# NVIDIAGameWorks/kaolin-wisp

Hardware: AMD Instinct MI355X
Metric: training rays/sec, HashGrid NeRF (nerf_hash.yaml), synthetic Lego 800x800 (higher is better)
Workload: dtype bf16

## Files before the change

### include/wisp_hip.h

```cpp
#ifndef WISP_HIP_H
#define WISP_HIP_H

#include <stdint.h>

#ifdef __cplusplus
extern "C" {
#endif

typedef void* wisp_stream_t;

enum { WISP_F32 = 0, WISP_F16 = 1, WISP_BF16 = 2 };

enum {
    WISP_OK = 0,
    WISP_ERR_INVALID = -1,
    WISP_ERR_LAUNCH = -2,
    WISP_ERR_UNSUPPORTED = -3,
    WISP_ERR_CAPACITY = -4
};

const char* wisp_last_error(void);
int wisp_abi_version(void);

int wisp_hashgrid_interpolate_fwd(const float* coords, int64_t n, int coord_dim,
                                  const void* codebook, int dtype, int feature_dim,
                                  const int64_t* first_idx, const int32_t* resolutions, int num_lods,
                                  int codebook_bitwidth, int zero_from_col,
                                  void* feats, wisp_stream_t stream);

int wisp_hashgrid_interpolate_bwd(const float* coords, int64_t n, int coord_dim,
                                  const void* grad_feats, int dtype, int feature_dim,
                                  const int64_t* first_idx, const int32_t* resolutions, int num_lods,
                                  int codebook_bitwidth, int zero_from_col,
                                  float* grad_codebook, void* workspace, int64_t workspace_bytes,
                                  const float* level_cap_scale , wisp_stream_t stream);
int64_t wisp_hashgrid_bwd_workspace_bytes(int64_t n, int coord_dim, int dtype ,
                                          int feature_dim, const int32_t* resolutions , int num_lods,
                                          int codebook_bitwidth, const float* level_cap_scale );
int wisp_hashgrid_bwd_slot_stats(int64_t n, int coord_dim, int dtype, int feature_dim, const int32_t* resolutions ,
                                 int num_lods, int codebook_bitwidth, int zero_from_col, const float* level_cap_scale,
                                 const void* workspace, int64_t workspace_bytes, uint32_t* max_fill, int32_t* cap_host,
                                 int32_t* base_cap_host, wisp_stream_t stream);

int wisp_hashgrid_grad_coords(const float* coords, int64_t n, int coord_dim, const void* grad_feats, const void* codebook,
                              int dtype, int feature_dim, const int64_t* first_idx, const int32_t* resolutions ,
                              int num_lods, int codebook_bitwidth, float* grad_coords, wisp_stream_t stream);

int wisp_hashgrid_interpolate_bwd_adamw(const float* coords, int64_t n, int coord_dim,
                                        const void* grad_feats, int dtype, int feature_dim,
                                        const int64_t* first_idx, const int32_t* resolutions, int num_lods,
                                        int codebook_bitwidth, int zero_from_col,
                                        float* grad_codebook, void* workspace, int64_t workspace_bytes,
                                        const float* level_cap_scale, float* param, float* exp_avg, float* exp_avg_sq,
                                        void* bf16_shadow, float lr, float beta1, float beta2, float eps, float weight_decay,
                                        int64_t step, float grad_scale, int64_t* covered_rows , wisp_stream_t stream);

typedef struct wisp_step_tail {
    const float* dw_partials;
    float* dec_grad;
    const float* loss_partials;
    float* loss;
    int32_t dw_rows, in_dim, loss_count;
    float inv_n;
} wisp_step_tail;
int wisp_hashgrid_interpolate_bwd_adamw_tail(const float* coords, int64_t n, int coord_dim,
                                             const void* grad_feats, int dtype, int feature_dim,
                                             const int64_t* first_idx, const int32_t* resolutions, int num_lods,
                                             int codebook_bitwidth, int zero_from_col,
                                             float* grad_codebook, void* workspace, int64_t workspace_bytes,
                                             const float* level_cap_scale, float* param, float* exp_avg, float* exp_avg_sq,
                                             void* bf16_shadow, float lr, float beta1, float beta2, float eps, float weight_decay,
                                             int64_t step, float grad_scale, int64_t* covered_rows ,
                                             const wisp_step_tail* tail, int* tail_done , wisp_stream_t stream);

int wisp_hashgrid_cells(const float* coords, int64_t n, int coord_dim, int32_t resolution, int codebook_bitwidth,
                        int32_t* cell, float* frac, int32_t* corner_idx, wisp_stream_t stream);

int wisp_hashgrid_query_fwd(const float* coords, int64_t n, const void* const* codebooks, int dtype, int feature_dim,
                            const int32_t* resolutions, int num_lods, int codebook_bitwidth, int probe_bitwidth,
                            void* feats, wisp_stream_t stream);
int wisp_hashgrid_query_bwd(const float* coords, int64_t n, const void* grad_feats, int dtype, int feature_dim,
                            const int32_t* resolutions, int num_lods, int codebook_bitwidth, int probe_bitwidth,
                            void* const* grad_codebooks, wisp_stream_t stream);

int wisp_spc_query(const uint8_t* octree, const int32_t* exsum, const float* coords, int64_t n,
                   int level, int with_parents, int64_t* pidx ,
                   wisp_stream_t stream);

int wisp_spc_query_chain(const uint8_t* octree, const int32_t* exsum, const int16_t* points, const float* coords,
                         int64_t n, int level, int first_level, const int32_t* hint_pidx, int hint_group,
                         int64_t* chain, wisp_stream_t stream);

int wisp_spc_build_bitfield(const int16_t* level_points, int64_t n_points, int level, uint32_t* bits,
                            wisp_stream_t stream);

int wisp_spc_mask_from_points(const int16_t* points, int64_t n, int level, uint8_t* leaf_mask, wisp_stream_t stream);
int wisp_spc_dense_bytes(uint8_t* dense, int level, wisp_stream_t stream);
int wisp_spc_points_from_index(const int64_t* index, int64_t n, int level, int16_t* points, wisp_stream_t stream);

int wisp_spc_raytrace_count(const uint8_t* octree, const int16_t* points, const int32_t* exsum,
                            const float* origins, const float* dirs, int64_t num_rays, int level,
                            int32_t* counts, float* cache, int cache_cap, wisp_stream_t stream);
int wisp_spc_raytrace_emit(const uint8_t* octree, const int16_t* points, const int32_t* exsum,
                           const float* origins, const float* dirs, int64_t num_rays, int level,
                           const int64_t* offsets, int with_exit, const float* cache, int cache_cap,
                           int32_t* ridx, int32_t* pidx, float* depth, wisp_stream_t stream);

int wisp_spc_first_hit(const uint8_t* octree, const int16_t* points, const int32_t* exsum,
                       const float* origins, const float* dirs, int64_t num_rays, int level,
                       const float* colors, int color_stride, int32_t level_first,
                       int32_t* pidx, float* depth, float* rgb, float* alpha, uint8_t* hit, wisp_stream_t stream);

int wisp_mark_pack_boundaries_i64(const int64_t* ids, int64_t n, uint8_t* boundary, wisp_stream_t stream);
int wisp_mark_pack_boundaries_i32(const int32_t* ids, int64_t n, uint8_t* boundary, wisp_stream_t stream);

int64_t wisp_scan_workspace_bytes(int64_t n);
int wisp_exclusive_scan_i32(const int32_t* counts, int64_t n, int64_t* offsets, void* workspace,
                            wisp_stream_t stream);
int wisp_inclusive_scan_i32(const int32_t* in, int64_t n, int32_t* out, void* workspace,
                            wisp_stream_t stream);
int wisp_boundary_tile_counts(const uint8_t* boundary, int64_t n, int32_t* counts, wisp_stream_t stream);
int wisp_boundary_pack_starts(const uint8_t* boundary, int64_t n, const int64_t* tile_offsets,
                              int64_t* starts, wisp_stream_t stream);

int wisp_spc_trilinear_coeffs(const float* coords, const int16_t* voxel_points , int64_t num_voxels,
                              int samples_per_voxel, int level, float* coeffs , wisp_stream_t stream);
int wisp_spc_trilinear_fwd(const float* coords, const void* pidx, int pidx_is_i64, const int16_t* points,
                           const int32_t* trinkets, const void* feats, int dtype, int64_t num_voxels,
                           int samples_per_voxel, int channels, int level, int half_round, float* out,
                           wisp_stream_t stream);
int wisp_spc_trilinear_bwd(const float* coords, const void* pidx, int pidx_is_i64, const int16_t* points,
                           const int32_t* trinkets, const float* grad_out, int64_t num_voxels,
                           int samples_per_voxel, int channels, int level, int64_t num_rows,
                           float* grad_feats , void* workspace, int64_t workspace_bytes,
                           wisp_stream_t stream);
int64_t wisp_spc_bwd_workspace_bytes(int64_t total_rows, int channels, int64_t dict_elems);

int wisp_spc_trilinear_multi_fwd(const float* coords, const int64_t* chain, int64_t chain_stride, const int16_t* points,
                                 const int32_t* trinkets, const void* const* feats, int dtype, int64_t num_samples,
                                 int num_lods, const int32_t* levels, int channels, int half_round, int sum, float* out,
                                 wisp_stream_t stream);
int wisp_spc_trilinear_multi_bwd(const float* coords, const int64_t* chain, int64_t chain_stride, const int16_t* points,
                                 const int32_t* trinkets, const float* grad_out, int64_t num_samples, int num_lods,
                                 const int32_t* levels, const int64_t* rows, int channels, int sum,
                                 float* const* grad_feats, void* workspace, int64_t workspace_bytes, wisp_stream_t stream);

int wisp_triplane_fwd(const float* coords, int64_t num_samples, const float* const* planes, const int32_t* sizes,
                      int num_lods, int feature_dim, int sum, float* out, wisp_stream_t stream);
int wisp_triplane_bwd(const float* coords, int64_t num_samples, const float* grad_out, const int32_t* sizes, int num_lods,
                      int feature_dim, int sum, float* const* grad_planes, wisp_stream_t stream);

int wisp_grid_interpolate_fwd(const float* coords, const void* feats, int dtype, int64_t num_coords, int feature_dim,
                              void* out, wisp_stream_t stream);
int wisp_grid_interpolate_bwd(const float* coords, const void* grad_out, int dtype, int64_t num_coords, int feature_dim,
                              void* grad_feats, wisp_stream_t stream);

// ... 244 lines not shown
                                        int64_t workspace_bytes, int* partial_rows , wisp_stream_t stream);
int wisp_nerf_mlp_reduce_partials(const float* workspace, int partial_rows, int in_dim, float* grad_params, wisp_stream_t stream);

int wisp_small_decoder_fwd(const float* x, int64_t n, int in_dim, int hidden, const float* w1, const float* b1,
                           const float* w2, const float* b2, float* out , wisp_stream_t stream);
int wisp_small_decoder_bwd(const float* x, int64_t n, int in_dim, int hidden, const float* w1, const float* b1,
                           const float* w2, const float* b2, const float* grad_out, float* grad_x, float* grad_w1,
                           float* grad_b1, float* grad_w2, float* grad_b2, wisp_stream_t stream);

int wisp_adamw_step(float* param, const float* grad, float* exp_avg, float* exp_avg_sq, int64_t n,
                    float lr, float beta1, float beta2, float eps, float weight_decay, int64_t step,
                    float grad_scale, int zero_grad , void* bf16_shadow,
                    wisp_stream_t stream);
int wisp_adamw_step_groups(float* param, const float* grad, float* exp_avg, float* exp_avg_sq, int num_groups,
                           const int64_t* group_begin, const int64_t* group_len, const float* group_lr,
                           const float* group_weight_decay, void* const* group_bf16_shadow, float beta1, float beta2,
                           float eps, int64_t step, float grad_scale, int zero_grad, wisp_stream_t stream);

int wisp_optim_step_groups(int kind, float* param, const float* grad, float* state1, float* state2, int num_groups,
                           const int64_t* group_begin, const int64_t* group_len, const float* group_lr,
                           const float* group_weight_decay, void* const* group_bf16_shadow, float hyper0, float hyper1,
                           float eps, int64_t step, float grad_scale, int zero_grad, wisp_stream_t stream);

int wisp_gather_rows(const int64_t* index, int64_t num, int64_t num_src_rows, int num_tensors, const float* const* src,
                     const int* width, float* const* dst, wisp_stream_t stream);

void* wisp_host_reader_create(void);
int wisp_host_reader_issue(void* reader, const int64_t* src, wisp_stream_t stream);
int wisp_host_reader_wait(void* reader, int64_t* value );
void wisp_host_reader_destroy(void* reader);

typedef struct wisp_nerf_step_config {
    int64_t struct_bytes;
    const uint32_t* occ_bits;
    const uint8_t* octree;
    const int32_t* exsum;
    const uint32_t* coarse_bits;
    const void* table_lookup;
    const int64_t* first_idx;
    const int64_t* first_idx_host;
    const int32_t* resolutions;
    float* table_param;
    float* table_grad;
    float* table_exp_avg;
    float* table_exp_avg_sq;
    void* table_shadow;
    const float* dec_params;
    float* dec_grad;
    float* flat_param;
    float* flat_grad;
    float* flat_exp_avg;
    float* flat_exp_avg_sq;
    void* grid_shadow;
    int64_t decoder_begin, decoder_len, grid_begin, grid_len, rest_begin, rest_len;
    int64_t table_offset;
    int64_t max_rays, max_samples;
    int32_t level, coarse_level, num_samples , loss_kind ;
    int32_t dtype_table, num_lods, feature_dim, bitwidth;
    int32_t zero_from_col, in_dim, hidden, view_freqs;
    float near, range ;
    float bg[3];
    float reserved;
} wisp_nerf_step_config;

typedef struct wisp_nerf_step_hyper {
    int64_t struct_bytes;
    int64_t step;
    float lr_decoder, lr_grid, lr_rest, weight_decay, beta1, beta2, eps, grad_scale;
    int32_t optimizer;
    int32_t tail_fold;
} wisp_nerf_step_hyper;

int64_t wisp_nerf_step_config_bytes(void);
int64_t wisp_nerf_step_workspace_bytes(const wisp_nerf_step_config* cfg);
void* wisp_nerf_step_create(const wisp_nerf_step_config* cfg, void* workspace, int64_t workspace_bytes);
int wisp_nerf_step_reconfigure(void* step, const wisp_nerf_step_config* cfg);
void wisp_nerf_step_destroy(void* step);
int wisp_nerf_step_count(void* step, int slot, const float* origins, const float* dirs, int64_t num_rays, uint64_t seed,
                         wisp_stream_t stream);
int wisp_nerf_step_run(void* step, int slot, const float* gts, const float* next_origins, const float* next_dirs,
                       int64_t next_num_rays, uint64_t next_seed, const wisp_nerf_step_hyper* hp,
                       const float* level_cap_scale, void* hashgrid_workspace, int64_t hashgrid_workspace_bytes,
                       int record_timing, int64_t* num_samples, int64_t* covered_rows, float** loss, wisp_stream_t stream);
int wisp_nerf_step_read_timing(void* step, int max_steps, float* ms, int64_t* units, int* num_steps);

int wisp_mesh_to_sdf(const double* points, int64_t n, const double* mesh, int64_t f, int triangle_ranges,
                     int64_t max_pairs_per_launch, double* sdf, void* workspace, int64_t workspace_bytes, wisp_stream_t stream);
int wisp_mesh_to_sdf_triangle(const double* points, int64_t n, const double* mesh, int64_t f, int triangle_ranges,
                              int64_t max_pairs_per_launch, double* out, void* workspace, int64_t workspace_bytes,
                              wisp_stream_t stream);
int64_t wisp_mesh_sdf_workspace_bytes(int64_t n, int64_t f);

typedef struct wisp_tex_material {
    int64_t offset;
    int32_t height, width;
    float kd[3];
    int32_t has_map;
} wisp_tex_material;
int wisp_mesh_closest_tex(const double* points, int64_t n, const double* mesh, int64_t f, const void* tidx, int tidx_is_i64,
                          const float* texv, int64_t tv, const int64_t* texf, const float* texels, int64_t num_texels,
                          const wisp_tex_material* materials, int num_materials, double* hit, float* rgb, wisp_stream_t stream);
int wisp_mesh_sample_tex(const float* uv, const int64_t* material, int64_t n, const float* texels, int64_t num_texels,
                         const wisp_tex_material* materials, int num_materials, float* rgb, wisp_stream_t stream);

int wisp_multiview_sample(const uint8_t* images, const float* cameras, const float* camera_host, int64_t num_views, int height,
                          int width, int mip, int has_alpha, const int64_t* pix, const int64_t* view, int64_t view_index,
                          int64_t num_rays, float x0, float y0, float tan_half_fov_x, float tan_half_fov_y, const float* bg,
                          float* origins, float* dirs, float* rgb, uint8_t* mask, wisp_stream_t stream);

int wisp_image_sample(const uint8_t* image, int height, int width, const int64_t* pix, int64_t n, float* coords, float* rgb,
                      wisp_stream_t stream);

int wisp_image_field_render(const float* coords, int64_t first, int64_t n, int height, int width, const float* codebook,
                            const int64_t* first_idx, const int32_t* resolutions, int num_lods, int active_lods,
                            int codebook_bitwidth, const float* weights, int hidden_padded, const uint8_t* gts, float* out_f32,
                            uint8_t* out_u8, double* err_partials, wisp_stream_t stream);
int64_t wisp_image_field_render_partials(int64_t n);

int64_t wisp_image_field_train_scratch_bytes(int64_t n, int num_lods, int hidden);
int wisp_image_field_train_step(const float* coords, const float* rgb, int64_t n, const float* codebook, const int64_t* first_idx,
                                const int32_t* resolutions, int num_lods, int active_lods, int codebook_bitwidth, const float* w1,
                                const float* b1, const float* w2, const float* b2, int hidden, float* grad_codebook,
                                float* grad_w1, float* grad_b1, float* grad_w2, float* grad_b2, float* loss, float* pred,
                                void* scratch, int64_t scratch_bytes, wisp_stream_t stream);

int64_t wisp_ssim_scratch_bytes(int H, int W, int C);
int wisp_ssim(const float* x, int64_t x_row_stride, int64_t x_pix_stride, const float* y, int64_t y_row_stride,
              int64_t y_pix_stride, int H, int W, int C, int radius, const double* weights, double cov_norm, double c1, double c2,
              double* out, double* map, void* scratch, int64_t scratch_bytes, wisp_stream_t stream);

#ifdef __cplusplus
}
#endif
#endif
```

### kaolin-wisp_amd/csrc/hashgrid.hip

```cpp
#include "wisp_common.h"
#include <stdlib.h>

#include "hashgrid_dev.h"
#include "step_tail_dev.h"

#define HG_TILE 64

#define FW_WAVES 4
template <typename T, int F, int DIM>
__global__ void __launch_bounds__(FW_WAVES * 64)
hashgrid_fwd_kernel(const float* __restrict__ coords, int64_t n, const T* __restrict__ codebook,
                    const int64_t* __restrict__ first_idx, HashLevels lv, int num_lods, uint32_t tsize,
                    int tsize_pow2, int zero_from_col, int row_shift, int off32, T* __restrict__ feats) {
    extern __shared__ __attribute__((aligned(16))) uint32_t stage_all[];
    constexpr int W = (F * (int)sizeof(T)) / 4;
    const int lane = threadIdx.x & 63;
    const int wave = threadIdx.x >> 6;
    uint32_t* stage = stage_all + (size_t)wave * num_lods * 65 * W;
    const int64_t ntiles = (n + HG_TILE - 1) / HG_TILE;
    const int row_dw = num_lods * W;

    const int nwaves = blockDim.x >> 6;
    for (int64_t tile = (int64_t)blockIdx.x * nwaves + wave; tile < ntiles; tile += (int64_t)gridDim.x * nwaves) {
        const int64_t i = tile * HG_TILE + lane;
        const bool live = i < n;
        float c[DIM];
#pragma unroll
        for (int a = 0; a < DIM; ++a) c[a] = live ? coords[i * DIM + a] : 0.0f;

        for (int l = 0; l < num_lods; ++l) {
            const int32_t res = lv.res[l];
            const bool dense = lv.dense[l] != 0;
            float acc[F];
#pragma unroll
            for (int k = 0; k < F; ++k) acc[k] = 0.0f;
            if (live && l * F < zero_from_col) {
                const T* __restrict__ table = codebook + first_idx[l] * F;
                CornerSetup<DIM> cs;
                corner_setup<DIM>(c, res, lv.hi[l], lv.hr[l], dense, tsize, tsize_pow2 != 0, cs);
                if (dense && res >= 258) {
                    const int64_t last = first_idx[num_lods] - 1 - first_idx[l];
#pragma unroll
                    for (int j = 0; j < (1 << DIM); ++j)
                        if ((int64_t)(uint32_t)cs.idx[j] > last) cs.idx[j] = (int32_t)last;
                }
                T v[1 << DIM][F];
                auto fetch = [&](int j, const T* p) {
                    if constexpr (W == 1) {
                        *reinterpret_cast<uint32_t*>(&v[j][0]) = *reinterpret_cast<const uint32_t*>(p);
                    } else if constexpr (W == 2) {
                        *reinterpret_cast<uint2*>(&v[j][0]) = *reinterpret_cast<const uint2*>(p);
                    } else if constexpr (W == 4) {
                        *reinterpret_cast<uint4*>(&v[j][0]) = *reinterpret_cast<const uint4*>(p);
                    } else {
#pragma unroll
                        for (int k = 0; k < F; ++k) v[j][k] = p[k];
                    }
                };
                if (off32 && (W == 1 || W == 2 || W == 4)) {
                    const __amdgpu_buffer_rsrc_t rsrc =
                        __builtin_amdgcn_make_buffer_rsrc(const_cast<T*>(table), (short)0, (int)0x7fffffff, 0x00020000);
                    if (W == 1 && dense && res < 258) {
                        constexpr int half = 1 << (DIM - 1);
                        typedef uint32_t u32x2_t __attribute__((ext_vector_type(2)));
#pragma unroll
                        for (int j = 0; j < half; ++j) {
                            const int voff = (int)((uint32_t)cs.idx[j] * (uint32_t)(F * sizeof(T)));
                            const u32x2_t t = __builtin_amdgcn_raw_buffer_load_b64(rsrc, voff, 0, 0);
                            *reinterpret_cast<uint32_t*>(&v[j][0]) = t[0];
                            *reinterpret_cast<uint32_t*>(&v[j + half][0]) = t[1];
                        }
                    } else if (W == 1 && !dense && tsize_pow2 != 0 && tsize >= 2u) {
                        constexpr int half = 1 << (DIM - 1);
                        typedef uint32_t u32x2_t __attribute__((ext_vector_type(2)));
#pragma unroll
                        for (int j = 0; j < half; ++j) {
                            const uint32_t i0 = (uint32_t)cs.idx[j];
                            const u32x2_t t = __builtin_amdgcn_raw_buffer_load_b64(rsrc, (int)((i0 & ~1u) * 4u), 0, 0);
                            const bool upper = (i0 & 1u) != 0;
                            *reinterpret_cast<uint32_t*>(&v[j][0]) = upper ? t[1] : t[0];
                            *reinterpret_cast<uint32_t*>(&v[j + half][0]) = upper ? t[0] : t[1];
                        }
                        if (cs.cell[0] & 1) {
#pragma unroll
// ... 125 lines not shown
                    asm volatile("v_fmac_f32_dpp %0, %0, %1 " DPPSTR : "+v"(v[j][k]) : "v"(tk));             \
            heads |= take & (SRC_FLAGS);                                                                   \
        }                                                                                                  \
    }
    HG_SEG_STEP("row_shr:1 row_mask:0xf bank_mask:0xf", 0xfffefffefffefffeull, heads << 1)
    HG_SEG_STEP("row_shr:2 row_mask:0xf bank_mask:0xf", 0xfffcfffcfffcfffcull, heads << 2)
    HG_SEG_STEP("row_shr:4 row_mask:0xf bank_mask:0xf", 0xfff0fff0fff0fff0ull, heads << 4)
    HG_SEG_STEP("row_shr:8 row_mask:0xf bank_mask:0xf", 0xff00ff00ff00ff00ull, heads << 8)
    HG_SEG_STEP("row_bcast:15 row_mask:0xa bank_mask:0xf", 0xffff0000ffff0000ull,
                (((heads >> 15) & 1ull) ? 0x00000000ffff0000ull : 0ull) | (((heads >> 47) & 1ull) ? 0xffff000000000000ull : 0ull))
    HG_SEG_STEP("row_bcast:31 row_mask:0xc bank_mask:0xf", 0xffffffff00000000ull,
                ((heads >> 31) & 1ull) ? 0xffffffff00000000ull : 0ull)
#undef HG_SEG_STEP
    const uint64_t emitters = tails & __builtin_amdgcn_ballot_w64(live);
    uint32_t is_tail;
    asm volatile("v_cndmask_b32_e64 %0, 0, 1, %1" : "=v"(is_tail) : "s"(emitters));
    return is_tail != 0;
}

template <typename T, int F, int DIM, bool MERGE>
__global__ void __launch_bounds__(1024)
hashgrid_bwd_kernel(const float* __restrict__ coords, int64_t n, const T* __restrict__ grad_feats,
                    const int64_t* __restrict__ first_idx, HashLevels lv, LevelList levels, int num_lods, uint32_t tsize,
                    int tsize_pow2, int zero_from_col, float* __restrict__ grad_codebook) {
    const int lane = threadIdx.x & 63;
    const int wave = threadIdx.x >> 6;
    const int nwaves = blockDim.x >> 6;
    const int64_t ntiles = (n + HG_TILE - 1) / HG_TILE;
    for (int64_t tile = blockIdx.x; tile < ntiles; tile += gridDim.x) {
        const int64_t i = tile * HG_TILE + lane;
        const bool live = i < n;
        float c[DIM];
#pragma unroll
        for (int a = 0; a < DIM; ++a) c[a] = live ? coords[i * DIM + a] : 0.0f;
        for (int li = wave; li < levels.n; li += nwaves) {
            const int l = __builtin_amdgcn_readfirstlane(levels.lv[li]);
            const int32_t res = __builtin_amdgcn_readfirstlane(lv.res[l]);
            const bool dense = __builtin_amdgcn_readfirstlane(lv.dense[l]) != 0;
            CornerSetup<DIM> cs;
            float v[1 << DIM][F];
            const bool issue = tail_compute<T, F, DIM, MERGE>(c, live, l, res, lv.hi[l], lv.hr[l], dense, tsize, tsize_pow2 != 0, zero_from_col,
                                                              grad_feats + (i * num_lods + l) * F, lane, cs, v);
            if (issue) {
                const int64_t base = first_idx[l], total_rows = first_idx[num_lods];
#pragma unroll
                for (int j = 0; j < (1 << DIM); ++j) {
                    const int64_t row = base + (int64_t)(uint32_t)cs.idx[j];
                    if (row >= total_rows) continue;
                    float* p = grad_codebook + row * F;
#pragma unroll
                    for (int k = 0; k < F; ++k) atomicAdd(p + k, v[j][k]);
                }
            }
        }
    }
}

#ifndef EM_THREADS
#define EM_THREADS 512
#endif
#ifndef EM_GROUPS
#define EM_GROUPS 2
#endif
#define EM_TILE (EM_THREADS * EM_GROUPS)
#ifndef EM_MIN_WAVES
#define EM_MIN_WAVES 2
#endif
#ifndef EQ_THREADS
#define EQ_THREADS 512
#endif
#define EQ_WIDE 1024
#define EQ_WIDE_MIN ((int64_t)1 << 20)
#define EQ_SMALL 1024
#define EQ_SMALL_GROUPS 1
#define RD_THREADS 1024
#define BIN_MAX_CHUNKS 1024
#ifndef HG_ACC_PLANES
#define HG_ACC_PLANES 1
#endif
#ifndef HG_FLUSH_PAIRS
#define HG_FLUSH_PAIRS 1
#endif

template <typename T, int F> struct RecordCodec {
    static constexpr bool COMPACT = (sizeof(T) == 2 && F == 2);
    static constexpr int RW = COMPACT ? 2 : 1 + F;
    static __device__ __forceinline__ uint32_t store(uint32_t* dst, uint32_t loc, const float (&v)[F]) {
        if constexpr (COMPACT) {
            uint2 w;
            w.x = ((__float_as_uint(v[0]) + 0x40u) & ~0x7fu) | (loc & 0x7fu);
            w.y = ((__float_as_uint(v[1]) + 0x40u) & ~0x7fu) | (loc >> 7);
            *reinterpret_cast<uint2*>(dst) = w;
            return max(w.x & 0x7fffff80u, w.y & 0x7fffff80u);
        } else {
            dst[0] = loc;
            uint32_t m = 0;
#pragma unroll
            for (int k = 0; k < F; ++k) { dst[1 + k] = __float_as_uint(v[k]); m = max(m, __float_as_uint(v[k]) & 0x7fffffffu); }
            return m;
        }
    }
    static __device__ __forceinline__ uint32_t load(const uint32_t (&w)[RW], float (&v)[F]) {
        if constexpr (COMPACT) {
            v[0] = __uint_as_float(w[0] & ~0x7fu);
            v[1] = __uint_as_float(w[1] & ~0x7fu);
            return (w[0] & 0x7fu) | ((w[1] & 0x7fu) << 7);
        } else {
#pragma unroll
            for (int k = 0; k < F; ++k) v[k] = __uint_as_float(w[1 + k]);
            return w[0];
        }
    }
};

template <typename T, int F, int DIM>
__global__ void __launch_bounds__(EM_THREADS, EM_MIN_WAVES)
hashgrid_bwd_emit_kernel(const float* __restrict__ coords, int64_t n, const T* __restrict__ grad_feats,
                         const int64_t* __restrict__ first_idx, HashLevels lv, LevelList levels, int num_lods,
                         uint32_t tsize, int tsize_pow2, int zero_from_col, int chunk_shift, BinLevels bins,
                         uint32_t* __restrict__ counts, uint32_t* __restrict__ records, float* __restrict__ grad_codebook) {
    constexpr int NC = 1 << DIM;
    typedef RecordCodec<T, F> Codec;
    constexpr int RW = Codec::RW;
    constexpr int GROUPS = EM_TILE / EM_THREADS;
    static_assert((F * sizeof(T)) % 4 == 0, "a (sample, level) gradient is a whole number of dwords");
    constexpr int W = (F * (int)sizeof(T)) / 4;
    extern __shared__ __attribute__((aligned(16))) uint32_t em_smem[];
    const int total_ranks = bins.rank_base[levels.n];
    uint32_t* s_rank = em_smem;
    uint32_t* s_mx = em_smem + total_ranks;
    uint32_t* s_grad = em_smem + total_ranks + 1;
    uint32_t mx = 0;
    if (threadIdx.x == 0) *s_mx = 0;
    const int row_dw = num_lods * W;
    const int rowp = row_dw | 1;
    const int lane = threadIdx.x & 63;
    const int wave = threadIdx.x >> 6;
    const uint32_t ntiles = gridDim.x;
    const int64_t tile0 = (int64_t)blockIdx.x * EM_TILE;
    const int64_t total_rows = first_idx[num_lods];
    for (int b = threadIdx.x; b < total_ranks; b += EM_THREADS) s_rank[b] = 0;
    {
        const int64_t rows = (n - tile0) < (int64_t)EM_TILE ? (n - tile0) : (int64_t)EM_TILE;
        const uint32_t* __restrict__ src = reinterpret_cast<const uint32_t*>(grad_feats) + tile0 * row_dw;
        const int total = (int)rows * row_dw;
        for (int e = threadIdx.x; e < total; e += EM_THREADS) {
            const int r = e / row_dw;
            s_grad[r * rowp + (e - r * row_dw)] = src[e];
        }
    }
    float c[GROUPS][DIM];
    bool live[GROUPS];
#pragma unroll
    for (int g = 0; g < GROUPS; ++g) {
        const int64_t i = tile0 + (int64_t)(wave * GROUPS + g) * 64 + lane;
        live[g] = i < n;
#pragma unroll
        for (int a = 0; a < DIM; ++a) c[g][a] = live[g] ? coords[i * DIM + a] : 0.0f;
    }
    __syncthreads();
    for (int li = 0; li < levels.n; ++li) {
        const int l = levels.lv[li];
        const int32_t res = lv.res[l];
        const bool dense = lv.dense[l] != 0;
        const uint32_t cap = bins.cap[li];
        uint32_t* rank_l = s_rank + bins.rank_base[li];
        uint32_t* __restrict__ rec_l = records + (size_t)bins.rec_base[li] * RW;
        const uint32_t bucket_stride = __builtin_amdgcn_readfirstlane(ntiles * cap);
        const uint32_t slot0 = __builtin_amdgcn_readfirstlane(blockIdx.x * cap);
        const int64_t rows_l = first_idx[l + 1] - first_idx[l];
        const uint32_t owned = (uint32_t)(rows_l < (int64_t)bins.entries[li] ? (rows_l < 0 ? 0 : rows_l) : (int64_t)bins.entries[li]);
        const uint32_t magic = bins.strip_magic[li], nbuckets = (uint32_t)bins.chunks[li], rot_mask = bins.rot_mask[li];
#pragma unroll
        for (int g = 0; g < GROUPS; ++g) {
            const int sl = (wave * GROUPS + g) * 64 + lane;
            CornerSetup<DIM> cs;
            float v[NC][F];
            const bool issue = tail_compute<T, F, DIM, true>(c[g], live[g], l, res, lv.hi[l], lv.hr[l], dense, tsize, tsize_pow2 != 0, zero_from_col,
                                                             reinterpret_cast<const T*>(s_grad + sl * rowp + l * W), lane, cs, v);
            if (!issue) continue;
            uint32_t pos[NC];
#pragma unroll
            for (int j = 0; j < NC; ++j) {
                const uint32_t idx = (uint32_t)cs.idx[j];
                uint32_t b, loc;
                bucket_of(idx, chunk_shift, magic, nbuckets, rot_mask, b, loc);
                pos[j] = idx < owned ? atomicAdd(&rank_l[b], 1u) : 0xffffffffu;
            }
#pragma unroll
            for (int j = 0; j < NC; ++j) {
                const uint32_t idx = (uint32_t)cs.idx[j];
                uint32_t b, loc;
                bucket_of(idx, chunk_shift, magic, nbuckets, rot_mask, b, loc);
                if (pos[j] < cap) {
                    uint32_t* dst = rec_l + (size_t)((b * bucket_stride + slot0 + pos[j]) * RW);
                    mx = max(mx, Codec::store(dst, loc, v[j]));
                } else {
                    const int64_t row = first_idx[l] + (int64_t)idx;
                    if (row < total_rows) {
                        float* p = grad_codebook + row * F;
#pragma unroll
                        for (int k = 0; k < F; ++k) atomicAdd(p + k, v[j][k]);
                    }
                }
            }
        }
    }
    if (mx) atomicMax(s_mx, mx);
    __syncthreads();
    if (threadIdx.x == 0) counts[bins.max_base + blockIdx.x] = *s_mx;
    for (int li = 0; li < levels.n; ++li) {
        const int chunks = bins.chunks[li];
        const uint32_t cap = bins.cap[li];
        const uint32_t* rank_l = s_rank + bins.rank_base[li];
        uint32_t* __restrict__ cnt_l = counts + bins.cnt_base[li];
        for (int b = threadIdx.x; b < chunks; b += EM_THREADS) {
            const uint32_t cn = rank_l[b];
            cnt_l[(size_t)b * ntiles + blockIdx.x] = cn < cap ? cn : cap;
        }
    }
}

#define EQ_MAX_ROW 16
template <typename T, int DIM, int THREADS, int GROUPS = 2>
__global__ void __launch_bounds__(THREADS, EM_MIN_WAVES)
hashgrid_bwd_emit_q_kernel(const float* __restrict__ coords, int64_t n, const T* __restrict__ grad_feats,
                           const int64_t* __restrict__ first_idx, HashLevels lv, LevelList levels, int num_lods,
                           uint32_t tsize, int tsize_pow2, int zero_from_col, int chunk_shift, BinLevels bins,
                           uint32_t* __restrict__ counts, uint32_t* __restrict__ records, float* __restrict__ grad_codebook) {
    constexpr int F = 2;
    constexpr int NC = 1 << DIM;
    typedef RecordCodec<T, F> Codec;
    static_assert(Codec::COMPACT, "two 16-bit features per level");
    constexpr int RW = Codec::RW;
    constexpr int TILE = THREADS * GROUPS;
    constexpr int QROW = 3 * NC + 1;
    extern __shared__ __attribute__((aligned(16))) uint32_t em_smem[];
    const int total_ranks = bins.rank_base[levels.n];
    uint32_t* s_rank = em_smem;
    uint32_t* s_mx = em_smem + total_ranks;
    uint32_t mx = 0;
    if (threadIdx.x == 0) *s_mx = 0;
    const int lane = threadIdx.x & 63;
    const int wave = threadIdx.x >> 6;
    uint32_t* s_queue = em_smem + ((total_ranks + 4) & ~3) + wave * (64 * QROW);
    const uint32_t ntiles = gridDim.x;
    const int64_t total_rows = first_idx[num_lods];
    for (int b = threadIdx.x; b < total_ranks; b += THREADS) s_rank[b] = 0;
    __syncthreads();
    const uint32_t q_lane = (uint32_t)((lane / NC) * QROW + (lane % NC) * 3);
    const int64_t pieces = (n + TILE - 1) / TILE;
    for (int64_t piece = blockIdx.x; piece < pieces; piece += gridDim.x) {
        const int64_t tile0 = piece * TILE;
        float c[GROUPS][DIM];
        bool live[GROUPS];
        typedef uint32_t row_t __attribute__((ext_vector_type(EQ_MAX_ROW)));
        row_t grow[GROUPS];
#pragma unroll
        for (int g = 0; g < GROUPS; ++g) {
            const int64_t i = tile0 + (int64_t)(wave * GROUPS + g) * 64 + lane;
            live[g] = i < n;
#pragma unroll
            for (int a = 0; a < DIM; ++a) c[g][a] = live[g] ? coords[i * DIM + a] : 0.0f;
            const uint32_t* __restrict__ src = reinterpret_cast<const uint32_t*>(grad_feats) + (live[g] ? i : 0) * num_lods;
            if (num_lods == EQ_MAX_ROW) {
#pragma unroll
                for (int q = 0; q < EQ_MAX_ROW / 4; ++q) {
                    const uint4 t = reinterpret_cast<const uint4*>(src)[q];
                    grow[g][4 * q] = t.x; grow[g][4 * q + 1] = t.y; grow[g][4 * q + 2] = t.z; grow[g][4 * q + 3] = t.w;
                }
            } else {
#pragma unroll
                for (int q = 0; q < EQ_MAX_ROW; ++q) grow[g][q] = q < num_lods ? src[q] : 0u;
            }
        }
        for (int li = 0; li < levels.n; ++li) {
            const int l = levels.lv[li];
            const int32_t res = lv.res[l];
            const bool dense = lv.dense[l] != 0;
            const uint32_t cap = bins.cap[li];
            uint32_t* rank_l = s_rank + bins.rank_base[li];
            uint32_t* __restrict__ rec_l = records + (size_t)bins.rec_base[li] * RW;
            const uint32_t bucket_stride = __builtin_amdgcn_readfirstlane(ntiles * cap);
            const uint32_t slot0 = __builtin_amdgcn_readfirstlane(blockIdx.x * cap);
            const int64_t base_l = first_idx[l];
            const int64_t rows_l = first_idx[l + 1] - base_l;
            const uint32_t owned = (uint32_t)(rows_l < (int64_t)bins.entries[li] ? (rows_l < 0 ? 0 : rows_l) : (int64_t)bins.entries[li]);
            const uint32_t magic = bins.strip_magic[li], nbuckets = (uint32_t)bins.chunks[li], rot_mask = bins.rot_mask[li];
#pragma unroll
            for (int g = 0; g < GROUPS; ++g) {
                CornerSetup<DIM> cs;
                float v[NC][F];
                uint32_t gw = grow[g][l & (EQ_MAX_ROW - 1)];
                const bool issue = tail_compute<T, F, DIM, true>(c[g], live[g], l, res, lv.hi[l], lv.hr[l], dense, tsize, tsize_pow2 != 0, zero_from_col,
                                                                 reinterpret_cast<const T*>(&gw), lane, cs, v);
                const uint64_t tails = __builtin_amdgcn_ballot_w64(issue);
                if (tails == 0) continue;
                if (issue) {
                    const uint32_t t = __builtin_amdgcn_mbcnt_hi((uint32_t)(tails >> 32), __builtin_amdgcn_mbcnt_lo((uint32_t)tails, 0u));
                    uint32_t* q = s_queue + t * QROW;
#pragma unroll
                    for (int j = 0; j < NC; ++j) {
                        q[3 * j] = (uint32_t)cs.idx[j];
                        q[3 * j + 1] = __float_as_uint(v[j][0]);
                        q[3 * j + 2] = __float_as_uint(v[j][1]);
                    }
                }
                __builtin_amdgcn_fence(__ATOMIC_RELEASE, "wavefront");
                __builtin_amdgcn_wave_barrier();
                const uint32_t total = (uint32_t)__popcll(tails) * NC;
                for (uint32_t p = 0; p < total; p += 64) {
                    if (p + lane < total) {
                        const uint32_t* q = s_queue + (p / NC) * QROW + q_lane;
                        const uint32_t idx = q[0];
                        float val[F];
                        val[0] = __uint_as_float(q[1]);
                        val[1] = __uint_as_float(q[2]);
                        uint32_t b, loc;
                        bucket_of(idx, chunk_shift, magic, nbuckets, rot_mask, b, loc);
                        const uint32_t pos = idx < owned ? atomicAdd(&rank_l[b], 1u) : 0xffffffffu;
                        if (pos < cap) {
                            uint32_t* dst = rec_l + (size_t)((b * bucket_stride + slot0 + pos) * RW);
                            mx = max(mx, Codec::store(dst, loc, val));
                        } else {
                            const int64_t row = base_l + (int64_t)idx;
                            if (row < total_rows) {
                                float* pg = grad_codebook + row * F;
                                atomicAdd(pg, val[0]);
                                atomicAdd(pg + 1, val[1]);
                            }
                        }
                    }
                }
                __builtin_amdgcn_fence(__ATOMIC_ACQUIRE, "wavefront");
                __builtin_amdgcn_wave_barrier();
            }
        }
    }
    if (mx) atomicMax(s_mx, mx);
    __syncthreads();
    if (threadIdx.x == 0) counts[bins.max_base + blockIdx.x] = *s_mx;
    for (int li = 0; li < levels.n; ++li) {
        const int chunks = bins.chunks[li];
        const uint32_t cap = bins.cap[li];
        const uint32_t* rank_l = s_rank + bins.rank_base[li];
        uint32_t* __restrict__ cnt_l = counts + bins.cnt_base[li];
        for (int b = threadIdx.x; b < chunks; b += THREADS) {
            const uint32_t cn = rank_l[b];
            cnt_l[(size_t)b * ntiles + blockIdx.x] = cn < cap ? cn : cap;
        }
    }
}

static inline size_t queue_emitter_lds(int total_ranks, int dim, int threads) {
    return ((size_t)((total_ranks + 4) & ~3) + (size_t)(threads / 64) * 64 * (3 * (1 << dim) + 1)) * 4;
}
template <typename T, int DIM, int THREADS, int GROUPS = 2>
static int queue_emitter_residency() {
    static const int v = [] {
        int nb = 0;
        auto eq = hashgrid_bwd_emit_q_kernel<T, DIM, THREADS, GROUPS>;
        const size_t lds = queue_emitter_lds(1024, DIM, THREADS);
        (void)hipFuncSetAttribute(reinterpret_cast<const void*>(eq), hipFuncAttributeMaxDynamicSharedMemorySize, (int)lds);
        if (hipOccupancyMaxActiveBlocksPerMultiprocessor(&nb, eq, THREADS, lds) != hipSuccess || nb <= 0) nb = THREADS >= 1024 ? 1 : 2;
        return nb;
    }();
    return v;
}

struct AccFix64 {
    unsigned long long* acc;
    float mul;
    double inv;
    __device__ __forceinline__ void zero(uint32_t i) const { acc[i] = 0ull; }
    __device__ __forceinline__ void add(uint32_t i, float v) const {
        const float a = fabsf(v) * mul;
        const float h = floorf(a);
        const unsigned long long mag = ((unsigned long long)(uint32_t)h << 32) | (uint32_t)((a - h) * 4294967296.0f);
        const unsigned long long sgn = (unsigned long long)(long long)((int32_t)__float_as_uint(v) >> 31);
        const unsigned long long q = (mag ^ sgn) - sgn;
        atomicAdd(acc + i, q);
    }
    __device__ __forceinline__ float get(uint32_t i) const { return (float)((double)(long long)acc[i] * inv); }
};
struct AccF32 {
    float* acc;
    __device__ __forceinline__ void zero(uint32_t i) const { acc[i] = 0.0f; }
    __device__ __forceinline__ void add(uint32_t i, float v) const { atomicAdd(acc + i, v); }
    __device__ __forceinline__ float get(uint32_t i) const { return acc[i]; }
};

struct AdamFlush {
    float* p; float* m; float* v; __hip_bfloat16* shadow;
    float lr, wd, b1, b2, eps, bc1, bc2_sqrt, gscale;
};
#define HG_TAIL_ROWS 8192
#define WISP_WHOLE_LEVEL ((int64_t)1 << 62)
struct TailLevels { int first_level, end_level, blocks; };
struct StepTail {
    const float* dw_partials; float* dec_grad; const float* loss_partials; float* loss;
    int dw_rows, in_dim, loss_count; float inv_n;
    int loss_wgs, dw_wgs, wgs;
};
static_assert(RD_THREADS == STEP_TAIL_THREADS, "the side jobs run in reduce workgroups");

template <typename T, int F, typename ACC, bool ADAM>
static __device__ __forceinline__ void
hashgrid_bwd_reduce_body(const ACC A, const int64_t* __restrict__ first_idx, const LevelList& levels, int chunk_shift,
                         const BinLevels& bins, uint32_t ntiles, const uint32_t* __restrict__ counts,
                         const uint32_t* __restrict__ records, float* __restrict__ grad_codebook, int li, int b, int z,
                         const AdamFlush& ad) {
    typedef RecordCodec<T, F> Codec;
    constexpr int RW = Codec::RW;
    const int splits = bins.splits[li];
    const int l = levels.lv[li];
    const uint32_t csize = 1u << chunk_shift;
    const uint32_t cap = bins.cap[li];
    const uint32_t first = (uint32_t)b << chunk_shift;
    const int64_t rows_l = first_idx[l + 1] - first_idx[l];
    const uint32_t entries = (uint32_t)(rows_l < (int64_t)bins.entries[li] ? (rows_l < 0 ? 0 : rows_l) : (int64_t)bins.entries[li]);
    const uint32_t magic = bins.strip_magic[li], nbuckets = (uint32_t)bins.chunks[li], rot_mask = bins.rot_mask[li];
    const bool strips = magic != 0;
    const uint32_t strip_rounds = (((entries + (1u << HG_STRIP_SHIFT) - 1u) >> HG_STRIP_SHIFT) + nbuckets - 1u) / nbuckets;
    const uint32_t lim = (strips ? min(strip_rounds << HG_STRIP_SHIFT, csize) : (entries > first ? min(entries - first, csize) : 0u)) * F;
    auto ax = [&](uint32_t x) -> uint32_t {
#if HG_ACC_PLANES
        return (x % (uint32_t)F) * csize + x / (uint32_t)F;
#else
        return x;
#endif
    };
    for (uint32_t e = threadIdx.x; e < lim; e += RD_THREADS) A.zero(ax(e));
    __syncthreads();
    const uint32_t* __restrict__ cnt = counts + bins.cnt_base[li] + (size_t)b * ntiles;
    const uint32_t* __restrict__ src = records + ((size_t)bins.rec_base[li] + (size_t)b * ntiles * cap) * RW;
    const int lane = threadIdx.x & 63, wave = threadIdx.x >> 6;
    constexpr int NW = RD_THREADS / 64;
    constexpr int INFLIGHT = 8;
    const uint32_t my_tiles = ntiles > (uint32_t)z ? (ntiles - z + splits - 1) / splits : 0u;
    for (uint32_t base = 0; base * NW + wave < my_tiles; base += 64) {
        const uint32_t k = (base + lane) * NW + wave;
        const uint32_t cnt_of_lane = k < my_tiles ? cnt[z + k * splits] : 0u;
        const uint32_t cc = (cnt_of_lane + 63u) >> 6;
        uint32_t inc = cc;
#pragma unroll
        for (int d = 1; d < 64; d <<= 1) {
            const uint32_t t = (uint32_t)__shfl_up((int)inc, d, 64);
            if (lane >= d) inc += t;
        }
        const uint32_t exc = inc - cc;
        const uint32_t pairs = (uint32_t)__builtin_amdgcn_readlane((int)inc, 63);
        for (uint32_t p0 = 0; p0 < pairs; p0 += INFLIGHT) {
            uint32_t w[INFLIGHT][RW];
            bool act[INFLIGHT];
#pragma unroll
            for (int u = 0; u < INFLIGHT; ++u) {
                const uint32_t pr = p0 + u < pairs ? p0 + u : p0;
                const int t = __popcll(__ballot(exc <= pr)) - 1;
                const uint32_t chunk = pr - (uint32_t)__builtin_amdgcn_readlane((int)exc, t);
                const uint32_t n_t = (uint32_t)__builtin_amdgcn_readlane((int)cnt_of_lane, t);
                const uint32_t r = chunk * 64 + lane;
                act[u] = (p0 + u < pairs) && r < n_t;
                const uint32_t tile = z + ((base + t) * NW + wave) * splits;
                const uint32_t* rec = src + ((size_t)tile * cap + (act[u] ? r : 0u)) * RW;
#pragma unroll
                for (int q = 0; q < RW; ++q) w[u][q] = rec[q];
            }
#pragma unroll
            for (int u = 0; u < INFLIGHT; ++u) {
                if (act[u]) {
                    float val[F];
                    const uint32_t e = Codec::load(w[u], val);
#pragma unroll
                    for (int kk = 0; kk < F; ++kk) {
#ifdef HG_EXP_NOATOM
                        if (e == 0xffffffffu && val[kk] == 123.0f)
#endif
                        A.add(ax(e * F + kk), val[kk]);
                    }
                }
            }
        }
    }
    __syncthreads();
    if (strips) {
        float* __restrict__ dl = grad_codebook + first_idx[l] * F;
        if constexpr (ADAM) {
            if (splits == 1) {
                const int64_t level0 = first_idx[l] * F;
                float2* __restrict__ pg = reinterpret_cast<float2*>(dl);
                float2* __restrict__ pp = reinterpret_cast<float2*>(ad.p + level0);
                float2* __restrict__ pm = reinterpret_cast<float2*>(ad.m + level0);
                float2* __restrict__ pv = reinterpret_cast<float2*>(ad.v + level0);
                uint32_t* __restrict__ ps = ad.shadow ? reinterpret_cast<uint32_t*>(ad.shadow + level0) : nullptr;
                constexpr int PQ = 4;
                const uint32_t pairs = lim / F;
                if ((((uintptr_t)grad_codebook | (uintptr_t)ad.p | (uintptr_t)ad.m | (uintptr_t)ad.v) & 7u) != 0) {
                    for (uint32_t e = threadIdx.x; e < lim; e += RD_THREADS) {
                        const uint32_t row = bucket_row((uint32_t)b, e / (uint32_t)F, chunk_shift, magic, nbuckets, rot_mask);
                        if (row >= entries) continue;
                        const int64_t x = level0 + (int64_t)row * F + e % (uint32_t)F;
                        const float c = grad_codebook[x];
                        float w = ad.p[x], m1 = ad.m[x], m2 = ad.v[x];
                        wisp_adamw_update(w, m1, m2, (c + A.get(ax(e))) * ad.gscale, ad.lr, ad.wd, ad.b1, ad.b2, ad.eps, ad.bc1, ad.bc2_sqrt);
                        ad.p[x] = w; ad.m[x] = m1; ad.v[x] = m2;
                        if (c != 0.0f) grad_codebook[x] = 0.0f;
                        if (ad.shadow) ad.shadow[x] = __float2bfloat16(w);
                    }
                    return;
                }
                for (uint32_t i0 = threadIdx.x; i0 < pairs; i0 += PQ * RD_THREADS) {
                    float2 cg[PQ], cp[PQ], cm[PQ], cv[PQ];
                    uint32_t row[PQ];
#pragma unroll
                    for (int q = 0; q < PQ; ++q) {
                        const uint32_t i = i0 + q * RD_THREADS;
                        row[q] = i < pairs ? bucket_row((uint32_t)b, i, chunk_shift, magic, nbuckets, rot_mask) : 0xffffffffu;
                        if (row[q] < entries) { cg[q] = pg[row[q]]; cp[q] = pp[row[q]]; cm[q] = pm[row[q]]; cv[q] = pv[row[q]]; }
                    }
#pragma unroll
                    for (int q = 0; q < PQ; ++q) {
                        const uint32_t i = i0 + q * RD_THREADS;
                        if (row[q] < entries) {
                            const bool dirty = cg[q].x != 0.0f || cg[q].y != 0.0f;
                            const float g0 = cg[q].x + A.get(ax(2 * i)), g1 = cg[q].y + A.get(ax(2 * i + 1));
                            wisp_adamw_update(cp[q].x, cm[q].x, cv[q].x, g0 * ad.gscale, ad.lr, ad.wd, ad.b1, ad.b2, ad.eps, ad.bc1, ad.bc2_sqrt);
                            wisp_adamw_update(cp[q].y, cm[q].y, cv[q].y, g1 * ad.gscale, ad.lr, ad.wd, ad.b1, ad.b2, ad.eps, ad.bc1, ad.bc2_sqrt);
                            pp[row[q]] = cp[q];
                            pm[row[q]] = cm[q];
                            pv[row[q]] = cv[q];
                            if (dirty) pg[row[q]] = make_float2(0.0f, 0.0f);
                            if (ps) {
                                const __hip_bfloat16 s0 = __float2bfloat16(cp[q].x), s1 = __float2bfloat16(cp[q].y);
                                ps[row[q]] = (uint32_t)__bfloat16_as_ushort(s0) | ((uint32_t)__bfloat16_as_ushort(s1) << 16);
                            }
                        }
                    }
                }
                return;
            }
        }
        auto elem = [&](uint32_t e) -> uint32_t {
            const uint32_t row = bucket_row((uint32_t)b, e / (uint32_t)F, chunk_shift, magic, nbuckets, rot_mask);
            return row < entries ? row * (uint32_t)F + e % (uint32_t)F : 0xffffffffu;
        };
        if (splits == 1) {
            constexpr int MAXE = 16;
            float cur[MAXE];
#pragma unroll
            for (int q = 0; q < MAXE; ++q) {
                const uint32_t e = threadIdx.x + q * RD_THREADS;
                const uint32_t x = e < lim ? elem(e) : 0xffffffffu;
                cur[q] = x != 0xffffffffu ? dl[x] : 0.0f;
            }
#pragma unroll
            for (int q = 0; q < MAXE; ++q) {
                const uint32_t e = threadIdx.x + q * RD_THREADS;
                const uint32_t x = e < lim ? elem(e) : 0xffffffffu;
                if (x != 0xffffffffu) {
                    const float a = A.get(ax(e));
                    if (a != 0.0f) dl[x] = cur[q] + a;
                }
            }
        } else {
            for (uint32_t e = threadIdx.x; e < lim; e += RD_THREADS) {
                const uint32_t x = elem(e);
                const float a = A.get(ax(e));
                if (x != 0xffffffffu && a != 0.0f) atomicAdd(dl + x, a);
            }
        }
        return;
    }
    const int64_t slice = (first_idx[l] + (int64_t)first) * F;
    float* __restrict__ dst = grad_codebook + slice;
    if constexpr (ADAM) {
        if (splits == 1) {
            float* __restrict__ pp = ad.p + slice;
            float* __restrict__ pm = ad.m + slice;
            float* __restrict__ pv = ad.v + slice;
            __hip_bfloat16* __restrict__ ps = ad.shadow ? ad.shadow + slice : nullptr;
            constexpr int PQ = 4;
            const uint32_t pairs = lim >> 1;
            if ((lim & 1u) == 0 && (((uintptr_t)dst | (uintptr_t)pp | (uintptr_t)pm | (uintptr_t)pv) & 7u) == 0) {
                for (uint32_t i0 = threadIdx.x; i0 < pairs; i0 += PQ * RD_THREADS) {
                    float2 cg[PQ], cp[PQ], cm[PQ], cv[PQ];
#pragma unroll
                    for (int q = 0; q < PQ; ++q) {
                        const uint32_t i = i0 + q * RD_THREADS;
                        if (i < pairs) {
                            cg[q] = reinterpret_cast<const float2*>(dst)[i]; cp[q] = reinterpret_cast<const float2*>(pp)[i];
                            cm[q] = reinterpret_cast<const float2*>(pm)[i]; cv[q] = reinterpret_cast<const float2*>(pv)[i];
                        }
                    }
#pragma unroll
                    for (int q = 0; q < PQ; ++q) {
                        const uint32_t i = i0 + q * RD_THREADS;
                        if (i < pairs) {
                            const bool dirty = cg[q].x != 0.0f || cg[q].y != 0.0f;
                            const float g0 = cg[q].x + A.get(ax(2 * i)), g1 = cg[q].y + A.get(ax(2 * i + 1));
                            wisp_adamw_update(cp[q].x, cm[q].x, cv[q].x, g0 * ad.gscale, ad.lr, ad.wd, ad.b1, ad.b2, ad.eps, ad.bc1, ad.bc2_sqrt);
                            wisp_adamw_update(cp[q].y, cm[q].y, cv[q].y, g1 * ad.gscale, ad.lr, ad.wd, ad.b1, ad.b2, ad.eps, ad.bc1, ad.bc2_sqrt);
                            reinterpret_cast<float2*>(pp)[i] = cp[q];
                            reinterpret_cast<float2*>(pm)[i] = cm[q];
                            reinterpret_cast<float2*>(pv)[i] = cv[q];
                            if (dirty) reinterpret_cast<float2*>(dst)[i] = make_float2(0.0f, 0.0f);
                            if (ps) {
                                const __hip_bfloat16 s0 = __float2bfloat16(cp[q].x), s1 = __float2bfloat16(cp[q].y);
                                reinterpret_cast<uint32_t*>(ps)[i] = (uint32_t)__bfloat16_as_ushort(s0) | ((uint32_t)__bfloat16_as_ushort(s1) << 16);
                            }
                        }
                    }
                }
            } else {
                for (uint32_t e = threadIdx.x; e < lim; e += RD_THREADS) {
                    const float c = dst[e];
                    float x = pp[e], m1 = pm[e], m2 = pv[e];
                    wisp_adamw_update(x, m1, m2, (c + A.get(ax(e))) * ad.gscale, ad.lr, ad.wd, ad.b1, ad.b2, ad.eps, ad.bc1, ad.bc2_sqrt);
                    pp[e] = x; pm[e] = m1; pv[e] = m2;
                    if (c != 0.0f) dst[e] = 0.0f;
                    if (ps) ps[e] = __float2bfloat16(x);
                }
            }
            return;
        }
    }
    if (splits == 1) {
        constexpr int MAXQ = 4;
        const uint32_t quads = lim >> 2;
        if (quads <= MAXQ * RD_THREADS && (lim & 3u) == 0 && ((uintptr_t)dst & 15u) == 0) {
            float4 cur[MAXQ];
#pragma unroll
            for (int q = 0; q < MAXQ; ++q) {
                const uint32_t i = threadIdx.x + q * RD_THREADS;
                if (i < quads) cur[q] = reinterpret_cast<const float4*>(dst)[i];
            }
#pragma unroll
            for (int q = 0; q < MAXQ; ++q) {
                const uint32_t i = threadIdx.x + q * RD_THREADS;
                if (i < quads) {
                    float4 t = cur[q];
                    t.x += A.get(ax(4 * i)); t.y += A.get(ax(4 * i + 1));
                    t.z += A.get(ax(4 * i + 2)); t.w += A.get(ax(4 * i + 3));
                    reinterpret_cast<float4*>(dst)[i] = t;
                }
            }
        } else if (HG_FLUSH_PAIRS && (lim >> 1) <= 2 * MAXQ * RD_THREADS && (lim & 1u) == 0 && ((uintptr_t)dst & 7u) == 0) {
            const uint32_t pairs = lim >> 1;
            float2 cur[2 * MAXQ];
#pragma unroll
            for (int q = 0; q < 2 * MAXQ; ++q) {
                const uint32_t i = threadIdx.x + q * RD_THREADS;
                if (i < pairs) cur[q] = reinterpret_cast<const float2*>(dst)[i];
            }
#pragma unroll
            for (int q = 0; q < 2 * MAXQ; ++q) {
                const uint32_t i = threadIdx.x + q * RD_THREADS;
                if (i < pairs) {
                    float2 t = cur[q];
                    t.x += A.get(ax(2 * i)); t.y += A.get(ax(2 * i + 1));
                    reinterpret_cast<float2*>(dst)[i] = t;
                }
            }
        } else {
            for (uint32_t e = threadIdx.x; e < lim; e += RD_THREADS) {
                const float a = A.get(ax(e));
                if (a != 0.0f) dst[e] += a;
            }
        }
    } else {
        for (uint32_t e = threadIdx.x; e < lim; e += RD_THREADS) {
            const float a = A.get(ax(e));
            if (a != 0.0f) atomicAdd(dst + e, a);
        }
    }
}

template <typename T, int F, bool ADAM>
__global__ void __launch_bounds__(RD_THREADS)
hashgrid_bwd_reduce_kernel(const int64_t* __restrict__ first_idx, LevelList levels, int chunk_shift, BinLevels bins,
                           uint32_t ntiles, const uint32_t* __restrict__ counts, const uint32_t* __restrict__ records,
                           float* __restrict__ grad_codebook, int extra_bits, AdamFlush ad, TailLevels tail, StepTail side) {
    extern __shared__ __attribute__((aligned(16))) unsigned char rd_smem[];
    __shared__ uint32_t s_wave_max[RD_THREADS / 64];
    if constexpr (ADAM) {
        if (blockIdx.x < (unsigned)side.wgs) {
            float* lds = reinterpret_cast<float*>(rd_smem);
            const int w = (int)blockIdx.x - side.loss_wgs;
            if (w < 0) wisp_tail::loss_sum(side.loss_partials, side.loss_count, side.inv_n, side.loss, (int)threadIdx.x, lds);
            else wisp_tail::dw_reduce(side.dw_partials, side.dw_rows, side.in_dim, side.dec_grad, w, (int)threadIdx.x, lds);
            return;
        }
        const unsigned tail_index = blockIdx.x - (unsigned)side.wgs;
        if (tail_index < (unsigned)tail.blocks) {
            const int64_t k = (int64_t)tail_index;
            const int64_t begin = first_idx[tail.first_level] * F, end = first_idx[tail.end_level] * F;
            for (int64_t lo = begin + k * (int64_t)(HG_TAIL_ROWS * F); lo < end; lo += (int64_t)tail.blocks * (HG_TAIL_ROWS * F)) {
                const int64_t hi = lo + HG_TAIL_ROWS * F < end ? lo + HG_TAIL_ROWS * F : end;
                for (int64_t e = lo + threadIdx.x; e < hi; e += RD_THREADS) {
                    const float c = grad_codebook[e];
                    float x = ad.p[e], m1 = ad.m[e], m2 = ad.v[e];
                    wisp_adamw_update(x, m1, m2, c * ad.gscale, ad.lr, ad.wd, ad.b1, ad.b2, ad.eps, ad.bc1, ad.bc2_sqrt);
                    ad.p[e] = x; ad.m[e] = m1; ad.v[e] = m2;
                    if (c != 0.0f) grad_codebook[e] = 0.0f;
                    if (ad.shadow) ad.shadow[e] = __float2bfloat16(x);
                }
            }
            return;
        }
    }
    const int bid = (int)(gridDim.x - 1u - blockIdx.x);
    int li = 0;
    while (li + 1 < levels.n && bid >= bins.blk_base[li + 1]) ++li;
    const int splits = bins.splits[li];
    const int local = bid - bins.blk_base[li];
    const int b = local / splits, z = local - b * splits;
    uint32_t m = 0;
    for (uint32_t t = threadIdx.x; t < ntiles; t += RD_THREADS) m = max(m, counts[bins.max_base + t]);
#pragma unroll
    for (int d = 32; d >= 1; d >>= 1) m = max(m, (uint32_t)__shfl_xor((int)m, d, 64));
    if ((threadIdx.x & 63) == 0) s_wave_max[threadIdx.x >> 6] = m;
    __syncthreads();
    m = s_wave_max[0];
#pragma unroll
    for (int w = 1; w < RD_THREADS / 64; ++w) m = max(m, s_wave_max[w]);
    const int e = (int)(m >> 23);
    if (e < 255) {
        int sh = 165 - e - extra_bits;
        if (sh > 159) sh = 159;
        AccFix64 A{reinterpret_cast<unsigned long long*>(rd_smem), __uint_as_float((uint32_t)(sh - 32 + 127) << 23),
                   __longlong_as_double((long long)(1023 - sh) << 52)};
        hashgrid_bwd_reduce_body<T, F, AccFix64, ADAM>(A, first_idx, levels, chunk_shift, bins, ntiles, counts, records, grad_codebook, li, b, z, ad);
    } else {
        AccF32 A{reinterpret_cast<float*>(rd_smem)};
        hashgrid_bwd_reduce_body<T, F, AccF32, ADAM>(A, first_idx, levels, chunk_shift, bins, ntiles, counts, records, grad_codebook, li, b, z, ad);
    }
}

static inline int hg_grid(int64_t n) {
    int64_t tiles = ceil_div64(n, HG_TILE);
    int64_t g = tiles < 2048 ? tiles : 2048;
    return (int)(g < 1 ? 1 : g);
}

template <typename T, int F, int DIM>
static int launch_fwd(const float* coords, int64_t n, const void* codebook, const int64_t* first_idx,
                      const HashLevels& lv, int num_lods, uint32_t tsize, int zero_from_col, void* feats,
                      hipStream_t s) {
    constexpr int W = (F * (int)sizeof(T)) / 4;
    const size_t wave_lds = (size_t)num_lods * 65 * W * 4;
    int waves = FW_WAVES;
    while (waves > 1 && waves * wave_lds > 64 * 1024) --waves;
    const size_t lds = waves * wave_lds;
    const int pow2 = (tsize & (tsize - 1)) == 0;
    const int row_dw = num_lods * W;
    int row_shift = -1;
    if ((row_dw & (row_dw - 1)) == 0) { row_shift = 0; while ((1 << row_shift) < row_dw) ++row_shift; }
    auto kern = hashgrid_fwd_kernel<T, F, DIM>;
    if (lds > 48 * 1024) { if (const hipError_t e = WISP_ALLOW_LDS(kern, lds)) return wisp_fail(WISP_ERR_LAUNCH, __func__, hipGetErrorString(e)); }
    const int64_t tiles = ceil_div64(n, HG_TILE);
    int64_t g = ceil_div64(tiles, waves);
    if (g > 8192) g = 8192;
    const int off32 = (uint64_t)num_lods * tsize * F * sizeof(T) < 0x7fffffffull ? 1 : 0;
    hipLaunchKernelGGL(kern, dim3((unsigned)(g < 1 ? 1 : g)), dim3(waves * 64), lds, s, coords, n, (const T*)codebook,
                       first_idx, lv, num_lods, tsize, pow2, zero_from_col, row_shift, off32, (T*)feats);
    return 0;
}

static bool env_flag(const char* name, bool dflt) {
    const char* e = getenv(name);
    if (!e || !e[0]) return dflt;
    return e[0] != '0';
}
static bool bwd_merge_enabled() { static const bool v = env_flag("WISP_HG_BWD_MERGE", true); return v; }
static bool bwd_bin_enabled() { static const bool v = env_flag("WISP_HG_BWD_BIN", true); return v; }

static bool strip_buckets_enabled() { static const bool v = env_flag("WISP_HG_STRIP_BUCKETS", true); return v; }
static bool queue_emitter_enabled() { static const bool v = env_flag("WISP_HG_BWD_QUEUE", true); return v; }
static int64_t queue_emitter_grid_cap(int resident_per_cu) {
    static const int forced = [] { const char* e = getenv("WISP_HG_EMIT_WGS_PER_CU"); return e && e[0] ? atoi(e) : -1; }();
    const int per_cu = forced >= 0 ? forced : resident_per_cu;
    static const int cus = [] {
        int dev = 0, v = 0;
        if (hipGetDevice(&dev) != hipSuccess ||
            hipDeviceGetAttribute(&v, hipDeviceAttributeMultiprocessorCount, dev) != hipSuccess || v <= 0) v = 256;
        return v;
    }();
    return per_cu > 0 ? (int64_t)per_cu * cus : 0;
}

static int64_t coarse_level_wgs(int64_t n) { return n >= ((int64_t)1 << 21) ? 64 : 16; }

struct BinPlan { int chunk_shift, max_chunks, max_splits, total_blocks, total_ranks, emit_threads ; int64_t ntiles; BinLevels bins; int64_t count_bytes, record_bytes; bool ok;
                 uint32_t base_cap[HG_MAX_LODS]; };
static BinPlan bin_plan(int64_t n, const HashLevels& lv, const LevelList& levels, int feature_dim, int64_t tsize, int dim,
                        int rec_dwords, int64_t max_emitters = 0, const float* cap_scale = nullptr, int64_t piece = EM_TILE) {
    BinPlan p{};
    const int corners = 1 << dim;
    int64_t centries = 16384 / feature_dim;
    {
        static const struct { int64_t entries, below; } alt = [] {
            const char* e = getenv("WISP_HG_CHUNK_ENTRIES_BELOW");
            long long a = 0, b = 0;
            if (e && sscanf(e, "%lld:%lld", &a, &b) == 2 && a >= 256 && b > 0) return decltype(alt){(int64_t)a, (int64_t)b};
            return decltype(alt){0, 0};
        }();
        if (alt.entries > 0 && n < alt.below && alt.entries < centries) centries = alt.entries;
    }
    while (((int64_t)1 << (p.chunk_shift + 1)) <= centries) ++p.chunk_shift;
    p.ntiles = ceil_div64(n, piece);
    p.emit_threads = 0;
    int64_t tile_samples = piece;
    if (max_emitters > 0 && p.ntiles > max_emitters) {
        const int64_t pieces_per_wg = ceil_div64(p.ntiles, max_emitters);
        tile_samples = pieces_per_wg * piece;
        p.ntiles = ceil_div64(p.ntiles, pieces_per_wg);
    }
    int64_t cnt = 0, rec = 0;
    p.ok = true;
    for (int li = 0; li < levels.n; ++li) {
        const int l = levels.lv[li];
        int64_t entries = tsize;
        if (lv.dense[l]) { entries = 1; for (int a = 0; a < dim; ++a) entries *= (int64_t)lv.res[l]; }
        if (entries > tsize) entries = tsize;
        const int64_t chunks = (entries + ((int64_t)1 << p.chunk_shift) - 1) >> p.chunk_shift;
        int64_t cap = (tile_samples * corners + chunks - 1) / chunks;
        cap = lv.dense[l] ? cap * 2 : cap + cap / 4;
        if (cap < 128) cap = 128;
        if (lv.dense[l] && cap > 2048 * (tile_samples / EM_TILE)) cap = 2048 * (tile_samples / EM_TILE);
        if (cap > tile_samples * corners) cap = tile_samples * corners;
        p.base_cap[li] = (uint32_t)cap;
        if (cap_scale) {
            float f = cap_scale[l];
            if (!(f > 0.0f)) f = 1.0f;
            if (f < 1.0f) { cap = (int64_t)((double)cap * f) + 1; if (cap < 32) cap = 32; }
        }
        if (max_emitters > 0) {
            cap = (cap + 31) / 32;
            cap = (cap | 1) * 32;
        }
        if (chunks > BIN_MAX_CHUNKS || entries > 0xffffffffLL || chunks * p.ntiles * cap * rec_dwords > 0xffffffffLL) p.ok = false;
        p.bins.chunks[li] = (int32_t)chunks;
        p.bins.strip_magic[li] = 0; p.bins.rot_mask[li] = 0;
        if (lv.dense[l] && chunks >= 2 && strip_buckets_enabled()) {
            p.bins.strip_magic[li] = (uint32_t)((((uint64_t)1 << 32) + (uint64_t)chunks - 1) / (uint64_t)chunks);
            uint32_t pw = 1; while (pw * 2 <= (uint32_t)chunks) pw *= 2;
            p.bins.rot_mask[li] = pw - 1;
        }
        p.bins.cap[li] = (uint32_t)cap;
        p.bins.cnt_base[li] = cnt;
        p.bins.rec_base[li] = rec;
        p.bins.entries[li] = (uint32_t)entries;
        int splits = (int)(coarse_level_wgs(n) / chunks);
        if (splits < 2 && chunks <= 32) splits = 2;
        if (splits > p.ntiles) splits = (int)p.ntiles;
        p.bins.splits[li] = splits < 1 ? 1 : splits;
        if (chunks > p.max_chunks) p.max_chunks = (int)chunks;
        if (p.bins.splits[li] > p.max_splits) p.max_splits = p.bins.splits[li];
        p.bins.blk_base[li] = p.total_blocks;
        p.total_blocks += (int)chunks * p.bins.splits[li];
        p.bins.rank_base[li] = p.total_ranks;
        p.total_ranks += (int)chunks;
        cnt += chunks * p.ntiles;
        rec += chunks * p.ntiles * cap;
    }
    p.bins.blk_base[levels.n] = p.total_blocks;
    p.bins.rank_base[levels.n] = p.total_ranks;
    p.bins.max_base = cnt;
    cnt += p.ntiles;
    p.count_bytes = (cnt * 4 + 255) / 256 * 256;
    p.record_bytes = rec * rec_dwords * 4;
    return p;
}

// ... 114 lines not shown
    while (((int64_t)1 << (21 + extra_bits)) < n) ++extra_bits;
    StepTail side{};
    if (fused && side_jobs && side_done && rd_lds >= sizeof(float) * STEP_TAIL_DW_LDS_FLOATS) {
        side = *side_jobs;
        side.loss_wgs = side.loss_partials && side.loss ? 1 : 0;
        side.dw_wgs = side.dw_partials && side.dec_grad && side.dw_rows > 0 ? wisp_tail::DW_COL_BLOCKS : 0;
        side.wgs = side.loss_wgs + side.dw_wgs;
        *side_done = 1;
    }
    hipLaunchKernelGGL(rd, dim3(plan.total_blocks + tail.blocks + side.wgs), dim3(RD_THREADS), rd_lds, s, first_idx, active, plan.chunk_shift,
                       plan.bins, (uint32_t)plan.ntiles, counts, records, grad_codebook, extra_bits, fused ? *adam : AdamFlush{}, tail, side);
    return 0;
}

#define HG_DISPATCH_F(T, DIM, FN, ...)                                   \
    switch (feature_dim) {                                               \
        case 2: FN<T, 2, DIM>(__VA_ARGS__); break;                       \
        case 4: FN<T, 4, DIM>(__VA_ARGS__); break;                       \
        case 8: FN<T, 8, DIM>(__VA_ARGS__); break;                       \
        case 16: FN<T, 16, DIM>(__VA_ARGS__); break;                     \
        default: return wisp_fail(WISP_ERR_UNSUPPORTED, __func__, "feature_dim must be 2, 4, 8 or 16"); \
    }

#define HG_DISPATCH(FN, ...)                                             \
    if (coord_dim == 3) {                                                \
        if (dtype == WISP_F32) { HG_DISPATCH_F(float, 3, FN, __VA_ARGS__) }              \
        else if (dtype == WISP_F16) { HG_DISPATCH_F(__half, 3, FN, __VA_ARGS__) }        \
        else { HG_DISPATCH_F(__hip_bfloat16, 3, FN, __VA_ARGS__) }                       \
    } else {                                                             \
        if (dtype == WISP_F32) { HG_DISPATCH_F(float, 2, FN, __VA_ARGS__) }              \
        else if (dtype == WISP_F16) { HG_DISPATCH_F(__half, 2, FN, __VA_ARGS__) }        \
        else { HG_DISPATCH_F(__hip_bfloat16, 2, FN, __VA_ARGS__) }                       \
    }

extern "C" int wisp_hashgrid_interpolate_fwd(const float* coords, int64_t n, int coord_dim, const void* codebook,
                                             int dtype, int feature_dim, const int64_t* first_idx,
                                             const int32_t* resolutions, int num_lods, int codebook_bitwidth,
                                             int zero_from_col, void* feats, wisp_stream_t stream) {
    WISP_REQUIRE(n >= 0, "negative n");
    if (n == 0) return WISP_OK;
    WISP_REQUIRE(coords && codebook && first_idx && resolutions && feats, "null pointer");
    WISP_REQUIRE(coord_dim == 2 || coord_dim == 3, "coord_dim must be 2 or 3");
    WISP_REQUIRE(num_lods >= 1 && num_lods <= HG_MAX_LODS, "num_lods out of range");
    WISP_REQUIRE(codebook_bitwidth >= 1 && codebook_bitwidth <= 30, "codebook_bitwidth out of range");
    WISP_REQUIRE(dtype == WISP_F32 || dtype == WISP_F16 || dtype == WISP_BF16, "bad dtype");
    HashLevels lv;
    const int64_t tsize = (int64_t)1 << codebook_bitwidth;
    WISP_REQUIRE(fill_levels(resolutions, num_lods, coord_dim, tsize, lv) == 0, "bad resolution");
    hipStream_t s = (hipStream_t)stream;
    HG_DISPATCH(launch_fwd, coords, n, codebook, first_idx, lv, num_lods, (uint32_t)tsize, zero_from_col, feats, s)
    WISP_CHECK_LAUNCH();
    return WISP_OK;
}

extern "C" int wisp_hashgrid_interpolate_bwd(const float* coords, int64_t n, int coord_dim, const void* grad_feats,
                                             int dtype, int feature_dim, const int64_t* first_idx,
                                             const int32_t* resolutions, int num_lods, int codebook_bitwidth,
                                             int zero_from_col, float* grad_codebook, void* workspace,
                                             int64_t workspace_bytes, const float* level_cap_scale, wisp_stream_t stream) {
    WISP_REQUIRE(n >= 0, "negative n");
    if (n == 0) return WISP_OK;
    WISP_REQUIRE(coords && grad_feats && first_idx && resolutions && grad_codebook, "null pointer");
    WISP_REQUIRE(coord_dim == 2 || coord_dim == 3, "coord_dim must be 2 or 3");
    WISP_REQUIRE(num_lods >= 1 && num_lods <= HG_MAX_LODS, "num_lods out of range");
    WISP_REQUIRE(codebook_bitwidth >= 1 && codebook_bitwidth <= 30, "codebook_bitwidth out of range");
    WISP_REQUIRE(dtype == WISP_F32 || dtype == WISP_F16 || dtype == WISP_BF16, "bad dtype");
    HashLevels lv;
    const int64_t tsize = (int64_t)1 << codebook_bitwidth;
    WISP_REQUIRE(fill_levels(resolutions, num_lods, coord_dim, tsize, lv) == 0, "bad resolution");
    hipStream_t s = (hipStream_t)stream;
    HG_DISPATCH(launch_bwd, coords, n, grad_feats, first_idx, lv, num_lods, (uint32_t)tsize, zero_from_col,
                grad_codebook, workspace, workspace_bytes, level_cap_scale, s)
    WISP_CHECK_LAUNCH();
    return WISP_OK;
}

static int bwd_adamw_impl(const float* coords, int64_t n, int coord_dim, const void* grad_feats,
                          int dtype, int feature_dim, const int64_t* first_idx,
                          const int32_t* resolutions, int num_lods, int codebook_bitwidth,
                          int zero_from_col, float* grad_codebook, void* workspace,
                          int64_t workspace_bytes, const float* level_cap_scale, float* param,
                          float* exp_avg, float* exp_avg_sq, void* bf16_shadow, float lr, float beta1,
                          float beta2, float eps, float weight_decay, int64_t step, float grad_scale,
                          int64_t* covered_rows, const StepTail* side_jobs, int* side_done,
                          wisp_stream_t stream) {
    WISP_REQUIRE(n >= 0, "negative n");
    WISP_REQUIRE(num_lods >= 1 && num_lods <= HG_MAX_LODS, "num_lods out of range");
    WISP_REQUIRE(covered_rows && param && exp_avg && exp_avg_sq && step >= 1, "optimizer arguments missing");
    for (int l = 0; l < num_lods; ++l) covered_rows[l] = 0;
    if (n == 0) return WISP_OK;
    WISP_REQUIRE(coords && grad_feats && first_idx && resolutions && grad_codebook, "null pointer");
    WISP_REQUIRE(coord_dim == 2 || coord_dim == 3, "coord_dim must be 2 or 3");
    WISP_REQUIRE(codebook_bitwidth >= 1 && codebook_bitwidth <= 30, "codebook_bitwidth out of range");
    WISP_REQUIRE(dtype == WISP_F32 || dtype == WISP_F16 || dtype == WISP_BF16, "bad dtype");
    HashLevels lv;
    const int64_t tsize = (int64_t)1 << codebook_bitwidth;
    WISP_REQUIRE(fill_levels(resolutions, num_lods, coord_dim, tsize, lv) == 0, "bad resolution");
    const AdamFlush ad{param, exp_avg, exp_avg_sq, (__hip_bfloat16*)bf16_shadow, lr, weight_decay, beta1, beta2, eps,
                       1.0f - powf(beta1, (float)step), sqrtf(1.0f - powf(beta2, (float)step)), grad_scale};
    hipStream_t s = (hipStream_t)stream;
    HG_DISPATCH(launch_bwd, coords, n, grad_feats, first_idx, lv, num_lods, (uint32_t)tsize, zero_from_col,
                grad_codebook, workspace, workspace_bytes, level_cap_scale, s, &ad, covered_rows, side_jobs, side_done)
    WISP_CHECK_LAUNCH();
    return WISP_OK;
}

extern "C" int wisp_hashgrid_interpolate_bwd_adamw(const float* coords, int64_t n, int coord_dim, const void* grad_feats,
                                                   int dtype, int feature_dim, const int64_t* first_idx,
                                                   const int32_t* resolutions, int num_lods, int codebook_bitwidth,
                                                   int zero_from_col, float* grad_codebook, void* workspace,
                                                   int64_t workspace_bytes, const float* level_cap_scale, float* param,
                                                   float* exp_avg, float* exp_avg_sq, void* bf16_shadow, float lr, float beta1,
                                                   float beta2, float eps, float weight_decay, int64_t step, float grad_scale,
                                                   int64_t* covered_rows, wisp_stream_t stream) {
    return bwd_adamw_impl(coords, n, coord_dim, grad_feats, dtype, feature_dim, first_idx, resolutions, num_lods, codebook_bitwidth,
                          zero_from_col, grad_codebook, workspace, workspace_bytes, level_cap_scale, param, exp_avg, exp_avg_sq, bf16_shadow,
                          lr, beta1, beta2, eps, weight_decay, step, grad_scale, covered_rows, nullptr, nullptr, stream);
}

extern "C" int wisp_hashgrid_interpolate_bwd_adamw_tail(const float* coords, int64_t n, int coord_dim, const void* grad_feats,
                                                        int dtype, int feature_dim, const int64_t* first_idx,
                                                        const int32_t* resolutions, int num_lods, int codebook_bitwidth,
                                                        int zero_from_col, float* grad_codebook, void* workspace,
                                                        int64_t workspace_bytes, const float* level_cap_scale, float* param,
                                                        float* exp_avg, float* exp_avg_sq, void* bf16_shadow, float lr, float beta1,
                                                        float beta2, float eps, float weight_decay, int64_t step, float grad_scale,
                                                        int64_t* covered_rows, const wisp_step_tail* tail, int* tail_done,
                                                        wisp_stream_t stream) {
    WISP_REQUIRE(tail && tail_done, "side-job descriptor missing");
    WISP_REQUIRE(tail->dw_rows >= 0 && tail->loss_count >= 0 && tail->in_dim >= 1 && tail->in_dim <= wisp_mlp::IN, "side-job descriptor out of range");
    *tail_done = 0;
    StepTail side{};
    side.dw_partials = tail->dw_partials; side.dec_grad = tail->dec_grad; side.dw_rows = tail->dw_rows; side.in_dim = tail->in_dim;
    side.loss_partials = tail->loss_partials; side.loss = tail->loss; side.loss_count = tail->loss_count; side.inv_n = tail->inv_n;
    return bwd_adamw_impl(coords, n, coord_dim, grad_feats, dtype, feature_dim, first_idx, resolutions, num_lods, codebook_bitwidth,
                          zero_from_col, grad_codebook, workspace, workspace_bytes, level_cap_scale, param, exp_avg, exp_avg_sq, bf16_shadow,
                          lr, beta1, beta2, eps, weight_decay, step, grad_scale, covered_rows, &side, tail_done, stream);
}

template <typename T>
__global__ void __launch_bounds__(256)
hashgrid_grad_coords_kernel(const float* __restrict__ coords, int64_t n, const T* __restrict__ grad_feats,
                            const T* __restrict__ codebook, const int64_t* __restrict__ first_idx, HashLevels lv, int num_lods,
                            int F, uint32_t tsize, int pow2, float* __restrict__ grad_coords) {
    const int64_t i = (int64_t)blockIdx.x * blockDim.x + threadIdx.x;
    if (i >= n) return;
    const float c[3] = {coords[i * 3], coords[i * 3 + 1], coords[i * 3 + 2]};
    float gx = 0.0f, gy = 0.0f, gz = 0.0f;
    for (int l = 0; l < num_lods; ++l) {
        CornerSetup<3> cs;
        corner_setup<3>(c, lv.res[l], lv.hi[l], lv.hr[l], lv.dense[l] != 0, tsize, pow2 != 0, cs);
        const int64_t base = first_idx[l];
        const int64_t rows = first_idx[l + 1] - base;
        const T* __restrict__ tab = codebook + base * F;
        int64_t r[8];
#pragma unroll
        for (int k = 0; k < 8; ++k) { int64_t q = cs.idx[k]; r[k] = (q < rows ? q : rows - 1) * F; }
        const float x_ = cs.frac[0], y_ = cs.frac[1], z_ = cs.frac[2];
        const float _x = 1.0f - x_, _y = 1.0f - y_, _z = 1.0f - z_;
        for (int j = 0; j < F; ++j) {
            const float go = (float)grad_feats[i * (int64_t)num_lods * F + j];
            float v[8];
#pragma unroll
            for (int k = 0; k < 8; ++k) v[k] = (float)tab[r[k] + j];
            gx += go * ((_y * _z) * (v[4] - v[0]) + (_y * z_) * (v[5] - v[1]) + (y_ * _z) * (v[6] - v[2]) + (y_ * z_) * (v[7] - v[3]));
            gy += go * ((_x * _z) * (v[2] - v[0]) + (_x * z_) * (v[3] - v[1]) + (x_ * _z) * (v[6] - v[4]) + (x_ * z_) * (v[7] - v[6]));
            gz += go * ((_x * _y) * (v[1] - v[0]) + (_x * y_) * (v[3] - v[2]) + (x_ * _y) * (v[5] - v[4]) + (x_ * y_) * (v[7] - v[6]));
        }
    }
    grad_coords[i * 3] = gx; grad_coords[i * 3 + 1] = gy; grad_coords[i * 3 + 2] = gz;
}

extern "C" int wisp_hashgrid_grad_coords(const float* coords, int64_t n, int coord_dim, const void* grad_feats, const void* codebook,
                                         int dtype, int feature_dim, const int64_t* first_idx, const int32_t* resolutions,
                                         int num_lods, int codebook_bitwidth, float* grad_coords, wisp_stream_t stream) {
    WISP_REQUIRE(n >= 0, "negative n");
    if (n == 0) return WISP_OK;
    WISP_REQUIRE(coords && grad_feats && codebook && first_idx && resolutions && grad_coords, "null pointer");
    WISP_REQUIRE(coord_dim == 2 || coord_dim == 3, "coord_dim must be 2 or 3");
    WISP_REQUIRE(num_lods >= 1 && num_lods <= HG_MAX_LODS, "num_lods out of range");
    WISP_REQUIRE(feature_dim >= 1, "feature_dim out of range");
    WISP_REQUIRE(codebook_bitwidth >= 1 && codebook_bitwidth <= 30, "codebook_bitwidth out of range");
    WISP_REQUIRE(dtype == WISP_F32 || dtype == WISP_F16 || dtype == WISP_BF16, "bad dtype");
    hipStream_t s = (hipStream_t)stream;
    if (coord_dim == 2) {
        if (const hipError_t e = hipMemsetAsync(grad_coords, 0, sizeof(float) * 3 * (size_t)n, s)) return wisp_fail(WISP_ERR_LAUNCH, __func__, hipGetErrorString(e));
        return WISP_OK;
    }
    HashLevels lv;
    const int64_t tsize = (int64_t)1 << codebook_bitwidth;
    WISP_REQUIRE(fill_levels(resolutions, num_lods, coord_dim, tsize, lv) == 0, "bad resolution");
    const dim3 grid((unsigned)ceil_div64(n, 256));
    const int pow2 = 1;
    if (dtype == WISP_F32)
        hipLaunchKernelGGL(hashgrid_grad_coords_kernel<float>, grid, dim3(256), 0, s, coords, n, (const float*)grad_feats,
                           (const float*)codebook, first_idx, lv, num_lods, feature_dim, (uint32_t)tsize, pow2, grad_coords);
    else if (dtype == WISP_F16)
        hipLaunchKernelGGL(hashgrid_grad_coords_kernel<__half>, grid, dim3(256), 0, s, coords, n, (const __half*)grad_feats,
                           (const __half*)codebook, first_idx, lv, num_lods, feature_dim, (uint32_t)tsize, pow2, grad_coords);
    else
        hipLaunchKernelGGL(hashgrid_grad_coords_kernel<__hip_bfloat16>, grid, dim3(256), 0, s, coords, n, (const __hip_bfloat16*)grad_feats,
                           (const __hip_bfloat16*)codebook, first_idx, lv, num_lods, feature_dim, (uint32_t)tsize, pow2, grad_coords);
    WISP_CHECK_LAUNCH();
    return WISP_OK;
}

struct QueryLevels {
    int32_t res[HG_MAX_LODS]; int32_t dense[HG_MAX_LODS]; float hi[HG_MAX_LODS]; float hr[HG_MAX_LODS];
    void* table[HG_MAX_LODS];
};

template <typename T, bool BWD>
__global__ void __launch_bounds__(256)
hashgrid_query_kernel(const float* __restrict__ coords, int64_t n, QueryLevels lv, int num_lods, uint32_t mod, int pow2,
                      int probe, int F, int64_t table_rows, T* __restrict__ io) {
    const int64_t e = (int64_t)blockIdx.x * blockDim.x + threadIdx.x;
    if (e >= n * num_lods) return;
    const int64_t i = e / num_lods;
    const int l = (int)(e - i * num_lods);
    const float c[3] = {coords[i * 3], coords[i * 3 + 1], coords[i * 3 + 2]};
// ... 89 lines not shown
                                       void* const* grad_codebooks, wisp_stream_t stream) {
    if (int rc = query_check(coords, n, grad_codebooks, dtype, feature_dim, resolutions, num_lods, codebook_bitwidth, probe_bitwidth, grad_feats)) return rc;
    if (n == 0) return WISP_OK;
    for (int l = 0; l < num_lods; ++l) WISP_REQUIRE(grad_codebooks[l], "null gradient table");
    WISP_REQUIRE(launch_query<true>(coords, n, grad_codebooks, dtype, feature_dim, resolutions, num_lods, codebook_bitwidth,
                                    probe_bitwidth, const_cast<void*>(grad_feats), (hipStream_t)stream) == 0, "bad resolution");
    WISP_CHECK_LAUNCH();
    return WISP_OK;
}

template <int DIM>
__global__ void __launch_bounds__(256)
hashgrid_cells_kernel(const float* __restrict__ coords, int64_t n, int32_t res, float hi, float hr, int dense, uint32_t tsize,
                      int pow2, int32_t* __restrict__ cell, float* __restrict__ frac, int32_t* __restrict__ corner_idx) {
    const int64_t i = (int64_t)blockIdx.x * blockDim.x + threadIdx.x;
    if (i >= n) return;
    float c[DIM];
#pragma unroll
    for (int a = 0; a < DIM; ++a) c[a] = coords[i * DIM + a];
    CornerSetup<DIM> cs;
    corner_setup<DIM>(c, res, hi, hr, dense != 0, tsize, pow2 != 0, cs);
#pragma unroll
    for (int a = 0; a < DIM; ++a) { cell[i * DIM + a] = cs.cell[a]; frac[i * DIM + a] = cs.frac[a]; }
    if (corner_idx) {
#pragma unroll
        for (int j = 0; j < (1 << DIM); ++j) corner_idx[i * (1 << DIM) + j] = cs.idx[j];
    }
}

extern "C" int wisp_hashgrid_cells(const float* coords, int64_t n, int coord_dim, int32_t resolution, int codebook_bitwidth,
                                   int32_t* cell, float* frac, int32_t* corner_idx, wisp_stream_t stream) {
    WISP_REQUIRE(n >= 0, "negative n");
    if (n == 0) return WISP_OK;
    WISP_REQUIRE(coords && cell && frac, "null pointer");
    WISP_REQUIRE(coord_dim == 2 || coord_dim == 3, "coord_dim must be 2 or 3");
    WISP_REQUIRE(codebook_bitwidth >= 1 && codebook_bitwidth <= 30, "codebook_bitwidth out of range");
    HashLevels lv;
    const int64_t tsize = (int64_t)1 << codebook_bitwidth;
    WISP_REQUIRE(fill_levels(&resolution, 1, coord_dim, tsize, lv) == 0, "bad resolution");
    const int pow2 = 1;
    const dim3 grid((unsigned)ceil_div64(n, 256)), block(256);
    hipStream_t s = (hipStream_t)stream;
    if (coord_dim == 3)
        hipLaunchKernelGGL(hashgrid_cells_kernel<3>, grid, block, 0, s, coords, n, lv.res[0], lv.hi[0], lv.hr[0], lv.dense[0],
                           (uint32_t)tsize, pow2, cell, frac, corner_idx);
    else
        hipLaunchKernelGGL(hashgrid_cells_kernel<2>, grid, block, 0, s, coords, n, lv.res[0], lv.hi[0], lv.hr[0], lv.dense[0],
                           (uint32_t)tsize, pow2, cell, frac, corner_idx);
    WISP_CHECK_LAUNCH();
    return WISP_OK;
}

extern "C" int64_t wisp_hashgrid_bwd_workspace_bytes(int64_t n, int coord_dim, int dtype, int feature_dim,
                                                     const int32_t* resolutions, int num_lods, int codebook_bitwidth,
                                                     const float* level_cap_scale) {
    if (n <= 0 || num_lods <= 0 || num_lods > HG_MAX_LODS || feature_dim <= 0 || !resolutions) return 0;
    if (coord_dim != 2 && coord_dim != 3) return 0;
    HashLevels lv;
    const int64_t tsize = (int64_t)1 << codebook_bitwidth;
    if (fill_levels(resolutions, num_lods, coord_dim, tsize, lv) != 0) return 0;
    LevelList all{0, {0}};
    for (int l = 0; l < num_lods; ++l) all.lv[all.n++] = l;
    if (dtype == WISP_F32 || dtype == WISP_F16 || dtype == WISP_BF16) {
        const BinPlan e = plan_for(n, lv, all, coord_dim, feature_dim, dtype, tsize, num_lods, level_cap_scale);
        return e.ok ? e.count_bytes + e.record_bytes : 0;
    }
    const BinPlan p = bin_plan(n, lv, all, feature_dim, tsize, coord_dim, 1 + feature_dim, 0, level_cap_scale);
    int64_t bytes = p.ok ? p.count_bytes + p.record_bytes : 0;
    if (feature_dim == 2 && num_lods <= EQ_MAX_ROW && queue_emitter_enabled()) {
        const BinPlan q = plan_for(n, lv, all, coord_dim, feature_dim, WISP_BF16, tsize, num_lods, level_cap_scale);
        if (q.ok && q.count_bytes + q.record_bytes > bytes) bytes = q.count_bytes + q.record_bytes;
    }
    return bytes;
}

__global__ void __launch_bounds__(1024)
hashgrid_bwd_slot_stats_kernel(LevelList levels, BinLevels bins, uint32_t ntiles, int num_lods, const uint32_t* __restrict__ counts,
                               uint32_t* __restrict__ max_fill) {
    __shared__ uint32_t s_max[16], s_sum[16];
    const int li = blockIdx.x;
    const uint32_t* __restrict__ c = counts + bins.cnt_base[li];
    const int64_t cells = (int64_t)bins.chunks[li] * ntiles;
    uint32_t m = 0, sum = 0;
    for (int64_t e = threadIdx.x; e < cells; e += blockDim.x) { const uint32_t v = c[e]; m = max(m, v); sum += v; }
#pragma unroll
    for (int d = 32; d >= 1; d >>= 1) { m = max(m, (uint32_t)__shfl_xor((int)m, d, 64)); sum += (uint32_t)__shfl_xor((int)sum, d, 64); }
    if ((threadIdx.x & 63) == 0) { s_max[threadIdx.x >> 6] = m; s_sum[threadIdx.x >> 6] = sum; }
    __syncthreads();
    if (threadIdx.x == 0) {
        for (int w = 1; w < 16; ++w) { m = max(m, s_max[w]); sum += s_sum[w]; }
        max_fill[levels.lv[li]] = m;
        max_fill[num_lods + levels.lv[li]] = sum;
    }
}

extern "C" int wisp_hashgrid_bwd_slot_stats(int64_t n, int coord_dim, int dtype, int feature_dim, const int32_t* resolutions,
                                            int num_lods, int codebook_bitwidth, int zero_from_col, const float* level_cap_scale,
                                            const void* workspace, int64_t workspace_bytes, uint32_t* max_fill,
                                            int32_t* cap_host, int32_t* base_cap_host, wisp_stream_t stream) {
    WISP_REQUIRE(n > 0 && resolutions && max_fill && cap_host && base_cap_host, "bad arguments");
    WISP_REQUIRE(coord_dim == 2 || coord_dim == 3, "coord_dim must be 2 or 3");
    WISP_REQUIRE(num_lods >= 1 && num_lods <= HG_MAX_LODS, "num_lods out of range");
    HashLevels lv;
    const int64_t tsize = (int64_t)1 << codebook_bitwidth;
    WISP_REQUIRE(fill_levels(resolutions, num_lods, coord_dim, tsize, lv) == 0, "bad resolution");
    LevelList active{0, {0}};
    for (int l = 0; l < num_lods; ++l)
        if (l * feature_dim < zero_from_col) active.lv[active.n++] = l;
    for (int l = 0; l < num_lods; ++l) { cap_host[l] = 0; base_cap_host[l] = 0; }
    const BinPlan plan = plan_for(n, lv, active, coord_dim, feature_dim, dtype, tsize, num_lods, level_cap_scale);
    bool merge = bwd_merge_enabled() && bwd_bin_enabled() && (feature_dim * (1 << coord_dim) <= 32);
    for (int l = 0; l < num_lods; ++l)
        if (lv.res[l] > 65536) merge = false;
    const int elem = dtype == WISP_F32 ? 4 : 2;
    const size_t em_lds = ((size_t)plan.total_ranks + 1 + (size_t)EM_TILE * ((num_lods * ((feature_dim * elem) / 4)) | 1)) * 4;
    if (!merge || em_lds > 150 * 1024 || !workspace || !plan.ok || plan.count_bytes + plan.record_bytes > workspace_bytes || n < 4096 ||
        active.n == 0)
        return 1;
    for (int li = 0; li < active.n; ++li) { cap_host[active.lv[li]] = (int32_t)plan.bins.cap[li]; base_cap_host[active.lv[li]] = (int32_t)plan.base_cap[li]; }
    hipStream_t s = (hipStream_t)stream;
    (void)hipMemsetAsync(max_fill, 0, sizeof(uint32_t) * 2 * num_lods, s);
    hipLaunchKernelGGL(hashgrid_bwd_slot_stats_kernel, dim3(active.n), dim3(1024), 0, s, active, plan.bins, (uint32_t)plan.ntiles,
                       num_lods, (const uint32_t*)workspace, max_fill);
    WISP_CHECK_LAUNCH();
    return WISP_OK;
}
```

### kaolin-wisp_amd/csrc/train_step.hip

```cpp
#include "wisp_common.h"

#include <new>
#include <vector>

namespace {

constexpr int NS_TIMED_KERNELS = 4;
constexpr int NS_STEP_EVENTS = 6;
constexpr int NS_EV_BEGIN[NS_TIMED_KERNELS] = {0, 1, 3, 4};
constexpr int NS_EV_END[NS_TIMED_KERNELS] = {1, 2, 4, 5};
constexpr int NS_MAX_TIMED_STEPS = 512;
constexpr int NS_LOSS_RING = 8;

struct MarchSlot {
    const float* origins = nullptr;
    const float* dirs = nullptr;
    int64_t num_rays = 0;
    uint64_t seed = 0;
    uint32_t* hitmask = nullptr;
    int32_t* counts = nullptr;
    int64_t* offsets = nullptr;
    void* scan_ws = nullptr;
    void* reader = nullptr;
    bool counted = false;
};

struct Layout {
    int64_t hitmask[2], counts[2], offsets[2], scan_ws[2];
    int64_t ridx, samples, depth, deltas, boundary, feats, dir_code, image, color, density, g_color, g_density, g_feats, comp_ws, loss, mlp_ws;
    int64_t comp_ws_floats, mlp_ws_bytes, total;
};

static int64_t align256(int64_t v) { return (v + 255) / 256 * 256; }

static int elt_bytes(int dtype) { return dtype == WISP_F32 ? 4 : 2; }

static Layout layout_of(const wisp_nerf_step_config& c) {
    Layout L{};
    int64_t at = 0;
    auto take = [&](int64_t bytes) { const int64_t o = at; at = align256(at + bytes); return o; };
    const int64_t R = c.max_rays, S = c.max_samples;
    const int64_t words = (c.num_samples + 31) / 32;
    for (int k = 0; k < 2; ++k) {
        L.hitmask[k] = take(R * words * 4);
        L.counts[k] = take(R * 4);
        L.offsets[k] = take((R + 1) * 8);
        L.scan_ws[k] = take(wisp_scan_workspace_bytes(R));
    }
    const int64_t row = (int64_t)c.num_lods * c.feature_dim * elt_bytes(c.dtype_table);
    L.ridx = take(S * 8);
    L.samples = take(S * 12);
    L.depth = take(S * 4);
    L.deltas = take(S * 4);
    L.boundary = take(S);
    L.feats = take(S * row);
    L.dir_code = take(R * 32 * 2);
    const int64_t image_bytes = wisp_nerf_mlp_operand_image_bytes(c.hidden);
    L.image = take(image_bytes > 0 ? image_bytes : 0);
    L.color = take(S * 12);
    L.density = take(S * 4);
    L.g_color = take(S * 12);
    L.g_density = take(S * 4);
    L.g_feats = take(S * row);
    L.comp_ws_floats = R > 4096 ? 2 * R : 8192;
    L.comp_ws = take(L.comp_ws_floats * 4);
    L.loss = take(NS_LOSS_RING * 4);
    L.mlp_ws_bytes = wisp_nerf_mlp_bwd_workspace_bytes(S, c.hidden) + 256;
    L.mlp_ws = take(L.mlp_ws_bytes);
    L.total = at;
    return L;
}

struct Step {
    wisp_nerf_step_config cfg;
    std::vector<int64_t> first_idx_host;
    std::vector<int32_t> res;
    char* ws = nullptr;
    Layout lay{};
    MarchSlot slot[2];
    int loss_at = 0;
    std::vector<hipEvent_t> ev;
    std::vector<int64_t> ev_units;
    int timed_steps = 0;
};

template <typename T> static T* at(const Step* s, int64_t off) { return reinterpret_cast<T*>(s->ws + off); }

static bool config_ok(const wisp_nerf_step_config* c, const char** why) {
#define NEED(cond, text) do { if (!(cond)) { *why = text; return false; } } while (0)
    NEED(c != nullptr, "null config");
    NEED(c->struct_bytes == (int64_t)sizeof(wisp_nerf_step_config), "wisp_nerf_step_config has another size than this library's (header / binding drift)");
    NEED(c->octree && c->exsum && c->level >= 1 && c->level <= 10 && c->num_samples >= 1, "occupancy structure");
    NEED(c->range > 0.0f, "dist_max must exceed dist_min");
    NEED(c->table_lookup && c->first_idx && c->first_idx_host && c->resolutions, "hash table");
    NEED(c->num_lods >= 1 && c->num_lods <= 16 && c->feature_dim == 2, "the fused step covers two-feature tables of at most 16 levels");
    NEED(c->dtype_table == WISP_BF16 || c->dtype_table == WISP_F16, "the fused step reads a 16-bit copy of the table (bf16 / fp16)");
    NEED(c->in_dim == c->num_lods * c->feature_dim && c->in_dim <= 32 && c->hidden == 64 && c->view_freqs == 4, "decoder shape (hidden 64, 4 view frequencies, 'cat' features)");
    NEED(c->dec_params && c->dec_grad && c->table_grad, "parameter / gradient pointers");
    NEED(c->loss_kind >= 0 && c->loss_kind <= 2, "loss kind");
    NEED(c->max_rays >= 1 && c->max_samples >= 1, "capacities");
    NEED(c->flat_param && c->flat_grad && c->flat_exp_avg && c->flat_exp_avg_sq, "flat optimizer buffers");
#undef NEED
    return true;
}

static int do_count(Step* s, int k, const float* o, const float* d, int64_t R, uint64_t seed, hipStream_t st) {
    const wisp_nerf_step_config& c = s->cfg;
    MarchSlot& m = s->slot[k];
    m.counted = false;
    if (!o || !d || R < 1) return wisp_fail(WISP_ERR_INVALID, "wisp_nerf_step_count", "null rays");
    if (R > c.max_rays) return wisp_fail(WISP_ERR_CAPACITY, "wisp_nerf_step_count", "more rays than the step was created for");
    int rc = wisp_raymarch_ray_count(c.occ_bits, c.octree, c.exsum, o, d, R, c.near, c.range, c.num_samples, c.level, nullptr, seed,
                                     c.coarse_bits, c.coarse_level, m.hitmask, m.counts, st);
    if (rc != WISP_OK) return rc;
    rc = wisp_exclusive_scan_i32(m.counts, R, m.offsets, m.scan_ws, st);
    if (rc != WISP_OK) return rc;
    rc = wisp_host_reader_issue(m.reader, m.offsets + R, st);
    if (rc != WISP_OK) return rc;
    m.origins = o; m.dirs = d; m.num_rays = R; m.seed = seed; m.counted = true;
    return WISP_OK;
}

}

extern "C" int64_t wisp_nerf_step_config_bytes(void) { return (int64_t)sizeof(wisp_nerf_step_config); }

extern "C" int64_t wisp_nerf_step_workspace_bytes(const wisp_nerf_step_config* cfg) {
    const char* why = "";
    if (!config_ok(cfg, &why)) return wisp_fail(WISP_ERR_INVALID, __func__, why);
    return layout_of(*cfg).total + 256;
}

extern "C" void* wisp_nerf_step_create(const wisp_nerf_step_config* cfg, void* workspace, int64_t workspace_bytes) {
    const char* why = "";
    if (!config_ok(cfg, &why)) { (void)wisp_fail(WISP_ERR_INVALID, __func__, why); return nullptr; }
    Step* s = new (std::nothrow) Step();
    if (!s) return nullptr;
    s->cfg = *cfg;
    s->first_idx_host.assign(cfg->first_idx_host, cfg->first_idx_host + cfg->num_lods + 1);
    s->res.assign(cfg->resolutions, cfg->resolutions + cfg->num_lods);
    s->cfg.first_idx_host = s->first_idx_host.data();
    s->cfg.resolutions = s->res.data();
    s->lay = layout_of(s->cfg);
    char* base = reinterpret_cast<char*>((reinterpret_cast<uintptr_t>(workspace) + 255) / 256 * 256);
    if (!workspace || base + s->lay.total > reinterpret_cast<char*>(workspace) + workspace_bytes) {
        (void)wisp_fail(WISP_ERR_INVALID, __func__, "workspace smaller than wisp_nerf_step_workspace_bytes()");
        delete s;
        return nullptr;
    }
    s->ws = base;
    for (int k = 0; k < 2; ++k) {
        MarchSlot& m = s->slot[k];
        m.hitmask = at<uint32_t>(s, s->lay.hitmask[k]);
        m.counts = at<int32_t>(s, s->lay.counts[k]);
        m.offsets = at<int64_t>(s, s->lay.offsets[k]);
        m.scan_ws = at<void>(s, s->lay.scan_ws[k]);
        m.reader = wisp_host_reader_create();
        if (!m.reader) {
            (void)wisp_fail(WISP_ERR_LAUNCH, __func__, "wisp_host_reader_create failed");
            if (k == 1) wisp_host_reader_destroy(s->slot[0].reader);
            delete s;
            return nullptr;
        }
    }
    s->ev.reserve((size_t)NS_MAX_TIMED_STEPS * NS_STEP_EVENTS);
    for (int i = 0; i < NS_MAX_TIMED_STEPS * NS_STEP_EVENTS; ++i) {
        hipEvent_t e;
        if (hipEventCreate(&e) != hipSuccess) break;
        s->ev.push_back(e);
    }
    s->ev_units.assign(NS_MAX_TIMED_STEPS, 0);
    return s;
}

extern "C" int wisp_nerf_step_reconfigure(void* step, const wisp_nerf_step_config* cfg) {
    WISP_REQUIRE(step, "null handle");
    const char* why = "";
    if (!config_ok(cfg, &why)) return wisp_fail(WISP_ERR_INVALID, __func__, why);
    Step* s = static_cast<Step*>(step);
    const Layout now = layout_of(*cfg);
    if (now.total != s->lay.total || cfg->max_rays != s->cfg.max_rays || cfg->max_samples != s->cfg.max_samples ||
        cfg->num_samples != s->cfg.num_samples || cfg->num_lods != s->cfg.num_lods || cfg->dtype_table != s->cfg.dtype_table ||
        cfg->hidden != s->cfg.hidden)
        return wisp_fail(WISP_ERR_INVALID, __func__, "another workspace layout: destroy the handle and create a new one");
    for (int k = 0; k < 2; ++k)
        if (s->slot[k].counted) { int64_t v = 0; (void)wisp_host_reader_wait(s->slot[k].reader, &v); s->slot[k].counted = false; }
    s->cfg = *cfg;
    s->first_idx_host.assign(cfg->first_idx_host, cfg->first_idx_host + cfg->num_lods + 1);
    s->res.assign(cfg->resolutions, cfg->resolutions + cfg->num_lods);
    s->cfg.first_idx_host = s->first_idx_host.data();
    s->cfg.resolutions = s->res.data();
    return WISP_OK;
}

extern "C" void wisp_nerf_step_destroy(void* step) {
    if (!step) return;
    Step* s = static_cast<Step*>(step);
    for (int k = 0; k < 2; ++k) {
        if (s->slot[k].counted) { int64_t v = 0; (void)wisp_host_reader_wait(s->slot[k].reader, &v); }
        wisp_host_reader_destroy(s->slot[k].reader);
    }
    for (hipEvent_t e : s->ev) (void)hipEventDestroy(e);
    delete s;
}

extern "C" int wisp_nerf_step_count(void* step, int slot, const float* origins, const float* dirs, int64_t num_rays, uint64_t seed,
                                    wisp_stream_t stream) {
    WISP_REQUIRE(step && (slot == 0 || slot == 1), "bad handle / slot");
    Step* s = static_cast<Step*>(step);
    if (s->slot[slot].counted) { int64_t v = 0; (void)wisp_host_reader_wait(s->slot[slot].reader, &v); }
    return do_count(s, slot, origins, dirs, num_rays, seed, (hipStream_t)stream);
}

extern "C" int wisp_nerf_step_run(void* step, int slot, const float* gts, const float* next_origins, const float* next_dirs,
                                  int64_t next_num_rays, uint64_t next_seed, const wisp_nerf_step_hyper* hp,
                                  const float* level_cap_scale, void* hashgrid_workspace, int64_t hashgrid_workspace_bytes,
                                  int record_timing, int64_t* num_samples, int64_t* covered_rows, float** loss, wisp_stream_t stream) {
    WISP_REQUIRE(step && (slot == 0 || slot == 1) && gts && hp && num_samples && loss, "null argument");
    Step* s = static_cast<Step*>(step);
    const wisp_nerf_step_config& c = s->cfg;
    MarchSlot& m = s->slot[slot];
    WISP_REQUIRE(m.counted, "this slot holds no counted batch (wisp_nerf_step_count first)");
    WISP_REQUIRE(hp->struct_bytes == (int64_t)sizeof(wisp_nerf_step_hyper), "wisp_nerf_step_hyper has another size than this library's");
    hipStream_t st = (hipStream_t)stream;
    int64_t S = 0;
    int rc = wisp_host_reader_wait(m.reader, &S);
    m.counted = false;
    if (rc != WISP_OK) return rc;
    *num_samples = S;
    const int64_t R = m.num_rays;
    if (S > c.max_samples) return wisp_fail(WISP_ERR_CAPACITY, __func__, "more packed samples than the step was created for");
    if (S < 1) return wisp_fail(WISP_ERR_CAPACITY, __func__, "no sample survived the occupancy test");

    int64_t* ridx = at<int64_t>(s, s->lay.ridx);
    float* samples = at<float>(s, s->lay.samples);
    float* depth = at<float>(s, s->lay.depth);
    float* deltas = at<float>(s, s->lay.deltas);
    uint8_t* boundary = at<uint8_t>(s, s->lay.boundary);
    void* feats = at<void>(s, s->lay.feats);
    void* code = at<void>(s, s->lay.dir_code);
    float* color = at<float>(s, s->lay.color);
    float* density = at<float>(s, s->lay.density);
    float* g_color = at<float>(s, s->lay.g_color);
    float* g_density = at<float>(s, s->lay.g_density);
    void* g_feats = at<void>(s, s->lay.g_feats);
    float* loss_slot = at<float>(s, s->lay.loss) + s->loss_at;
    s->loss_at = (s->loss_at + 1) % NS_LOSS_RING;
    *loss = loss_slot;

    hipEvent_t* ev = nullptr;
    if (record_timing && s->timed_steps < NS_MAX_TIMED_STEPS &&
        s->ev.size() >= (size_t)(s->timed_steps + 1) * NS_STEP_EVENTS) {
        ev = s->ev.data() + (size_t)s->timed_steps * NS_STEP_EVENTS;
        s->ev_units[s->timed_steps] = S;
        ++s->timed_steps;
    }
#define NS_MARK(i) do { if (ev) (void)hipEventRecord(ev[i], st); } while (0)
#define NS_CALL(expr) do { rc = (expr); if (rc != WISP_OK) return rc; } while (0)

    void* image = wisp_nerf_mlp_operand_image_bytes(c.hidden) > 0 ? at<void>(s, s->lay.image) : nullptr;
    NS_CALL(wisp_raymarch_ray_emit_coded(m.origins, m.dirs, R, c.near, c.range, c.num_samples, nullptr, m.seed, m.hitmask, m.offsets,
                                         ridx, samples, depth, deltas, boundary, nullptr, c.view_freqs, code,
                                         image ? c.dec_params : nullptr, c.in_dim, c.hidden, image, st));
    if (next_origins) NS_CALL(do_count(s, slot ^ 1, next_origins, next_dirs, next_num_rays, next_seed, st));

    NS_MARK(0);
    NS_CALL(wisp_hashgrid_interpolate_fwd(samples, S, 3, c.table_lookup, c.dtype_table, c.feature_dim, c.first_idx, c.resolutions,
                                          c.num_lods, c.bitwidth, c.zero_from_col, feats, st));
    NS_MARK(1);
    if (image)
        NS_CALL(wisp_nerf_mlp_fwd_rays_img(feats, c.dtype_table, code, ridx, S, c.in_dim, c.hidden, c.view_freqs, c.dec_params, image, color,
                                           density, st));
    else
        NS_CALL(wisp_nerf_mlp_fwd_rays(feats, c.dtype_table, code, ridx, S, c.in_dim, c.hidden, c.view_freqs, c.dec_params, color, density, st));
    NS_MARK(2);
    const bool fold = hp->optimizer == 2 && c.table_param && c.table_exp_avg && c.table_exp_avg_sq;
    const bool tail_fold = fold && hp->tail_fold != 0;
    wisp_step_tail tail{};
    tail.in_dim = c.in_dim;
    float* comp_ws = at<float>(s, s->lay.comp_ws);
    float* mlp_ws = at<float>(s, s->lay.mlp_ws);
    if (tail_fold) {
        NS_CALL(wisp_composite_loss_partials(color, density, deltas, m.offsets, R, S, c.bg, gts, c.loss_kind, g_color, g_density, nullptr,
                                             comp_ws, s->lay.comp_ws_floats, &tail.loss_count, &tail.inv_n, st));
        tail.loss_partials = comp_ws;
        tail.loss = loss_slot;
    } else {
        NS_CALL(wisp_composite_loss(color, density, deltas, m.offsets, R, S, c.bg, gts, c.loss_kind, g_color, g_density, nullptr, loss_slot,
                                    comp_ws, s->lay.comp_ws_floats, st));
    }
    NS_MARK(3);
    if (tail_fold) {
        if (image)
            NS_CALL(wisp_nerf_mlp_bwd_rays_img_partials(feats, c.dtype_table, code, ridx, S, c.in_dim, c.hidden, c.view_freqs, c.dec_params, image,
                                                        g_color, g_density, g_feats, mlp_ws, s->lay.mlp_ws_bytes, &tail.dw_rows, st));
        else
            NS_CALL(wisp_nerf_mlp_bwd_rays_partials(feats, c.dtype_table, code, ridx, S, c.in_dim, c.hidden, c.view_freqs, c.dec_params, g_color,
                                                    g_density, g_feats, mlp_ws, s->lay.mlp_ws_bytes, &tail.dw_rows, st));
        tail.dw_partials = mlp_ws;
        tail.dec_grad = c.dec_grad;
    } else if (image) {
        NS_CALL(wisp_nerf_mlp_bwd_rays_img(feats, c.dtype_table, code, ridx, S, c.in_dim, c.hidden, c.view_freqs, c.dec_params, image, g_color,
                                           g_density, g_feats, c.dec_grad, mlp_ws, s->lay.mlp_ws_bytes, st));
    } else {
        NS_CALL(wisp_nerf_mlp_bwd_rays(feats, c.dtype_table, code, ridx, S, c.in_dim, c.hidden, c.view_freqs, c.dec_params, g_color, g_density,
                                       g_feats, c.dec_grad, mlp_ws, s->lay.mlp_ws_bytes, st));
    }
    int64_t covered[16] = {0};
    NS_MARK(4);
    if (tail_fold) {
        int tail_done = 0;
        NS_CALL(wisp_hashgrid_interpolate_bwd_adamw_tail(samples, S, 3, g_feats, c.dtype_table, c.feature_dim, c.first_idx, c.resolutions,
                                                         c.num_lods, c.bitwidth, c.zero_from_col, c.table_grad, hashgrid_workspace,
                                                         hashgrid_workspace_bytes, level_cap_scale, c.table_param, c.table_exp_avg,
                                                         c.table_exp_avg_sq, c.table_shadow, hp->lr_grid, hp->beta1, hp->beta2, hp->eps,
                                                         hp->weight_decay, hp->step, hp->grad_scale, covered, &tail, &tail_done, st));
        if (!tail_done) {
            NS_CALL(wisp_nerf_mlp_reduce_partials(tail.dw_partials, tail.dw_rows, tail.in_dim, tail.dec_grad, st));
            NS_CALL(wisp_loss_sum(tail.loss_partials, tail.loss_count, tail.inv_n, tail.loss, st));
        }
    } else if (fold)
        NS_CALL(wisp_hashgrid_interpolate_bwd_adamw(samples, S, 3, g_feats, c.dtype_table, c.feature_dim, c.first_idx, c.resolutions,
                                                    c.num_lods, c.bitwidth, c.zero_from_col, c.table_grad, hashgrid_workspace,
                                                    hashgrid_workspace_bytes, level_cap_scale, c.table_param, c.table_exp_avg,
                                                    c.table_exp_avg_sq, c.table_shadow, hp->lr_grid, hp->beta1, hp->beta2, hp->eps,
                                                    hp->weight_decay, hp->step, hp->grad_scale, covered, st));
    else
        NS_CALL(wisp_hashgrid_interpolate_bwd(samples, S, 3, g_feats, c.dtype_table, c.feature_dim, c.first_idx, c.resolutions, c.num_lods,
                                              c.bitwidth, c.zero_from_col, c.table_grad, hashgrid_workspace, hashgrid_workspace_bytes,
                                              level_cap_scale, st));
    NS_MARK(5);
    if (covered_rows)
        for (int l = 0; l < c.num_lods; ++l) covered_rows[l] = covered[l];

    if (hp->optimizer >= 1) {
        int64_t begin[24], len[24];
        float lr[24], wd[24];
        void* shadow[24];
        int n = 0;
        auto add = [&](int64_t b, int64_t l, float rate, void* sh) {
            if (l > 0 && n < 24) { begin[n] = b; len[n] = l; lr[n] = rate; wd[n] = hp->weight_decay; shadow[n] = sh; ++n; }
        };
        add(c.decoder_begin, c.decoder_len, hp->lr_decoder, nullptr);
        const int64_t ga = c.grid_begin, gb = c.grid_begin + c.grid_len;
        char* gsh = static_cast<char*>(c.grid_shadow);
        if (!fold) {
            add(ga, c.grid_len, hp->lr_grid, gsh);
        } else {
            int64_t at_ = ga;
            for (int l = 0; l < c.num_lods; ++l) {
                int64_t rows = covered[l];
                const int64_t have = s->first_idx_host[l + 1] - s->first_idx_host[l];
                if (rows > have) rows = have;
                if (rows <= 0) continue;
                const int64_t lo = c.table_offset + s->first_idx_host[l] * c.feature_dim;
                const int64_t hi = c.table_offset + (s->first_idx_host[l] + rows) * c.feature_dim;
                if (lo > at_) add(at_, lo - at_, hp->lr_grid, gsh ? gsh + (at_ - ga) * 2 : nullptr);
                if (hi > at_) at_ = hi;
            }
            if (gb > at_) add(at_, gb - at_, hp->lr_grid, gsh ? gsh + (at_ - ga) * 2 : nullptr);
        }
        add(c.rest_begin, c.rest_len, hp->lr_rest, nullptr);
        if (n > 0)
            NS_CALL(wisp_adamw_step_groups(c.flat_param, c.flat_grad, c.flat_exp_avg, c.flat_exp_avg_sq, n, begin, len, lr, wd, shadow,
                                           hp->beta1, hp->beta2, hp->eps, hp->step, hp->grad_scale, 1, st));
    }
#undef NS_MARK
#undef NS_CALL
    return WISP_OK;
}

extern "C" int wisp_nerf_step_read_timing(void* step, int max_steps, float* ms , int64_t* units ,
                                          int* num_steps ) {
    WISP_REQUIRE(step && ms && units && num_steps && max_steps >= 0, "null argument");
    Step* s = static_cast<Step*>(step);
    const int n = s->timed_steps < max_steps ? s->timed_steps : max_steps;
    for (int i = 0; i < n; ++i) {
        hipEvent_t* ev = s->ev.data() + (size_t)i * NS_STEP_EVENTS;
        for (int k = 0; k < NS_TIMED_KERNELS; ++k) {
            float t = 0.0f;
            const hipError_t e = hipEventElapsedTime(&t, ev[NS_EV_BEGIN[k]], ev[NS_EV_END[k]]);
            if (e != hipSuccess) return wisp_fail(WISP_ERR_LAUNCH, __func__, hipGetErrorString(e));
            ms[(size_t)i * NS_TIMED_KERNELS + k] = t;
        }
        units[i] = s->ev_units[i];
    }
    *num_steps = n;
    s->timed_steps = 0;
    return WISP_OK;
}
```

### kaolin-wisp_amd/wisp/_C.py

```python
import ctypes
import os

import numpy as np
import torch

_HERE = os.path.dirname(os.path.abspath(__file__))
LIB_PATH = os.environ.get("WISP_HIP_LIB") or os.path.normpath(os.path.join(_HERE, "..", "csrc", "libwisp_hip.so"))

if not os.path.exists(LIB_PATH):
    raise ImportError(
        f"wisp HIP extension not built: {LIB_PATH} is missing. Build it with "
        f"`make -C {os.path.dirname(LIB_PATH)}` (or `python -c 'import __graft_entry__ as g; g.build()'`). "
        "There is no CPU fallback for the hot path.")

lib = ctypes.CDLL(LIB_PATH)

F32, F16, BF16 = 0, 1, 2
_DTYPE_CODE = {torch.float32: F32, torch.float16: F16, torch.bfloat16: BF16}

c_vp, c_i64, c_i32, c_f32, c_u64 = ctypes.c_void_p, ctypes.c_int64, ctypes.c_int, ctypes.c_float, ctypes.c_uint64
c_f64 = ctypes.c_double

SIGNATURES = {
    "wisp_hashgrid_interpolate_fwd": [c_vp, c_i64, c_i32, c_vp, c_i32, c_i32, c_vp, c_vp, c_i32, c_i32, c_i32, c_vp, c_vp],
    "wisp_hashgrid_interpolate_bwd": [c_vp, c_i64, c_i32, c_vp, c_i32, c_i32, c_vp, c_vp, c_i32, c_i32, c_i32, c_vp, c_vp, c_i64, c_vp, c_vp],
    "wisp_hashgrid_interpolate_bwd_adamw": [c_vp, c_i64, c_i32, c_vp, c_i32, c_i32, c_vp, c_vp, c_i32, c_i32, c_i32, c_vp, c_vp, c_i64, c_vp,
                                            c_vp, c_vp, c_vp, c_vp, c_f32, c_f32, c_f32, c_f32, c_f32, c_i64, c_f32, c_vp, c_vp],
    "wisp_hashgrid_interpolate_bwd_adamw_tail": [c_vp, c_i64, c_i32, c_vp, c_i32, c_i32, c_vp, c_vp, c_i32, c_i32, c_i32, c_vp, c_vp, c_i64, c_vp,
                                                 c_vp, c_vp, c_vp, c_vp, c_f32, c_f32, c_f32, c_f32, c_f32, c_i64, c_f32, c_vp, c_vp, c_vp, c_vp],
    "wisp_hashgrid_grad_coords": [c_vp, c_i64, c_i32, c_vp, c_vp, c_i32, c_i32, c_vp, c_vp, c_i32, c_i32, c_vp, c_vp],
    "wisp_hashgrid_bwd_workspace_bytes": [c_i64, c_i32, c_i32, c_i32, c_vp, c_i32, c_i32, c_vp],
    "wisp_hashgrid_bwd_slot_stats": [c_i64, c_i32, c_i32, c_i32, c_vp, c_i32, c_i32, c_i32, c_vp, c_vp, c_i64, c_vp, c_vp, c_vp, c_vp],
    "wisp_hashgrid_cells": [c_vp, c_i64, c_i32, c_i32, c_i32, c_vp, c_vp, c_vp, c_vp],
    "wisp_hashgrid_query_fwd": [c_vp, c_i64, c_vp, c_i32, c_i32, c_vp, c_i32, c_i32, c_i32, c_vp, c_vp],
    "wisp_hashgrid_query_bwd": [c_vp, c_i64, c_vp, c_i32, c_i32, c_vp, c_i32, c_i32, c_i32, c_vp, c_vp],
    "wisp_spc_query": [c_vp, c_vp, c_vp, c_i64, c_i32, c_i32, c_vp, c_vp],
    "wisp_spc_query_chain": [c_vp, c_vp, c_vp, c_vp, c_i64, c_i32, c_i32, c_vp, c_i32, c_vp, c_vp],
    "wisp_spc_build_bitfield": [c_vp, c_i64, c_i32, c_vp, c_vp],
    "wisp_spc_raytrace_count": [c_vp, c_vp, c_vp, c_vp, c_vp, c_i64, c_i32, c_vp, c_vp, c_i32, c_vp],
    "wisp_spc_raytrace_emit": [c_vp, c_vp, c_vp, c_vp, c_vp, c_i64, c_i32, c_vp, c_i32, c_vp, c_i32, c_vp, c_vp, c_vp, c_vp],
    "wisp_spc_first_hit": [c_vp, c_vp, c_vp, c_vp, c_vp, c_i64, c_i32, c_vp, c_i32, c_i32, c_vp, c_vp, c_vp, c_vp, c_vp, c_vp],
    "wisp_spc_trilinear_coeffs": [c_vp, c_vp, c_i64, c_i32, c_i32, c_vp, c_vp],
    "wisp_spc_trilinear_fwd": [c_vp, c_vp, c_i32, c_vp, c_vp, c_vp, c_i32, c_i64, c_i32, c_i32, c_i32, c_i32, c_vp, c_vp],
    "wisp_spc_trilinear_bwd": [c_vp, c_vp, c_i32, c_vp, c_vp, c_vp, c_i64, c_i32, c_i32, c_i32, c_i64, c_vp, c_vp, c_i64, c_vp],
    "wisp_spc_bwd_workspace_bytes": [c_i64, c_i32, c_i64],
    "wisp_spc_trilinear_multi_fwd": [c_vp, c_vp, c_i64, c_vp, c_vp, c_vp, c_i32, c_i64, c_i32, c_vp, c_i32, c_i32, c_i32, c_vp, c_vp],
    "wisp_spc_trilinear_multi_bwd": [c_vp, c_vp, c_i64, c_vp, c_vp, c_vp, c_i64, c_i32, c_vp, c_vp, c_i32, c_i32, c_vp, c_vp, c_i64, c_vp],
    "wisp_triplane_fwd": [c_vp, c_i64, c_vp, c_vp, c_i32, c_i32, c_i32, c_vp, c_vp],
    "wisp_triplane_bwd": [c_vp, c_i64, c_vp, c_vp, c_i32, c_i32, c_i32, c_vp, c_vp],
    "wisp_codebook_trilinear_fwd": [c_vp, c_vp, c_i32, c_vp, c_vp, c_vp, c_vp, c_i64, c_i32, c_i32, c_i32, c_i32, c_i32, c_vp, c_vp],
    "wisp_codebook_decode_rows": [c_vp, c_vp, c_i64, c_i32, c_i32, c_i32, c_vp, c_vp],
    "wisp_codebook_trilinear_bwd": [c_vp, c_vp, c_i32, c_vp, c_vp, c_vp, c_vp, c_vp, c_i64, c_i32, c_i32, c_i32, c_i32, c_i64, c_vp, c_vp, c_vp, c_i64, c_vp],
    "wisp_codebook_trilinear_multi_bwd": [c_vp, c_vp, c_i64, c_vp, c_vp, c_vp, c_vp, c_vp, c_i64, c_i32, c_vp, c_vp, c_i32, c_i32, c_i32, c_vp, c_vp,
                                          c_vp, c_i64, c_vp],
    "wisp_mark_pack_boundaries_i64": [c_vp, c_i64, c_vp, c_vp],
    "wisp_mark_pack_boundaries_i32": [c_vp, c_i64, c_vp, c_vp],
    "wisp_scan_workspace_bytes": [c_i64],
    "wisp_exclusive_scan_i32": [c_vp, c_i64, c_vp, c_vp, c_vp],
    "wisp_inclusive_scan_i32": [c_vp, c_i64, c_vp, c_vp, c_vp],
    "wisp_boundary_tile_counts": [c_vp, c_i64, c_vp, c_vp],
    "wisp_boundary_pack_starts": [c_vp, c_i64, c_vp, c_vp, c_vp],
    "wisp_raymarch_ray_count": [c_vp, c_vp, c_vp, c_vp, c_vp, c_i64, c_f32, c_f32, c_i32, c_i32, c_vp, c_u64, c_vp, c_i32, c_vp, c_vp, c_vp],
    "wisp_raymarch_ray_emit": [c_vp, c_vp, c_i64, c_f32, c_f32, c_i32, c_vp, c_u64, c_vp, c_vp, c_vp, c_vp, c_vp, c_vp, c_vp, c_vp, c_vp],
    "wisp_raymarch_ray_emit_coded": [c_vp, c_vp, c_i64, c_f32, c_f32, c_i32, c_vp, c_u64, c_vp, c_vp, c_vp, c_vp, c_vp, c_vp, c_vp, c_vp, c_i32,
                                     c_vp, c_vp, c_i32, c_i32, c_vp, c_vp],
    "wisp_raymarch_voxel_emit": [c_vp, c_vp, c_vp, c_vp, c_i64, c_i32, c_vp, c_u64, c_vp, c_vp, c_vp, c_vp, c_vp, c_vp],
    "wisp_raymarch_uniform_count": [c_vp, c_i64, c_f32, c_vp, c_vp],
    "wisp_spc_mask_from_points": [c_vp, c_i64, c_i32, c_vp, c_vp],
    "wisp_spc_dense_bytes": [c_vp, c_i32, c_vp],
    "wisp_spc_points_from_index": [c_vp, c_i64, c_i32, c_vp, c_vp],
    "wisp_sdf_trace_step_fused": [c_i64, c_i32, c_vp, c_vp, c_vp, c_vp, c_f32, c_f32, c_f32, c_vp, c_vp, c_vp, c_vp, c_vp, c_vp, c_vp,
                                  c_vp, c_vp, c_vp, c_vp, c_vp, c_vp, c_vp, c_i32, c_vp, c_i32, c_i32, c_i32, c_vp, c_vp, c_vp,
                                  c_vp, c_i32, c_f32, c_vp, c_vp],
    "wisp_sdf_query": [c_vp, c_i64, c_vp, c_vp, c_vp, c_vp, c_vp, c_i32, c_vp, c_i32, c_i32, c_i32, c_vp, c_vp, c_vp, c_vp, c_i32, c_i32,
                       c_vp, c_vp, c_vp, c_vp],
    "wisp_sdf_fd_gradient": [c_vp, c_i64, c_vp, c_vp, c_vp, c_vp, c_vp, c_i32, c_vp, c_i32, c_i32, c_i32, c_vp, c_vp, c_vp, c_vp, c_i32,
                             c_i32, c_f32, c_vp, c_vp],
    "wisp_hash_sdf_query": [c_vp, c_i64, c_vp, c_i32, c_vp, c_vp, c_i32, c_i32, c_i32, c_i32, c_i32, c_vp, c_vp, c_vp, c_vp, c_i32,
                            c_vp, c_vp, c_vp, c_vp],
    "wisp_hash_sdf_fd_gradient": [c_vp, c_i64, c_vp, c_i32, c_vp, c_vp, c_i32, c_i32, c_i32, c_i32, c_i32, c_vp, c_vp, c_vp, c_vp, c_i32,
                                  c_f32, c_vp, c_vp],
    "wisp_hash_sdf_trace_step_fused": [c_i64, c_i32, c_vp, c_vp, c_vp, c_vp, c_f32, c_f32, c_f32, c_vp, c_vp, c_vp, c_vp, c_vp, c_vp, c_vp,
                                       c_vp, c_vp, c_vp, c_i32, c_vp, c_vp, c_i32, c_i32, c_i32, c_i32, c_i32, c_vp, c_vp, c_vp, c_vp, c_i32,
                                       c_f32, c_vp, c_vp],
    "wisp_triplane_sdf_query": [c_vp, c_i64, c_vp, c_vp, c_i32, c_i32, c_i32, c_vp, c_vp, c_vp, c_vp, c_i32, c_vp, c_vp, c_vp, c_vp],
    "wisp_triplane_sdf_fd_gradient": [c_vp, c_i64, c_vp, c_vp, c_i32, c_i32, c_i32, c_vp, c_vp, c_vp, c_vp, c_i32, c_f32, c_vp, c_vp],
    "wisp_triplane_sdf_trace_step_fused": [c_i64, c_i32, c_vp, c_vp, c_vp, c_vp, c_f32, c_f32, c_f32, c_vp, c_vp, c_vp, c_vp, c_vp, c_vp,
                                           c_vp, c_vp, c_vp, c_vp, c_vp, c_i32, c_i32, c_i32, c_vp, c_vp, c_vp, c_vp, c_i32, c_f32, c_vp,
                                           c_vp],
    "wisp_hash_sdf_train_scratch_bytes": [c_i64, c_i32, c_i32, c_i32, c_i32],
    "wisp_hash_sdf_train_step": [c_vp, c_vp, c_i64, c_vp, c_i32, c_vp, c_vp, c_i32, c_i32, c_i32, c_i32, c_i32, c_vp, c_vp, c_vp, c_vp, c_i32,
                                 c_vp, c_vp, c_vp, c_vp, c_vp, c_vp, c_vp, c_i64, c_vp],
    "wisp_triplane_sdf_train_scratch_bytes": [c_i64, c_vp, c_i32, c_i32, c_i32, c_i32],
    "wisp_triplane_sdf_train_step": [c_vp, c_vp, c_i64, c_vp, c_vp, c_i32, c_i32, c_i32, c_vp, c_vp, c_vp, c_vp, c_i32, c_vp, c_vp, c_vp,
                                     c_vp, c_vp, c_vp, c_vp, c_i64, c_vp],
    "wisp_sdf_train_scratch_bytes": [c_i64, c_i32, c_i32, c_i32],
    "wisp_sdf_train_step": [c_vp, c_vp, c_i64, c_vp, c_vp, c_vp, c_vp, c_vp, c_vp, c_vp, c_i32, c_i32, c_i32, c_vp, c_vp, c_vp, c_vp, c_i32,
                            c_vp, c_vp, c_vp, c_vp, c_vp, c_vp, c_vp, c_i64, c_vp, c_i64, c_vp],
    "wisp_sdf_tex_train_scratch_bytes": [c_i64, c_i32, c_i32, c_i32, c_i32],
    "wisp_sdf_tex_train_step": [c_vp, c_vp, c_vp, c_i64, c_vp, c_vp, c_vp, c_vp, c_vp, c_vp, c_vp, c_i32, c_i32, c_i32, c_i32, c_vp, c_vp,
                                c_vp, c_vp, c_i32, c_vp, c_vp, c_vp, c_vp, c_vp, c_vp, c_vp, c_i64, c_vp, c_i64, c_vp],
    "wisp_grid_interpolate_fwd": [c_vp, c_vp, c_i32, c_i64, c_i32, c_vp, c_vp],
    "wisp_grid_interpolate_bwd": [c_vp, c_vp, c_i32, c_i64, c_i32, c_vp, c_vp],
    "wisp_small_decoder_fwd": [c_vp, c_i64, c_i32, c_i32, c_vp, c_vp, c_vp, c_vp, c_vp, c_vp],
    "wisp_small_decoder_bwd": [c_vp, c_i64, c_i32, c_i32, c_vp, c_vp, c_vp, c_vp, c_vp, c_vp, c_vp, c_vp, c_vp, c_vp, c_vp],
    "wisp_uniform_sample": [c_i32, c_vp, c_vp, c_vp, c_i64, c_vp, c_vp, c_vp, c_vp],
    "wisp_raymarch_uniform_emit": [c_vp, c_vp, c_vp, c_vp, c_i64, c_f32, c_vp, c_vp, c_vp, c_vp, c_vp, c_vp, c_vp],
    "wisp_packed_sum_reduce": [c_vp, c_i64, c_i32, c_vp, c_i64, c_vp, c_vp],
    "wisp_packed_cumsum": [c_vp, c_i64, c_i32, c_vp, c_i64, c_i32, c_i32, c_vp, c_vp],
    "wisp_find_depth_bound": [c_vp, c_vp, c_vp, c_i64, c_i64, c_vp, c_vp],
    "wisp_sphere_trace_step": [c_i64, c_vp, c_vp, c_vp, c_vp, c_f32, c_f32, c_f32, c_vp, c_vp, c_vp, c_vp, c_vp, c_vp, c_vp, c_vp, c_vp, c_vp],
    "wisp_optim_step_groups": [c_i32, c_vp, c_vp, c_vp, c_vp, c_i32, c_vp, c_vp, c_vp, c_vp, c_vp, c_f32, c_f32, c_f32, c_i64, c_f32, c_i32, c_vp],
    "wisp_adamw_step_groups": [c_vp, c_vp, c_vp, c_vp, c_i32, c_vp, c_vp, c_vp, c_vp, c_vp, c_f32, c_f32, c_f32, c_i64, c_f32, c_i32, c_vp],
    "wisp_gather_rows": [c_vp, c_i64, c_i64, c_i32, c_vp, c_vp, c_vp, c_vp],
    "wisp_composite_loss": [c_vp, c_vp, c_vp, c_vp, c_i64, c_i64, c_vp, c_vp, c_i32, c_vp, c_vp, c_vp, c_vp, c_vp, c_i64, c_vp],
    "wisp_composite_loss_partials": [c_vp, c_vp, c_vp, c_vp, c_i64, c_i64, c_vp, c_vp, c_i32, c_vp, c_vp, c_vp, c_vp, c_i64, c_vp, c_vp, c_vp],
    "wisp_loss_sum": [c_vp, c_i32, c_f32, c_vp, c_vp],
    "wisp_rgb_loss": [c_vp, c_vp, c_i64, c_i32, c_vp, c_vp, c_vp, c_vp],
    "wisp_generate_rays": [c_vp, c_vp, c_i64, c_i32, c_f32, c_f32, c_f32, c_f32, c_f32, c_f32, c_vp, c_vp, c_vp, c_vp, c_vp],
    "wisp_composite_fwd": [c_vp, c_vp, c_vp, c_vp, c_vp, c_vp, c_i64, c_i64, c_i64, c_vp, c_vp, c_vp, c_vp, c_vp, c_vp, c_vp],
    "wisp_composite_bwd": [c_vp, c_vp, c_vp, c_vp, c_vp, c_vp, c_vp, c_vp, c_vp, c_i64, c_i64, c_vp, c_vp, c_vp, c_vp],
    "wisp_nerf_mlp_param_count": [c_i32, c_i32, c_i32],
    "wisp_nerf_mlp_fwd": [c_vp, c_i32, c_vp, c_i64, c_i32, c_i32, c_i32, c_vp, c_i32, c_vp, c_vp, c_vp],
    "wisp_nerf_mlp_bwd": [c_vp, c_i32, c_vp, c_i64, c_i32, c_i32, c_i32, c_vp, c_i32, c_vp, c_vp, c_vp, c_vp, c_vp, c_i64, c_vp],
    "wisp_nerf_prune_query": [c_vp, c_vp, c_i64, c_i32, c_vp, c_i32, c_i32, c_i32, c_vp, c_vp, c_i32, c_i32, c_i32, c_vp, c_i32, c_i32,
                              c_i32, c_vp, c_f32, c_f32, c_vp, c_vp, c_vp],
    "wisp_nerf_prune_query_debug": [c_vp, c_vp, c_i64, c_i32, c_vp, c_i32, c_i32, c_i32, c_vp, c_vp, c_i32, c_i32, c_i32, c_vp, c_i32,
                                    c_i32, c_i32, c_vp, c_f32, c_f32, c_vp, c_vp, c_vp, c_vp, c_vp],
    "wisp_nerf_query": [c_vp, c_vp, c_vp, c_i64, c_i64, c_vp, c_i32, c_i32, c_i32, c_vp, c_vp, c_i32, c_i32, c_i32, c_vp, c_i32, c_i32,
                        c_i32, c_vp, c_vp, c_vp],
    "wisp_nerf_mlp_dir_code": [c_vp, c_i64, c_i32, c_vp, c_vp],
    "wisp_nerf_mlp_operand_image_bytes": [c_i32],
    "wisp_nerf_mlp_build_operand_image": [c_vp, c_i32, c_i32, c_vp, c_vp],
    "wisp_nerf_mlp_fwd_rays_img": [c_vp, c_i32, c_vp, c_vp, c_i64, c_i32, c_i32, c_i32, c_vp, c_vp, c_vp, c_vp, c_vp],
    "wisp_nerf_mlp_bwd_rays_img": [c_vp, c_i32, c_vp, c_vp, c_i64, c_i32, c_i32, c_i32, c_vp, c_vp, c_vp, c_vp, c_vp, c_vp, c_vp, c_i64, c_vp],
    "wisp_nerf_mlp_fwd_rays": [c_vp, c_i32, c_vp, c_vp, c_i64, c_i32, c_i32, c_i32, c_vp, c_vp, c_vp, c_vp],
    "wisp_nerf_mlp_bwd_rays": [c_vp, c_i32, c_vp, c_vp, c_i64, c_i32, c_i32, c_i32, c_vp, c_vp, c_vp, c_vp, c_vp, c_vp, c_i64, c_vp],
    "wisp_nerf_mlp_bwd_rays_partials": [c_vp, c_i32, c_vp, c_vp, c_i64, c_i32, c_i32, c_i32, c_vp, c_vp, c_vp, c_vp, c_vp, c_i64, c_vp, c_vp],
    "wisp_nerf_mlp_bwd_rays_img_partials": [c_vp, c_i32, c_vp, c_vp, c_i64, c_i32, c_i32, c_i32, c_vp, c_vp, c_vp, c_vp, c_vp, c_vp, c_i64, c_vp, c_vp],
    "wisp_nerf_mlp_reduce_partials": [c_vp, c_i32, c_i32, c_vp, c_vp],
    "wisp_nerf_mlp_bwd_workspace_bytes": [c_i64, c_i32],
    "wisp_nerf_mlp_workspace_floats": [],
    "wisp_adamw_step": [c_vp, c_vp, c_vp, c_vp, c_i64, c_f32, c_f32, c_f32, c_f32, c_f32, c_i64, c_f32, c_i32, c_vp, c_vp],
    "wisp_host_reader_create": [],
    "wisp_host_reader_issue": [c_vp, c_vp, c_vp],
    "wisp_host_reader_wait": [c_vp, c_vp],
    "wisp_host_reader_destroy": [c_vp],
    "wisp_nerf_step_config_bytes": [],
    "wisp_nerf_step_workspace_bytes": [c_vp],
    "wisp_nerf_step_create": [c_vp, c_vp, c_i64],
    "wisp_nerf_step_reconfigure": [c_vp, c_vp],
    "wisp_nerf_step_destroy": [c_vp],
    "wisp_nerf_step_count": [c_vp, c_i32, c_vp, c_vp, c_i64, c_u64, c_vp],
    "wisp_nerf_step_run": [c_vp, c_i32, c_vp, c_vp, c_vp, c_i64, c_u64, c_vp, c_vp, c_vp, c_i64, c_i32, c_vp, c_vp, c_vp, c_vp],
    "wisp_nerf_step_read_timing": [c_vp, c_i32, c_vp, c_vp, c_vp],
    "wisp_mesh_to_sdf": [c_vp, c_i64, c_vp, c_i64, c_i32, c_i64, c_vp, c_vp, c_i64, c_vp],
    "wisp_mesh_to_sdf_triangle": [c_vp, c_i64, c_vp, c_i64, c_i32, c_i64, c_vp, c_vp, c_i64, c_vp],
    "wisp_mesh_sdf_workspace_bytes": [c_i64, c_i64],
    "wisp_mesh_closest_tex": [c_vp, c_i64, c_vp, c_i64, c_vp, c_i32, c_vp, c_i64, c_vp, c_vp, c_i64, c_vp, c_i32, c_vp, c_vp, c_vp],
    "wisp_mesh_sample_tex": [c_vp, c_vp, c_i64, c_vp, c_i64, c_vp, c_i32, c_vp, c_vp],
    "wisp_multiview_sample": [c_vp, c_vp, c_vp, c_i64, c_i32, c_i32, c_i32, c_i32, c_vp, c_vp, c_i64, c_i64, c_f32, c_f32, c_f32, c_f32,
                              c_vp, c_vp, c_vp, c_vp, c_vp, c_vp],
    "wisp_image_sample": [c_vp, c_i32, c_i32, c_vp, c_i64, c_vp, c_vp, c_vp],
    "wisp_image_field_render": [c_vp, c_i64, c_i64, c_i32, c_i32, c_vp, c_vp, c_vp, c_i32, c_i32, c_i32, c_vp, c_i32, c_vp, c_vp, c_vp,
                                c_vp, c_vp],
    "wisp_image_field_render_partials": [c_i64],
    "wisp_image_field_train_scratch_bytes": [c_i64, c_i32, c_i32],
    "wisp_image_field_train_step": [c_vp, c_vp, c_i64, c_vp, c_vp, c_vp, c_i32, c_i32, c_i32, c_vp, c_vp, c_vp, c_vp, c_i32, c_vp, c_vp, c_vp,
                                    c_vp, c_vp, c_vp, c_vp, c_vp, c_i64, c_vp],
    "wisp_ssim_scratch_bytes": [c_i32, c_i32, c_i32],
    "wisp_ssim": [c_vp, c_i64, c_i64, c_vp, c_i64, c_i64, c_i32, c_i32, c_i32, c_i32, c_vp, c_f64, c_f64, c_f64, c_vp, c_vp, c_vp, c_i64, c_vp],
    "wisp_last_error": [],
    "wisp_abi_version": [],
}
_RESTYPES = {"wisp_ssim_scratch_bytes": c_i64, "wisp_image_field_render_partials": c_i64, "wisp_image_field_train_scratch_bytes": c_i64, "wisp_mesh_sdf_workspace_bytes": c_i64, "wisp_nerf_mlp_bwd_workspace_bytes": c_i64, "wisp_spc_bwd_workspace_bytes": c_i64, "wisp_sdf_train_scratch_bytes": c_i64, "wisp_sdf_tex_train_scratch_bytes": c_i64, "wisp_hash_sdf_train_scratch_bytes": c_i64, "wisp_triplane_sdf_train_scratch_bytes": c_i64, "wisp_hashgrid_bwd_workspace_bytes": c_i64, "wisp_scan_workspace_bytes": c_i64, "wisp_nerf_mlp_param_count": c_i64, "wisp_nerf_mlp_workspace_floats": c_i64,
             "wisp_last_error": ctypes.c_char_p, "wisp_host_reader_create": c_vp, "wisp_host_reader_destroy": None,
             "wisp_nerf_step_config_bytes": c_i64, "wisp_nerf_step_workspace_bytes": c_i64, "wisp_nerf_step_create": c_vp,
             "wisp_nerf_step_destroy": None}

for _name, _args in SIGNATURES.items():
    _fn = getattr(lib, _name)
    _fn.argtypes = _args
    _fn.restype = _RESTYPES.get(_name, c_i32)

ABI_VERSION = 4
if lib.wisp_abi_version() != ABI_VERSION:
    raise ImportError(f"{LIB_PATH} implements ABI version {lib.wisp_abi_version()}, this binding is written for version "
                      f"{ABI_VERSION}: rebuild the library (make -C {os.path.dirname(LIB_PATH)})")


WISP_ERR_CAPACITY = -4


class NerfStepConfig(ctypes.Structure):
    _fields_ = ([("struct_bytes", c_i64)]
                + [(n, c_vp) for n in ("occ_bits", "octree", "exsum", "coarse_bits", "table_lookup", "first_idx", "first_idx_host",
                                       "resolutions", "table_param", "table_grad", "table_exp_avg", "table_exp_avg_sq", "table_shadow",
                                       "dec_params", "dec_grad", "flat_param", "flat_grad", "flat_exp_avg", "flat_exp_avg_sq",
                                       "grid_shadow")]
                + [(n, c_i64) for n in ("decoder_begin", "decoder_len", "grid_begin", "grid_len", "rest_begin", "rest_len", "table_offset",
                                        "max_rays", "max_samples")]
                + [(n, c_i32) for n in ("level", "coarse_level", "num_samples", "loss_kind", "dtype_table", "num_lods", "feature_dim",
                                        "bitwidth", "zero_from_col", "in_dim", "hidden", "view_freqs")]
                + [("near", c_f32), ("range", c_f32), ("bg", c_f32 * 3), ("reserved", c_f32)])


class NerfStepHyper(ctypes.Structure):
    _fields_ = ([("struct_bytes", c_i64), ("step", c_i64)]
                + [(n, c_f32) for n in ("lr_decoder", "lr_grid", "lr_rest", "weight_decay", "beta1", "beta2", "eps", "grad_scale")]
                + [("optimizer", c_i32), ("tail_fold", c_i32)])


class StepTail(ctypes.Structure):
    _fields_ = ([(n, c_vp) for n in ("dw_partials", "dec_grad", "loss_partials", "loss")]
                + [(n, c_i32) for n in ("dw_rows", "in_dim", "loss_count")] + [("inv_n", c_f32)])


if ctypes.sizeof(NerfStepConfig) != lib.wisp_nerf_step_config_bytes():
    raise ImportError(f"wisp_nerf_step_config: this binding lays it out in {ctypes.sizeof(NerfStepConfig)} bytes, {LIB_PATH} in "
                      f"{lib.wisp_nerf_step_config_bytes()}: rebuild the library")


TIMING = None
TIMING_ALL = None
_cdll = lib


class _LibProxy:

    def __getattr__(self, name):
        fn = getattr(_cdll, name)
        sig = SIGNATURES.get(name)
        if not sig or sig[-1] is not c_vp or name.endswith("_bytes") or name.endswith("_count") and "raymarch" not in name and "raytrace" not in name:
            setattr(self, name, fn)
            return fn

# ... 105 lines not shown


def _host_res(resolutions):
    key = resolutions if type(resolutions) is tuple else tuple(int(r) for r in resolutions)
    hit = _res_cache.get(key)
    if hit is None:
        arr, ptr = _host_i32(key)
        hit = _res_cache[key] = (key, arr, ptr)
    return hit


def _host_f32(values):
    arr = np.ascontiguousarray(np.asarray(values, dtype=np.float32).reshape(-1))
    return arr, arr.ctypes.data_as(c_vp)


_first_idx_ok = {}


def _check_first_idx(first_idx, num_lods, rows):
    if first_idx.numel() < num_lods + 1:
        raise RuntimeError(f"codebook_first_idx must hold num_lods + 1 = {num_lods + 1} offsets, got {first_idx.numel()}")
    key = (first_idx.data_ptr(), first_idx._version, num_lods, rows)
    if key not in _first_idx_ok:
        if len(_first_idx_ok) > 64:
            _first_idx_ok.clear()
        host = [int(v) for v in first_idx[:num_lods + 1].tolist()]
        if host[num_lods] > rows:
            raise RuntimeError(f"codebook_first_idx[{num_lods}] = {host[num_lods]} exceeds the {rows} rows of the table")
        _first_idx_ok[key] = host
    return _first_idx_ok[key]


def hashgrid_interpolate(coords, codebook, first_idx, resolutions, codebook_bitwidth, zero_from_col=None):
    coords = _need(coords, torch.float32, "coords")
    codebook = _need(codebook, None, "codebook")
    first_idx = _need(first_idx, torch.int64, "codebook_first_idx")
    n, dim = coords.shape
    L, F = len(resolutions), codebook.shape[1]
    _check_first_idx(first_idx, L, codebook.shape[0])
    if zero_from_col is None:
        zero_from_col = L * F
    _, res_arr, res_ptr = _host_res(resolutions)
    feats = torch.empty(n, L * F, dtype=codebook.dtype, device=coords.device)
    with _timed("hashgrid_fwd", n):
        _check(lib.wisp_hashgrid_interpolate_fwd(_p(coords), n, dim, _p(codebook), _DTYPE_CODE[codebook.dtype], F,
                                                 _p(first_idx), res_ptr, L, codebook_bitwidth, zero_from_col, _p(feats),
                                                 _stream()), "hashgrid_interpolate_fwd")
    return feats


def hashgrid_interpolate_backward(coords, grad_feats, codebook_shape, first_idx, resolutions, codebook_bitwidth,
                                  zero_from_col=None, out=None, adamw=None):
    coords = _need(coords, torch.float32, "coords")
    grad_feats = _need(grad_feats, None, "grad_feats")
    first_idx = _need(first_idx, torch.int64, "codebook_first_idx")
    n, dim = coords.shape
    L, F = len(resolutions), codebook_shape[1]
    first_host = _check_first_idx(first_idx, L, codebook_shape[0])
    if zero_from_col is None:
        zero_from_col = L * F
    res_key, res_arr, res_ptr = _host_res(resolutions)
    grad = out if out is not None else torch.zeros(tuple(codebook_shape), dtype=torch.float32, device=coords.device)
    assert grad.dtype == torch.float32 and grad.is_contiguous()
    dt = _DTYPE_CODE[grad_feats.dtype]
    fit = _slot_fit(coords.device, dim, dt, F, res_key, codebook_bitwidth, zero_from_col, n >= HASHGRID_EMIT_WIDE_MIN) if n >= 4096 else None
    scale_arr, scale_ptr = fit.scales(n) if fit is not None else (None, None)
    ws_bytes = int(lib.wisp_hashgrid_bwd_workspace_bytes(n, dim, dt, F, res_ptr, L, codebook_bitwidth, scale_ptr))
    ws = _bwd_workspace(coords.device, ws_bytes) if 0 < ws_bytes <= HASHGRID_BWD_WORKSPACE_LIMIT else None
    covered = None
    with _timed("hashgrid_bwd", n):
        if adamw is None:
            _check(lib.wisp_hashgrid_interpolate_bwd(_p(coords), n, dim, _p(grad_feats), dt, F,
                                                     _p(first_idx), res_ptr, L, codebook_bitwidth, zero_from_col, _p(grad),
                                                     _p(ws), ws.numel() if ws is not None else 0, scale_ptr, _stream()),
                   "hashgrid_interpolate_bwd")
        else:
            assert out is not None, "the fused update leaves the uncovered rows' gradient in `out`"
            prm, m1, m2, sh = adamw["param"], adamw["exp_avg"], adamw["exp_avg_sq"], adamw.get("shadow")
            for t in (prm, m1, m2):
                assert t.is_cuda and t.dtype == torch.float32 and t.is_contiguous() and t.numel() == grad.numel()
            assert sh is None or (sh.dtype == torch.bfloat16 and sh.is_contiguous() and sh.numel() == grad.numel())
            cov = (ctypes.c_int64 * L)()
            _check(lib.wisp_hashgrid_interpolate_bwd_adamw(_p(coords), n, dim, _p(grad_feats), dt, F,
                                                           _p(first_idx), res_ptr, L, codebook_bitwidth, zero_from_col, _p(grad),
                                                           _p(ws), ws.numel() if ws is not None else 0, scale_ptr,
                                                           _p(prm), _p(m1), _p(m2), _p(sh), float(adamw["lr"]), float(adamw["beta1"]),
                                                           float(adamw["beta2"]), float(adamw["eps"]), float(adamw["weight_decay"]),
                                                           int(adamw["step"]), float(adamw.get("grad_scale", 1.0)),
                                                           ctypes.cast(cov, ctypes.c_void_p), _stream()),
                   "hashgrid_interpolate_bwd_adamw")
            covered = [min(int(c), first_host[l + 1] - first_host[l]) for l, c in enumerate(cov)]
    if fit is not None and ws is not None:
        fit.after_launch(n, res_ptr, scale_arr, scale_ptr, ws, ws_bytes)
    return grad if adamw is None else (grad, covered)


def hashgrid_grad_coords(coords, grad_feats, codebook, first_idx, resolutions, codebook_bitwidth):
    coords = _need(coords, torch.float32, "coords")
    codebook = _need(codebook, None, "codebook")
    if grad_feats.dtype != codebook.dtype:
        grad_feats = grad_feats.to(codebook.dtype)
    grad_feats = _need(grad_feats, None, "grad_feats")
    first_idx = _need(first_idx, torch.int64, "codebook_first_idx")
    n, dim = coords.shape
    L, F = len(resolutions), codebook.shape[1]
    _check_first_idx(first_idx, L, codebook.shape[0])
    if grad_feats.shape != (n, L * F):
        raise ValueError(f"grad_feats must be [{n}, {L * F}], got {tuple(grad_feats.shape)}")
    res_arr, res_ptr = _host_i32(resolutions)
    out = torch.empty(n, 3, dtype=torch.float32, device=coords.device)
    _check(lib.wisp_hashgrid_grad_coords(_p(coords), n, dim, _p(grad_feats), _p(codebook), _DTYPE_CODE[codebook.dtype], F,
                                         _p(first_idx), res_ptr, L, int(codebook_bitwidth), _p(out), _stream()), "hashgrid_grad_coords")
    return out


HASHGRID_BWD_WORKSPACE_LIMIT = 24 << 30
_bwd_ws = {}
_slot_fits = {}
SLOT_FIT_ENABLED = os.environ.get("WISP_HG_SLOT_FIT", "1") != "0"


class _SlotFit:
    CHECK_EVERY, HEADROOM, GROW, FLOOR, ADOPT_AFTER = 32, float(os.environ.get("WISP_HG_SLOT_HEADROOM", "1.2")), 1.6, 0.02, 8

    def __init__(self, device, dim, dt, F, res, bitwidth, zero_from_col):
        self.key = (dim, dt, F, res, bitwidth, zero_from_col)
        self.L = len(res)
        self.scale = [1.0] * self.L
        self.calls = 0
        self.pending = None
        self.last = None
        self.dev_fill = torch.zeros(2 * self.L, dtype=torch.int32, device=device)
        self.host_fill = torch.zeros(2 * self.L, dtype=torch.int32).pin_memory()
        self._scale_c = None

    def scales(self, n):
        self._collect()
        if self._scale_c is None or self._scale_c[2] != self.scale:
            arr = (ctypes.c_float * self.L)(*self.scale)
            self._scale_c = (arr, ctypes.cast(arr, ctypes.c_void_p), list(self.scale))
        return self._scale_c[0], self._scale_c[1]

    def _collect(self):
        p = self.pending
        if p is None:
            return
        if self.calls - p["at"] < self.ADOPT_AFTER:
            return
        p["event"].synchronize()
        self.pending = None
        both = self.host_fill.tolist()
        fill, written = both[:self.L], both[self.L:]
        for l in range(self.L):
            cap, base = p["cap"][l], p["base"][l]
            if base <= 0:
                continue
            if fill[l] >= cap:
                self.scale[l] = min(1.0, max(self.scale[l], cap / base) * self.GROW)
            else:
                self.scale[l] = min(1.0, max(self.FLOOR, self.HEADROOM * fill[l] / base))
        self.last = dict(fill=fill, records=written, cap=list(p["cap"]), base=list(p["base"]), scale=list(self.scale),
                         workspace_bytes=p["ws_bytes"])

    def after_launch(self, n, res_ptr, scale_arr, scale_ptr, ws, ws_bytes):
        self.calls += 1
        if self.pending is not None or (self.calls - 1) % self.CHECK_EVERY:
            return
        dim, dt, F, res, bitwidth, zero_from_col = self.key
        cap = (ctypes.c_int32 * self.L)()
        base = (ctypes.c_int32 * self.L)()
        rc = lib.wisp_hashgrid_bwd_slot_stats(n, dim, dt, F, res_ptr, self.L, bitwidth, zero_from_col, scale_ptr, _p(ws), ws.numel(),
                                              _p(self.dev_fill), ctypes.cast(cap, ctypes.c_void_p), ctypes.cast(base, ctypes.c_void_p),
                                              _stream())
        if rc < 0:
            _check(rc, "hashgrid_bwd_slot_stats")
        if rc != 0:
            return
        self.host_fill.copy_(self.dev_fill, non_blocking=True)
        ev = torch.cuda.Event()
        ev.record()
        self.pending = dict(event=ev, cap=list(cap), base=list(base), ws_bytes=int(ws_bytes), at=self.calls)


HASHGRID_EMIT_WIDE_MIN = 1 << 20


def _slot_fit(device, dim, dt, F, res, bitwidth, zero_from_col, wide=False):
    if not SLOT_FIT_ENABLED:
        return None
    key = (device, _stream().value, dim, dt, F, res, bitwidth, zero_from_col, bool(wide))
    fit = _slot_fits.get(key)
    if fit is None:
        fit = _slot_fits[key] = _SlotFit(device, dim, dt, F, res, bitwidth, zero_from_col)
    return fit


def hashgrid_cells(coords, resolution, codebook_bitwidth, with_corners=True):
    coords = _need(coords, torch.float32, "coords")
# ... 1709 lines not shown
```

### kaolin-wisp_amd/wisp/trainers/_native_step.py

```python
import ctypes
import os

import numpy as np
import torch

ENABLED = os.environ.get("WISP_NATIVE_STEP", "1") != "0"
TAIL_FOLD = os.environ.get("WISP_STEP_TAIL_FOLD", "1") != "0"


def _hip():
    import wisp._C as C
    return C


class _Elapsed:
    __slots__ = ("ms",)

    def __init__(self, ms):
        self.ms = ms

    def elapsed_time(self, _other):
        return self.ms


class NativeHashStep:
    TIMED = ("hashgrid_fwd", "nerf_mlp_fwd", "nerf_mlp_bwd", "hashgrid_bwd")

    def __init__(self, trainer):
        self.t = trainer
        self.handle = None
        self.key = None
        self.shape = None
        self.keep = None
        self.pending = None
        self.next_slot = 0
        self.hg_ws = None
        self.hg_scale = None
        self.fallbacks = 0
        self.steps = 0

    def applies(self, rays, jitter):
        t = self.t
        d = t._direct
        C = _hip()
        if not ENABLED or d is None or not d.hash_fast or not t.enable_amp or d.biasless or jitter is not None:
            return False
        if t.optimizer != 'adamw' or t.world > 1 or t.force_allreduce or getattr(t, "grad_accum_steps", 1) > 1:
            return False
        if t.comm_timing is not None or C.TIMING_ALL is not None:
            return False
        cls = type(t)
        from wisp.trainers.multiview_trainer import MultiviewTrainStep, FUSED_COMPOSITE_LOSS
        if not FUSED_COMPOSITE_LOSS or 'optimizer_step' in t.__dict__ or cls.optimizer_step is not MultiviewTrainStep.optimizer_step \
                or cls.reduce_and_update is not MultiviewTrainStep.reduce_and_update:
            return False
        pipe = t.pipeline
        tracer, grid = pipe.tracer, pipe.nef.grid
        i, h, f = d.shape
        if tracer.raymarch_type != 'ray' or h != 64 or f != 4 or i != len(d.res) * 2 or i > 32 or d.table.shape[1] != 2:
            return False
        if t.rgb_loss_type not in ('huber', 'l2', 'l1') or not rays.origins.is_cuda or rays.origins.dtype != torch.float32:
            return False
        if torch.is_tensor(rays.dist_min) or torch.is_tensor(rays.dist_max):
            return False
        if not C.nerf_mlp_rays_preferred(torch.bfloat16, i, h, f, True):
            return False
        blas = grid.blas
        return blas.max_level <= 10 and rays.origins.shape[0] <= t.max_rays and rays.origins.is_contiguous() and rays.dirs.is_contiguous()

    def _capacity(self):
        t = self.t
        return int(t.max_rays), int(max(2 * t.target_sample_size, 1 << 17))

    def _ensure(self, rays):
        C = _hip()
        t, d = self.t, self.t._direct
        from wisp.ops.grid import current_shadow
        pipe = t.pipeline
        tracer, grid = pipe.tracer, pipe.nef.grid
        blas = grid.blas
        dev = rays.origins.device
        blas._to_device(dev)
        f = t.flat
        shadow = current_shadow(d.table, torch.bfloat16)
        if shadow is None:
            return False
        packed, packed_grad = d._params()
        max_rays, max_samples = self._capacity()
        near, far = float(rays.dist_min), float(rays.dist_max)
        key = (id(blas), blas.octree.data_ptr(), near, far, tracer.num_steps, d.table.data_ptr(), shadow.data_ptr(), f.data.data_ptr(),
               f.grad.data_ptr(), packed.data_ptr(), packed_grad.data_ptr(), max_rays, max_samples, t.rgb_loss_type,
               tuple(float(v) for v in tracer._bg_host()), torch.cuda.current_stream().cuda_stream)
        if self.handle is not None and key == self.key:
            return True
        level = blas.max_level
        occ = blas._bitfield(level)
        if occ is None:
            return False
        coarse, lc = blas._coarse_bitfield(rays, tracer.num_steps, level)
        L = len(d.res)
        first_host = (ctypes.c_int64 * (L + 1))(*[int(v) for v in d._first_idx_host[:L + 1]])
        res = (ctypes.c_int32 * L)(*d.res)
        off = next(o for p, o in f._grid_params if p is d.table)
        n = d.table.numel()
        ga, gb = f.ranges["grid"]
        da, db = f.ranges["decoder"]
        ra, rb = f.ranges["rest"]
        cfg = C.NerfStepConfig()
        cfg.struct_bytes = ctypes.sizeof(C.NerfStepConfig)
        P = lambda x: None if x is None else x.data_ptr()
        cfg.occ_bits, cfg.octree, cfg.exsum, cfg.coarse_bits = P(occ), P(blas.octree), P(blas.prefix), P(coarse)
        cfg.table_lookup, cfg.first_idx = P(shadow), P(d.first_idx)
        cfg.first_idx_host, cfg.resolutions = ctypes.cast(first_host, ctypes.c_void_p), ctypes.cast(res, ctypes.c_void_p)
        cfg.table_param, cfg.table_grad = P(d.table), P(d.table.grad)
        cfg.table_exp_avg, cfg.table_exp_avg_sq = f.exp_avg.data_ptr() + 4 * off, f.exp_avg_sq.data_ptr() + 4 * off
        cfg.table_shadow = None if f.shadow is None else f.shadow.data_ptr() + 2 * (off - ga)
        cfg.dec_params, cfg.dec_grad = P(packed), P(packed_grad)
        cfg.flat_param, cfg.flat_grad, cfg.flat_exp_avg, cfg.flat_exp_avg_sq = P(f.data), P(f.grad), P(f.exp_avg), P(f.exp_avg_sq)
        cfg.grid_shadow = P(f.shadow)
        cfg.decoder_begin, cfg.decoder_len, cfg.grid_begin, cfg.grid_len, cfg.rest_begin, cfg.rest_len = da, db - da, ga, gb - ga, ra, rb - ra
        cfg.table_offset, cfg.max_rays, cfg.max_samples = off, max_rays, max_samples
        cfg.level, cfg.coarse_level, cfg.num_samples = level, int(lc), int(tracer.num_steps)
        cfg.loss_kind = {"huber": 0, "l2": 1, "l1": 2}[t.rgb_loss_type]
        cfg.dtype_table, cfg.num_lods, cfg.feature_dim, cfg.bitwidth = C.BF16, L, 2, int(d.bitwidth)
        i, h, fq = d.shape
        cfg.zero_from_col, cfg.in_dim, cfg.hidden, cfg.view_freqs = int(d.zero_from_col), i, h, fq
        cfg.near = float(np.float32(near))
        cfg.range = float(np.float32(far - near))
        bg = tracer._bg_host()
        cfg.bg[0], cfg.bg[1], cfg.bg[2] = float(bg[0]), float(bg[1]), float(bg[2])
        shape = (max_rays, max_samples, int(tracer.num_steps), L, dev, torch.cuda.current_stream().cuda_stream)
        if self.handle is not None and shape == self.shape and C.lib.wisp_nerf_step_reconfigure(self.handle, ctypes.byref(cfg)) == 0:
            ws = self.keep[0]
        else:
            self.close()
            need = int(C.lib.wisp_nerf_step_workspace_bytes(ctypes.byref(cfg)))
            if need <= 0:
                raise RuntimeError(f"wisp_nerf_step_workspace_bytes: {C.last_error()}")
            ws = torch.empty(need, dtype=torch.uint8, device=dev)
            self.handle = C.lib.wisp_nerf_step_create(ctypes.byref(cfg), ws.data_ptr(), need)
            if not self.handle:
                self.handle = None
                raise RuntimeError(f"wisp_nerf_step_create: {C.last_error()}")
            self.loss_view = {}
        self.key, self.shape = key, shape
        self.keep = (ws, first_host, res, occ, coarse, shadow, packed, packed_grad, blas, cfg)
        self.blas = blas
        if self.pending is not None:
            self.pending["slot"] = None
        return True

    def close(self):
        if self.handle is not None:
            _hip().lib.wisp_nerf_step_destroy(self.handle)
            self.handle, self.key, self.keep, self.shape = None, None, None, None

    def __del__(self):
        try:
            self.close()
        except Exception:
            pass

    def _hyper(self):
        C = _hip()
        t = self.t
        step = t.opt_steps + 1
        s = t._lr_scale(step)
        hp = C.NerfStepHyper()
        hp.struct_bytes = ctypes.sizeof(C.NerfStepHyper)
        hp.step = step
        hp.lr_decoder = t.lr * s
        hp.lr_grid = t.lr * t.grid_lr_weight * s
        hp.lr_rest = t.lr * s
        hp.weight_decay, hp.beta1, hp.beta2, hp.eps = t.weight_decay, t.betas[0], t.betas[1], t.eps
        hp.grad_scale = 1.0 / t.world
        hp.optimizer = 2 if t.fuse_grid_optimizer else 1
        hp.tail_fold = 1 if TAIL_FOLD else 0
        return hp

    def _hashgrid_scratch(self, dev, n_guess):
        C = _hip()
        d = self.t._direct
        res_key, res_arr, res_ptr = C._host_res(d.res)
        fit = C._slot_fit(dev, 3, C.BF16, 2, res_key, d.bitwidth, d.zero_from_col, n_guess >= C.HASHGRID_EMIT_WIDE_MIN) if n_guess >= 4096 else None
        scale_arr, scale_ptr = fit.scales(n_guess) if fit is not None else (None, None)
        if self.hg_ws is None or self.hg_scale is not scale_arr:
            _, max_samples = self._capacity()
            need = max(int(C.lib.wisp_hashgrid_bwd_workspace_bytes(n, 3, C.BF16, 2, res_ptr, len(d.res), d.bitwidth, scale_ptr))
                       for n in (max_samples, min(max_samples, C.HASHGRID_EMIT_WIDE_MIN - 1), max(4096, int(1.3 * n_guess))))
            if self.hg_ws is None or self.hg_ws.numel() < need or self.hg_ws.numel() > 3 * need + (64 << 20):
                self.hg_ws = None
                self.hg_ws = torch.empty(need + 256, dtype=torch.uint8, device=dev)
            self.hg_scale = scale_arr
        return fit, res_ptr, scale_arr, scale_ptr

    def step(self, rays, img_gts, prefetch):
        C = _hip()
        t, d = self.t, self.t._direct
        if not self._ensure(rays):
            return None
        lib, h = C.lib, self.handle
        dev = rays.origins.device
        stream = C._stream()
        blas = self.blas
        p, self.pending = self.pending, None
        if p is None or p["rays"] is not rays:
            st, d._pending = d._pending, None
            seed = st["seed"] if (st is not None and st.get("rays") is rays) else blas._draw_seed()
            slot = self.next_slot
        elif p["slot"] is None or p["blas"] is not blas:
            seed, slot = p["seed"], self.next_slot
        else:
            seed, slot = p["seed"], p["slot"]
            p = "counted"
        if p != "counted":
            C._check(lib.wisp_nerf_step_count(h, slot, rays.origins.data_ptr(), rays.dirs.data_ptr(), rays.origins.shape[0], seed, stream),
                     "nerf_step_count")
        self.next_slot = slot ^ 1
        gts = img_gts if (img_gts.dtype == torch.float32 and img_gts.is_contiguous()) else img_gts.float().contiguous()
        nxt = None
        if prefetch is not None and self.applies(prefetch, None) and float(prefetch.dist_min) == float(rays.dist_min) \
                and float(prefetch.dist_max) == float(rays.dist_max):
            nxt = dict(rays=prefetch, slot=slot ^ 1, seed=blas._draw_seed(), blas=blas)
        guess = t.pipeline.tracer.get_prev_num_samples() or t.target_sample_size
        fit, res_ptr, scale_arr, scale_ptr = self._hashgrid_scratch(dev, int(guess))
        hp = self._hyper()
        S = ctypes.c_int64(0)
        cov = (ctypes.c_int64 * 16)()
        loss_ptr = ctypes.c_void_p()
        record = 1 if C.TIMING is not None else 0
        t.wait_for_parameters()
        rc = lib.wisp_nerf_step_run(h, slot, gts.data_ptr(),
                                    None if nxt is None else nxt["rays"].origins.data_ptr(), None if nxt is None else nxt["rays"].dirs.data_ptr(),
                                    0 if nxt is None else nxt["rays"].origins.shape[0], 0 if nxt is None else nxt["seed"],
                                    ctypes.byref(hp), scale_ptr, self.hg_ws.data_ptr(), self.hg_ws.numel(), record,
                                    ctypes.byref(S), ctypes.cast(cov, ctypes.c_void_p), ctypes.byref(loss_ptr), stream)
        if rc == C.WISP_ERR_CAPACITY:
            self.fallbacks += 1
            d._pending = d._count(rays, None, seed=seed)
            d._next_seed = None if nxt is None else nxt["seed"]
            return None
        C._check(rc, "nerf_step_run")
        self.pending = nxt
        self.steps += 1
        n = int(S.value)
        t.pipeline.tracer.prev_num_samples = n
        t.opt_steps += 1
        if hp.optimizer == 2:
            L = len(d.res)
            first = d._first_idx_host
            cover = [min(int(cov[l]), first[l + 1] - first[l]) for l in range(L)]
            ga, gb = t.flat.ranges["grid"]
            t.fused_elements_last = 2 * sum(max(0, c) for c in cover)
            self.covered_last = cover
        else:
            t.fused_elements_last = 0
        t.flat.mark_shadow_current()
        if fit is not None:
            ws_bytes = self.hg_ws.numel()
            if fit.pending is None and fit.calls % fit.CHECK_EVERY == 0:
                ws_bytes = int(C.lib.wisp_hashgrid_bwd_workspace_bytes(n, 3, C.BF16, 2, res_ptr, len(d.res), d.bitwidth, scale_ptr))
            fit.after_launch(n, res_ptr, scale_arr, scale_ptr, self.hg_ws, ws_bytes)
        addr = loss_ptr.value
        view = self.loss_view.get(addr)
        if view is None:
            ws = self.keep[0]
            o = addr - ws.data_ptr()
            view = self.loss_view[addr] = ws[o:o + 4].view(torch.float32)
        return view, n

    def drain_timing(self, sink):
        if self.handle is None or sink is None:
            return
        C = _hip()
        cap = 2048
        ms = (ctypes.c_float * (4 * cap))()
        units = (ctypes.c_int64 * cap)()
        n = ctypes.c_int32(0)
        C._check(C.lib.wisp_nerf_step_read_timing(self.handle, cap, ctypes.cast(ms, ctypes.c_void_p), ctypes.cast(units, ctypes.c_void_p),
                                                  ctypes.byref(n)), "nerf_step_read_timing")
        for i in range(int(n.value)):
            for k, name in enumerate(self.TIMED):
                sink.setdefault(name, []).append((_Elapsed(float(ms[4 * i + k])), None, int(units[i])))
```

### kaolin-wisp_amd/wisp/trainers/multiview_trainer.py

```python
import logging as log
import math
import os
import weakref
from dataclasses import dataclass
from typing import Optional

import numpy as np
import torch
import torch.distributed as dist

from wisp.core import Rays
from wisp.ops.grid import current_shadow, mark_shadow_current, register_table_aux
from wisp.trainers.base_trainer import BaseTrainer, ConfigBaseTrainer


def _hip():
    import wisp._C as _C
    return _C


def _range_push(msg):
    torch.cuda.nvtx.range_push(msg)


# ... 629 lines not shown
                                   "fp32 master of other ranks' slices is stale; call sync_master() on every rank, then "
                                   "flat.refresh_shadow(), before the next step")

    def sync_master(self):
        if not self._master_stale:
            return
        self.wait_for_parameters()
        plan = self._plan
        f = self.flat
        self._gather_grid(f.data[plan["ga"]:plan["gb"]], plan, "fp32")
        f.mark_shadow_current()
        self._master_stale = False

    def wait_for_parameters(self):
        ev = self._params_ready
        if ev is not None:
            if self.comm_timing:
                here = torch.cuda.Event(enable_timing=True)
                here.record()
                self.comm_timing[-1]["waited_at"] = here
            torch.cuda.current_stream().wait_event(ev)
            self._params_ready = None

    def comm_summary(self):
        rows = [r for r in (self.comm_timing or []) if r["waited_at"] is not None]
        if not rows:
            return None
        n = len(rows)
        phases = {}
        for r in rows:
            prev = r["start"]
            for label, ev in r["marks"]:
                phases[label] = phases.get(label, 0.0) + prev.elapsed_time(ev)
                prev = ev
        total = sum(r["start"].elapsed_time(r["done"]) for r in rows) / n
        exposed = sum(max(0.0, r["waited_at"].elapsed_time(r["done"])) for r in rows) / n
        out = dict(steps=n, side_stream_ms=total, exposed_wait_ms=exposed, hidden_ms=max(0.0, total - exposed),
                   path="reduce-scatter + sharded optimizer + all-gather" if self.sharded_optimizer else "all-reduce + replicated optimizer")
        for label, v in phases.items():
            out[label + "_ms"] = v / n
        out["collective_ms"] = sum(v for k, v in phases.items() if k != "optimizer") / n
        return out

    def pre_step(self):
        if self.prune_every > -1 and self.total_iterations > 1 and self.total_iterations % self.prune_every == 0:
            self.prune()

    def prune(self):
        self.wait_for_parameters()
        nef = self.pipeline.nef
        if (getattr(nef, 'prune_density_decay', None) is None or getattr(nef, 'prune_min_density', None) is None
                or getattr(nef.grid, 'dense_points', None) is None or not hasattr(nef, 'prune')):
            return
        self.sync_master()
        cells = nef.grid.dense_points.shape[0]
        dev = self._prune_gen.device
        unit = torch.rand(cells, 3, generator=self._prune_gen, device=dev)
        views = torch.randn(cells, 3, generator=self._prune_gen, device=dev)
        if not (hasattr(nef, 'prune_fused') and nef.prune_fused()):
            views = torch.nn.functional.normalize(views, dim=1)
        nef.prune(unit_samples=unit, view_dirs=views)

    def calc_adaptive_rays(self, num_rays_in_batch):
        spr = self.pipeline.tracer.get_prev_num_samples() / max(num_rays_in_batch, 1)
        n = self.target_sample_size / max(spr, 1)
        self.num_rays = int(math.floor(min(n, self.max_rays)))
        return self.num_rays

    def loss_fn(self, rgb, gts):
        if self.rgb_loss_type == 'l2':
            return torch.nn.functional.mse_loss(rgb, gts, reduction='none').mean()
        if self.rgb_loss_type == 'l1':
            return torch.abs(rgb - gts).mean()
        if self.rgb_loss_type == 'huber':
            return torch.nn.functional.smooth_l1_loss(rgb, gts, reduction='none').mean()
        raise NotImplementedError

    def native_timing_into(self, sink):
        if self._native is not None:
            self._native.drain_timing(sink)

    def accumulate(self, rays: Rays, img_gts, jitter=None):
        assert self.grad_accum_steps > 1, "set grad_accum_steps to the number of micro-batches per optimizer step first"
        self._refuse_stale_master_forward()
        if self._direct is not None and self.pipeline.nef.training:
            with torch.no_grad():
                loss, _ = self._direct.run(rays, img_gts, jitter, None, fused_update=None)
        else:
            self.wait_for_parameters()
            kw = {} if jitter is None else {"jitter": jitter}
            with torch.autocast('cuda', dtype=torch.bfloat16, enabled=self.enable_amp):
                rb = self.pipeline(rays=rays, lod_idx=None, channels=["rgb"], **kw)
                loss = self.loss_fn(rb.rgb.float(), img_gts)
            loss.backward()
        return loss.detach(), self.pipeline.tracer.get_prev_num_samples()

    def step(self, rays: Rays, img_gts, jitter=None, prefetch: Optional[Rays] = None):
        _range_push("MultiviewTrainer.step")
        try:
            self.pre_step()
            self._refuse_stale_master_forward()
            self.total_iterations += 1
            self._fused_cover = None
            self._last_step_modular = not (self._direct is not None and self.pipeline.nef.training)
            done = None
            if not self._last_step_modular and self._native is not None and self._native.applies(rays, jitter):
                done = self._native.step(rays, img_gts, prefetch)
            if done is not None:
                loss = done[0]
                self.calc_adaptive_rays(rays.origins.shape[0])
                return loss, done[1]
            if not self._last_step_modular:
                with torch.no_grad():
                    loss, _ = self._direct.run(rays, img_gts, jitter, prefetch, fused_update=self._fused_update_args())
            else:
                self.wait_for_parameters()
                kw = {} if jitter is None else {"jitter": jitter}
                with torch.autocast('cuda', dtype=torch.bfloat16, enabled=self.enable_amp):
                    rb = self.pipeline(rays=rays, lod_idx=None, channels=["rgb"], **kw)
                    loss = self.loss_fn(rb.rgb.float(), img_gts)
                _range_push("MultiviewTrainer.backward")
                try:
                    loss.backward()
                finally:
                    _range_pop()
            self.reduce_and_update()
            self.calc_adaptive_rays(rays.origins.shape[0])
        finally:
            _range_pop()
        return loss.detach(), self.pipeline.tracer.get_prev_num_samples()


EVAL_FUSED_QUERY = True


@dataclass
class ConfigMultiviewTrainer(ConfigBaseTrainer):
    start_prune: int = 1000
    prune_every: int = 100
    random_lod: bool = False
    rgb_lambda: float = 1.0
    opacity_loss: float = 0.0
    rgb_loss_type: str = 'l2'
    rgb_loss_denom: str = 'rays'
    target_sample_size: int = 2 ** 18
    save_valid_imgs: bool = False


class MultiviewTrainer(BaseTrainer):

    def __init__(self, cfg, pipeline, train_dataset, validation_dataset=None, tracker=None, device='cuda', scene_state=None):
        super().__init__(cfg=cfg, pipeline=pipeline, train_dataset=train_dataset, tracker=tracker, device=device,
                         scene_state=scene_state)
        self.validation_dataset = validation_dataset

    def pre_step(self):
        super().pre_step()
        every = self.cfg.prune_every
        if every > -1 and self.total_iterations > 1 and self.total_iterations % every == 0:
            self.pipeline.nef.prune()

    def calc_adaptive_rays(self, rays, warmup=False):
        pipe = self.pipeline
        if warmup:
            marched = pipe.nef.grid.raymarch(rays, level=pipe.nef.grid.active_lods[-1], num_samples=pipe.tracer.num_steps,
                                             raymarch_type=pipe.tracer.raymarch_type)
            pipe.tracer.prev_num_samples = marched.samples.shape[0]
        per_ray = pipe.tracer.get_prev_num_samples() / rays.shape[0]
        num_rays = int(math.floor(min(self.cfg.target_sample_size / max(per_ray, 1), 2 ** 18)))
        transform = getattr(self.train_dataset, 'transform', None)
        if not hasattr(transform, 'set_num_samples') or type(transform).__name__ != 'SampleRays':
            raise Exception("SampleRays should be used as the transform for the dataset")
        transform.set_num_samples(num_rays)

    def step(self, data):
        _range_push("MultiviewTrainer.step")
        try:
            return self._step(data)
        finally:
            _range_pop()

    def _step(self, data):
        rays = data['rays'].to(self.device).squeeze(0)
        img_gts = data['rgb'].to(self.device).squeeze(0)
        tracer = self.pipeline.tracer
        if tracer.get_prev_num_samples() is None:
            self.calc_adaptive_rays(rays, warmup=True)
            return
        self.optimizer.zero_grad()
        lod_idx = None
        if self.cfg.random_lod:
            import random
            lods = self.pipeline.nef.grid.num_lods
            total = float(sum(2 ** i for i in range(lods)))
# ... 125 lines not shown
```

Before: 15.19 million.

## Skip reading hash-grid gradient buffer in fused Adam flush when known clean

Adds a grad-clean flag so the fused AdamW flush in the hashgrid backward reduce can skip loading the dense gradient buffer when no emit block spilled direct atomic writes into it and the previous step left it zeroed. Spill state is tracked with a dirty bit packed into the count and max words, and is OR-reduced across tiles and waves. Python tracks cleanliness across native steps and marks it dirty on fallback or rebuild. This saves one float2 load stream per entry in the flush, at the cost of extra bookkeeping, atomics, and the risk of wrong gradients if the cleanliness invariant is broken.

New measurement: 15.39 million, median of 6. 1.01x the previous value.

```diff
diff --git a/include/wisp_hip.h b/include/wisp_hip.h
--- a/include/wisp_hip.h
+++ b/include/wisp_hip.h
@@ -72,6 +72,18 @@
                                              void* bf16_shadow, float lr, float beta1, float beta2, float eps, float weight_decay,
                                              int64_t step, float grad_scale, int64_t* covered_rows ,
                                              const wisp_step_tail* tail, int* tail_done , wisp_stream_t stream);
+
+#define WISP_HG_BWD_GRAD_CLEAN 1u
+int wisp_hashgrid_interpolate_bwd_adamw_flags(const float* coords, int64_t n, int coord_dim,
+                                              const void* grad_feats, int dtype, int feature_dim,
+                                              const int64_t* first_idx, const int32_t* resolutions, int num_lods,
+                                              int codebook_bitwidth, int zero_from_col,
+                                              float* grad_codebook, void* workspace, int64_t workspace_bytes,
+                                              const float* level_cap_scale, float* param, float* exp_avg, float* exp_avg_sq,
+                                              void* bf16_shadow, float lr, float beta1, float beta2, float eps, float weight_decay,
+                                              int64_t step, float grad_scale, int64_t* covered_rows ,
+                                              const wisp_step_tail* tail , int* tail_done ,
+                                              uint32_t flags, wisp_stream_t stream);
 
 int wisp_hashgrid_cells(const float* coords, int64_t n, int coord_dim, int32_t resolution, int codebook_bitwidth,
                         int32_t* cell, float* frac, int32_t* corner_idx, wisp_stream_t stream);
@@ -482,6 +494,7 @@
                        int64_t next_num_rays, uint64_t next_seed, const wisp_nerf_step_hyper* hp,
                        const float* level_cap_scale, void* hashgrid_workspace, int64_t hashgrid_workspace_bytes,
                        int record_timing, int64_t* num_samples, int64_t* covered_rows, float** loss, wisp_stream_t stream);
+int wisp_nerf_step_grad_clean(void* step);
 int wisp_nerf_step_read_timing(void* step, int max_steps, float* ms, int64_t* units, int* num_steps);
 
 int wisp_mesh_to_sdf(const double* points, int64_t n, const double* mesh, int64_t f, int triangle_ranges,
diff --git a/kaolin-wisp_amd/csrc/hashgrid.hip b/kaolin-wisp_amd/csrc/hashgrid.hip
--- a/kaolin-wisp_amd/csrc/hashgrid.hip
+++ b/kaolin-wisp_amd/csrc/hashgrid.hip
@@ -1,5 +1,6 @@
 #include "wisp_common.h"
 #include <stdlib.h>
+#include <type_traits>
 
 #include "hashgrid_dev.h"
 #include "step_tail_dev.h"
@@ -291,6 +292,9 @@
 #define HG_FLUSH_PAIRS 1
 #endif
 
+#define HG_DIRTY_BIT 0x80000000u
+#define HG_WORD_MASK 0x7fffffffu
+
 template <typename T, int F> struct RecordCodec {
     static constexpr bool COMPACT = (sizeof(T) == 2 && F == 2);
     static constexpr int RW = COMPACT ? 2 : 1 + F;
@@ -339,8 +343,9 @@
     uint32_t* s_rank = em_smem;
     uint32_t* s_mx = em_smem + total_ranks;
     uint32_t* s_grad = em_smem + total_ranks + 1;
+    __shared__ uint32_t s_spill;
     uint32_t mx = 0;
-    if (threadIdx.x == 0) *s_mx = 0;
+    if (threadIdx.x == 0) { *s_mx = 0; s_spill = 0; }
     const int row_dw = num_lods * W;
     const int rowp = row_dw | 1;
     const int lane = threadIdx.x & 63;
@@ -405,6 +410,7 @@
                     uint32_t* dst = rec_l + (size_t)((b * bucket_stride + slot0 + pos[j]) * RW);
                     mx = max(mx, Codec::store(dst, loc, v[j]));
                 } else {
+                    if (idx >= owned) atomicOr(&s_spill, HG_DIRTY_BIT);
                     const int64_t row = first_idx[l] + (int64_t)idx;
                     if (row < total_rows) {
                         float* p = grad_codebook + row * F;
@@ -417,7 +423,7 @@
     }
     if (mx) atomicMax(s_mx, mx);
     __syncthreads();
-    if (threadIdx.x == 0) counts[bins.max_base + blockIdx.x] = *s_mx;
+    if (threadIdx.x == 0) counts[bins.max_base + blockIdx.x] = *s_mx | s_spill;
     for (int li = 0; li < levels.n; ++li) {
         const int chunks = bins.chunks[li];
         const uint32_t cap = bins.cap[li];
@@ -425,7 +431,7 @@
         uint32_t* __restrict__ cnt_l = counts + bins.cnt_base[li];
         for (int b = threadIdx.x; b < chunks; b += EM_THREADS) {
             const uint32_t cn = rank_l[b];
-            cnt_l[(size_t)b * ntiles + blockIdx.x] = cn < cap ? cn : cap;
+            cnt_l[(size_t)b * ntiles + blockIdx.x] = cn <= cap ? cn : (cap | HG_DIRTY_BIT);
         }
     }
 }
@@ -448,8 +454,9 @@
     const int total_ranks = bins.rank_base[levels.n];
     uint32_t* s_rank = em_smem;
     uint32_t* s_mx = em_smem + total_ranks;
+    __shared__ uint32_t s_spill;
     uint32_t mx = 0;
-    if (threadIdx.x == 0) *s_mx = 0;
+    if (threadIdx.x == 0) { *s_mx = 0; s_spill = 0; }
     const int lane = threadIdx.x & 63;
     const int wave = threadIdx.x >> 6;
     uint32_t* s_queue = em_smem + ((total_ranks + 4) & ~3) + wave * (64 * QROW);
@@ -532,6 +539,7 @@
                             uint32_t* dst = rec_l + (size_t)((b * bucket_stride + slot0 + pos) * RW);
                             mx = max(mx, Codec::store(dst, loc, val));
                         } else {
+                            if (idx >= owned) atomicOr(&s_spill, HG_DIRTY_BIT);
                             const int64_t row = base_l + (int64_t)idx;
                             if (row < total_rows) {
                                 float* pg = grad_codebook + row * F;
@@ -548,7 +556,7 @@
     }
     if (mx) atomicMax(s_mx, mx);
     __syncthreads();
-    if (threadIdx.x == 0) counts[bins.max_base + blockIdx.x] = *s_mx;
+    if (threadIdx.x == 0) counts[bins.max_base + blockIdx.x] = *s_mx | s_spill;
     for (int li = 0; li < levels.n; ++li) {
         const int chunks = bins.chunks[li];
         const uint32_t cap = bins.cap[li];
@@ -556,7 +564,7 @@
         uint32_t* __restrict__ cnt_l = counts + bins.cnt_base[li];
         for (int b = threadIdx.x; b < chunks; b += THREADS) {
             const uint32_t cn = rank_l[b];
-            cnt_l[(size_t)b * ntiles + blockIdx.x] = cn < cap ? cn : cap;
+            cnt_l[(size_t)b * ntiles + blockIdx.x] = cn <= cap ? cn : (cap | HG_DIRTY_BIT);
         }
     }
 }
@@ -602,6 +610,7 @@
 struct AdamFlush {
     float* p; float* m; float* v; __hip_bfloat16* shadow;
     float lr, wd, b1, b2, eps, bc1, bc2_sqrt, gscale;
+    int grad_clean;
 };
 #define HG_TAIL_ROWS 8192
 #define WISP_WHOLE_LEVEL ((int64_t)1 << 62)
@@ -618,7 +627,7 @@
 hashgrid_bwd_reduce_body(const ACC A, const int64_t* __restrict__ first_idx, const LevelList& levels, int chunk_shift,
                          const BinLevels& bins, uint32_t ntiles, const uint32_t* __restrict__ counts,
                          const uint32_t* __restrict__ records, float* __restrict__ grad_codebook, int li, int b, int z,
-                         const AdamFlush& ad) {
+                         const AdamFlush& ad, bool may_skip_grad, uint32_t* s_wave_flag) {
     typedef RecordCodec<T, F> Codec;
     constexpr int RW = Codec::RW;
     const int splits = bins.splits[li];
@@ -647,9 +656,12 @@
     constexpr int NW = RD_THREADS / 64;
     constexpr int INFLIGHT = 8;
     const uint32_t my_tiles = ntiles > (uint32_t)z ? (ntiles - z + splits - 1) / splits : 0u;
+    uint32_t seen = 0;
     for (uint32_t base = 0; base * NW + wave < my_tiles; base += 64) {
         const uint32_t k = (base + lane) * NW + wave;
-        const uint32_t cnt_of_lane = k < my_tiles ? cnt[z + k * splits] : 0u;
+        const uint32_t cnt_word = k < my_tiles ? cnt[z + k * splits] : 0u;
+        seen |= cnt_word;
+        const uint32_t cnt_of_lane = cnt_word & HG_WORD_MASK;
         const uint32_t cc = (cnt_of_lane + 63u) >> 6;
         uint32_t inc = cc;
 #pragma unroll
@@ -691,7 +703,22 @@
             }
         }
     }
+    bool need_grad = true;
+    if constexpr (ADAM) {
+        if (may_skip_grad && splits == 1) {
+            const bool overflowed = __ballot((seen & HG_DIRTY_BIT) != 0) != 0ull;
+            if (lane == 0) s_wave_flag[wave] = overflowed ? 1u : 0u;
+        }
+    }
     __syncthreads();
+    if constexpr (ADAM) {
+        if (may_skip_grad && splits == 1) {
+            uint32_t any = 0;
+#pragma unroll
+            for (int w = 0; w < NW; ++w) any |= s_wave_flag[w];
+            need_grad = any != 0;
+        }
+    }
     if (strips) {
         float* __restrict__ dl = grad_codebook + first_idx[l] * F;
         if constexpr (ADAM) {
@@ -718,6 +745,8 @@
                     }
                     return;
                 }
+                auto flush = [&](auto with_grad) {
+                constexpr bool WITH_GRAD = decltype(with_grad)::value;
                 for (uint32_t i0 = threadIdx.x; i0 < pairs; i0 += PQ * RD_THREADS) {
                     float2 cg[PQ], cp[PQ], cm[PQ], cv[PQ];
                     uint32_t row[PQ];
@@ -725,7 +754,10 @@
                     for (int q = 0; q < PQ; ++q) {
                         const uint32_t i = i0 + q * RD_THREADS;
                         row[q] = i < pairs ? bucket_row((uint32_t)b, i, chunk_shift, magic, nbuckets, rot_mask) : 0xffffffffu;
-                        if (row[q] < entries) { cg[q] = pg[row[q]]; cp[q] = pp[row[q]]; cm[q] = pm[row[q]]; cv[q] = pv[row[q]]; }
+                        if (row[q] < entries) {
+                            if constexpr (WITH_GRAD) cg[q] = pg[row[q]]; else cg[q] = make_float2(0.0f, 0.0f);
+                            cp[q] = pp[row[q]]; cm[q] = pm[row[q]]; cv[q] = pv[row[q]];
+                        }
                     }
 #pragma unroll
                     for (int q = 0; q < PQ; ++q) {
@@ -746,6 +778,8 @@
                         }
                     }
                 }
+                };
+                if (need_grad) flush(std::true_type{}); else flush(std::false_type{});
                 return;
             }
         }
@@ -791,13 +825,16 @@
             constexpr int PQ = 4;
             const uint32_t pairs = lim >> 1;
             if ((lim & 1u) == 0 && (((uintptr_t)dst | (uintptr_t)pp | (uintptr_t)pm | (uintptr_t)pv) & 7u) == 0) {
+                auto flush = [&](auto with_grad) {
+                constexpr bool WITH_GRAD = decltype(with_grad)::value;
                 for (uint32_t i0 = threadIdx.x; i0 < pairs; i0 += PQ * RD_THREADS) {
                     float2 cg[PQ], cp[PQ], cm[PQ], cv[PQ];
 #pragma unroll
                     for (int q = 0; q < PQ; ++q) {
                         const uint32_t i = i0 + q * RD_THREADS;
                         if (i < pairs) {
-                            cg[q] = reinterpret_cast<const float2*>(dst)[i]; cp[q] = reinterpret_cast<const float2*>(pp)[i];
+                            if constexpr (WITH_GRAD) cg[q] = reinterpret_cast<const float2*>(dst)[i]; else cg[q] = make_float2(0.0f, 0.0f);
+                            cp[q] = reinterpret_cast<const float2*>(pp)[i];
                             cm[q] = reinterpret_cast<const float2*>(pm)[i]; cv[q] = reinterpret_cast<const float2*>(pv)[i];
                         }
                     }
@@ -820,6 +857,8 @@
                         }
                     }
                 }
+                };
+                if (need_grad) flush(std::true_type{}); else flush(std::false_type{});
             } else {
                 for (uint32_t e = threadIdx.x; e < lim; e += RD_THREADS) {
                     const float c = dst[e];
@@ -923,25 +962,29 @@
     const int splits = bins.splits[li];
     const int local = bid - bins.blk_base[li];
     const int b = local / splits, z = local - b * splits;
-    uint32_t m = 0;
-    for (uint32_t t = threadIdx.x; t < ntiles; t += RD_THREADS) m = max(m, counts[bins.max_base + t]);
+    uint32_t m = 0, spill = 0;
+    for (uint32_t t = threadIdx.x; t < ntiles; t += RD_THREADS) { const uint32_t mw = counts[bins.max_base + t]; m = max(m, mw & HG_WORD_MASK); spill |= mw; }
 #pragma unroll
     for (int d = 32; d >= 1; d >>= 1) m = max(m, (uint32_t)__shfl_xor((int)m, d, 64));
+    if (__ballot((spill & HG_DIRTY_BIT) != 0) != 0ull) m |= HG_DIRTY_BIT;
     if ((threadIdx.x & 63) == 0) s_wave_max[threadIdx.x >> 6] = m;
     __syncthreads();
-    m = s_wave_max[0];
-#pragma unroll
-    for (int w = 1; w < RD_THREADS / 64; ++w) m = max(m, s_wave_max[w]);
+    m = 0; spill = 0;
+#pragma unroll
+    for (int w = 0; w < RD_THREADS / 64; ++w) { const uint32_t x = s_wave_max[w]; m = max(m, x & HG_WORD_MASK); spill |= x & HG_DIRTY_BIT; }
+    const bool may_skip_grad = ADAM && ad.grad_clean != 0 && spill == 0;
     const int e = (int)(m >> 23);
     if (e < 255) {
         int sh = 165 - e - extra_bits;
         if (sh > 159) sh = 159;
         AccFix64 A{reinterpret_cast<unsigned long long*>(rd_smem), __uint_as_float((uint32_t)(sh - 32 + 127) << 23),
                    __longlong_as_double((long long)(1023 - sh) << 52)};
-        hashgrid_bwd_reduce_body<T, F, AccFix64, ADAM>(A, first_idx, levels, chunk_shift, bins, ntiles, counts, records, grad_codebook, li, b, z, ad);
+        hashgrid_bwd_reduce_body<T, F, AccFix64, ADAM>(A, first_idx, levels, chunk_shift, bins, ntiles, counts, records, grad_codebook, li, b, z, ad,
+                                                       may_skip_grad, s_wave_max);
     } else {
         AccF32 A{reinterpret_cast<float*>(rd_smem)};
-        hashgrid_bwd_reduce_body<T, F, AccF32, ADAM>(A, first_idx, levels, chunk_shift, bins, ntiles, counts, records, grad_codebook, li, b, z, ad);
+        hashgrid_bwd_reduce_body<T, F, AccF32, ADAM>(A, first_idx, levels, chunk_shift, bins, ntiles, counts, records, grad_codebook, li, b, z, ad,
+                                                     may_skip_grad, s_wave_max);
     }
 }
 
@@ -998,6 +1041,11 @@
 }
 
 static int64_t coarse_level_wgs(int64_t n) { return n >= ((int64_t)1 << 21) ? 64 : 16; }
+
+static bool grad_clean_honoured() {
+    const char* e = getenv("WISP_HG_GRAD_CLEAN");
+    return !(e && e[0] == '0');
+}
 
 struct BinPlan { int chunk_shift, max_chunks, max_splits, total_blocks, total_ranks, emit_threads ; int64_t ntiles; BinLevels bins; int64_t count_bytes, record_bytes; bool ok;
                  uint32_t base_cap[HG_MAX_LODS]; };
@@ -1278,7 +1326,7 @@
                           int64_t workspace_bytes, const float* level_cap_scale, float* param,
                           float* exp_avg, float* exp_avg_sq, void* bf16_shadow, float lr, float beta1,
                           float beta2, float eps, float weight_decay, int64_t step, float grad_scale,
-                          int64_t* covered_rows, const StepTail* side_jobs, int* side_done,
+                          int64_t* covered_rows, const StepTail* side_jobs, int* side_done, uint32_t flags,
                           wisp_stream_t stream) {
     WISP_REQUIRE(n >= 0, "negative n");
     WISP_REQUIRE(num_lods >= 1 && num_lods <= HG_MAX_LODS, "num_lods out of range");
@@ -1293,7 +1341,8 @@
     const int64_t tsize = (int64_t)1 << codebook_bitwidth;
     WISP_REQUIRE(fill_levels(resolutions, num_lods, coord_dim, tsize, lv) == 0, "bad resolution");
     const AdamFlush ad{param, exp_avg, exp_avg_sq, (__hip_bfloat16*)bf16_shadow, lr, weight_decay, beta1, beta2, eps,
-                       1.0f - powf(beta1, (float)step), sqrtf(1.0f - powf(beta2, (float)step)), grad_scale};
+                       1.0f - powf(beta1, (float)step), sqrtf(1.0f - powf(beta2, (float)step)), grad_scale,
+                       (flags & WISP_HG_BWD_GRAD_CLEAN) != 0 && grad_clean_honoured() ? 1 : 0};
     hipStream_t s = (hipStream_t)stream;
     HG_DISPATCH(launch_bwd, coords, n, grad_feats, first_idx, lv, num_lods, (uint32_t)tsize, zero_from_col,
                 grad_codebook, workspace, workspace_bytes, level_cap_scale, s, &ad, covered_rows, side_jobs, side_done)
@@ -1311,7 +1360,7 @@
                                                    int64_t* covered_rows, wisp_stream_t stream) {
     return bwd_adamw_impl(coords, n, coord_dim, grad_feats, dtype, feature_dim, first_idx, resolutions, num_lods, codebook_bitwidth,
                           zero_from_col, grad_codebook, workspace, workspace_bytes, level_cap_scale, param, exp_avg, exp_avg_sq, bf16_shadow,
-                          lr, beta1, beta2, eps, weight_decay, step, grad_scale, covered_rows, nullptr, nullptr, stream);
+                          lr, beta1, beta2, eps, weight_decay, step, grad_scale, covered_rows, nullptr, nullptr, 0u, stream);
 }
 
 extern "C" int wisp_hashgrid_interpolate_bwd_adamw_tail(const float* coords, int64_t n, int coord_dim, const void* grad_feats,
@@ -1331,7 +1380,30 @@
     side.loss_partials = tail->loss_partials; side.loss = tail->loss; side.loss_count = tail->loss_count; side.inv_n = tail->inv_n;
     return bwd_adamw_impl(coords, n, coord_dim, grad_feats, dtype, feature_dim, first_idx, resolutions, num_lods, codebook_bitwidth,
                           zero_from_col, grad_codebook, workspace, workspace_bytes, level_cap_scale, param, exp_avg, exp_avg_sq, bf16_shadow,
-                          lr, beta1, beta2, eps, weight_decay, step, grad_scale, covered_rows, &side, tail_done, stream);
+                          lr, beta1, beta2, eps, weight_decay, step, grad_scale, covered_rows, &side, tail_done, 0u, stream);
+}
+
+extern "C" int wisp_hashgrid_interpolate_bwd_adamw_flags(const float* coords, int64_t n, int coord_dim, const void* grad_feats,
+                                                         int dtype, int feature_dim, const int64_t* first_idx,
+                                                         const int32_t* resolutions, int num_lods, int codebook_bitwidth,
+                                                         int zero_from_col, float* grad_codebook, void* workspace,
+                                                         int64_t workspace_bytes, const float* level_cap_scale, float* param,
+                                                         float* exp_avg, float* exp_avg_sq, void* bf16_shadow, float lr, float beta1,
+                                                         float beta2, float eps, float weight_decay, int64_t step, float grad_scale,
+                                                         int64_t* covered_rows, const wisp_step_tail* tail, int* tail_done,
+                                                         uint32_t flags, wisp_stream_t stream) {
+    WISP_REQUIRE((tail == nullptr) == (tail_done == nullptr), "side-job descriptor and its result go together");
+    WISP_REQUIRE((flags & ~(uint32_t)WISP_HG_BWD_GRAD_CLEAN) == 0, "unknown flag");
+    StepTail side{};
+    if (tail) {
+        WISP_REQUIRE(tail->dw_rows >= 0 && tail->loss_count >= 0 && tail->in_dim >= 1 && tail->in_dim <= wisp_mlp::IN, "side-job descriptor out of range");
+        *tail_done = 0;
+        side.dw_partials = tail->dw_partials; side.dec_grad = tail->dec_grad; side.dw_rows = tail->dw_rows; side.in_dim = tail->in_dim;
+        side.loss_partials = tail->loss_partials; side.loss = tail->loss; side.loss_count = tail->loss_count; side.inv_n = tail->inv_n;
+    }
+    return bwd_adamw_impl(coords, n, coord_dim, grad_feats, dtype, feature_dim, first_idx, resolutions, num_lods, codebook_bitwidth,
+                          zero_from_col, grad_codebook, workspace, workspace_bytes, level_cap_scale, param, exp_avg, exp_avg_sq, bf16_shadow,
+                          lr, beta1, beta2, eps, weight_decay, step, grad_scale, covered_rows, tail ? &side : nullptr, tail_done, flags, stream);
 }
 
 template <typename T>
@@ -1587,7 +1659,7 @@
     const uint32_t* __restrict__ c = counts + bins.cnt_base[li];
     const int64_t cells = (int64_t)bins.chunks[li] * ntiles;
     uint32_t m = 0, sum = 0;
-    for (int64_t e = threadIdx.x; e < cells; e += blockDim.x) { const uint32_t v = c[e]; m = max(m, v); sum += v; }
+    for (int64_t e = threadIdx.x; e < cells; e += blockDim.x) { const uint32_t v = c[e] & HG_WORD_MASK; m = max(m, v); sum += v; }
 #pragma unroll
     for (int d = 32; d >= 1; d >>= 1) { m = max(m, (uint32_t)__shfl_xor((int)m, d, 64)); sum += (uint32_t)__shfl_xor((int)sum, d, 64); }
     if ((threadIdx.x & 63) == 0) { s_max[threadIdx.x >> 6] = m; s_sum[threadIdx.x >> 6] = sum; }
diff --git a/kaolin-wisp_amd/csrc/train_step.hip b/kaolin-wisp_amd/csrc/train_step.hip
--- a/kaolin-wisp_amd/csrc/train_step.hip
+++ b/kaolin-wisp_amd/csrc/train_step.hip
@@ -82,6 +82,7 @@
     std::vector<hipEvent_t> ev;
     std::vector<int64_t> ev_units;
     int timed_steps = 0;
+    bool grad_clean = false;
 };
 
 template <typename T> static T* at(const Step* s, int64_t off) { return reinterpret_cast<T*>(s->ws + off); }
@@ -190,6 +191,13 @@
     s->res.assign(cfg->resolutions, cfg->resolutions + cfg->num_lods);
     s->cfg.first_idx_host = s->first_idx_host.data();
     s->cfg.resolutions = s->res.data();
+    s->grad_clean = false;
+    return WISP_OK;
+}
+
+extern "C" int wisp_nerf_step_grad_clean(void* step) {
+    WISP_REQUIRE(step, "null handle");
+    static_cast<Step*>(step)->grad_clean = true;
     return WISP_OK;
 }
 
@@ -218,6 +226,8 @@
                                   int record_timing, int64_t* num_samples, int64_t* covered_rows, float** loss, wisp_stream_t stream) {
     WISP_REQUIRE(step && (slot == 0 || slot == 1) && gts && hp && num_samples && loss, "null argument");
     Step* s = static_cast<Step*>(step);
+    const uint32_t hg_flags = s->grad_clean ? WISP_HG_BWD_GRAD_CLEAN : 0u;
+    s->grad_clean = false;
     const wisp_nerf_step_config& c = s->cfg;
     MarchSlot& m = s->slot[slot];
     WISP_REQUIRE(m.counted, "this slot holds no counted batch (wisp_nerf_step_count first)");
@@ -310,21 +320,21 @@
     NS_MARK(4);
     if (tail_fold) {
         int tail_done = 0;
-        NS_CALL(wisp_hashgrid_interpolate_bwd_adamw_tail(samples, S, 3, g_feats, c.dtype_table, c.feature_dim, c.first_idx, c.resolutions,
-                                                         c.num_lods, c.bitwidth, c.zero_from_col, c.table_grad, hashgrid_workspace,
-                                                         hashgrid_workspace_bytes, level_cap_scale, c.table_param, c.table_exp_avg,
-                                                         c.table_exp_avg_sq, c.table_shadow, hp->lr_grid, hp->beta1, hp->beta2, hp->eps,
-                                                         hp->weight_decay, hp->step, hp->grad_scale, covered, &tail, &tail_done, st));
+        NS_CALL(wisp_hashgrid_interpolate_bwd_adamw_flags(samples, S, 3, g_feats, c.dtype_table, c.feature_dim, c.first_idx, c.resolutions,
+                                                          c.num_lods, c.bitwidth, c.zero_from_col, c.table_grad, hashgrid_workspace,
+                                                          hashgrid_workspace_bytes, level_cap_scale, c.table_param, c.table_exp_avg,
+                                                          c.table_exp_avg_sq, c.table_shadow, hp->lr_grid, hp->beta1, hp->beta2, hp->eps,
+                                                          hp->weight_decay, hp->step, hp->grad_scale, covered, &tail, &tail_done, hg_flags, st));
         if (!tail_done) {
             NS_CALL(wisp_nerf_mlp_reduce_partials(tail.dw_partials, tail.dw_rows, tail.in_dim, tail.dec_grad, st));
             NS_CALL(wisp_loss_sum(tail.loss_partials, tail.loss_count, tail.inv_n, tail.loss, st));
         }
     } else if (fold)
-        NS_CALL(wisp_hashgrid_interpolate_bwd_adamw(samples, S, 3, g_feats, c.dtype_table, c.feature_dim, c.first_idx, c.resolutions,
-                                                    c.num_lods, c.bitwidth, c.zero_from_col, c.table_grad, hashgrid_workspace,
-                                                    hashgrid_workspace_bytes, level_cap_scale, c.table_param, c.table_exp_avg,
-                                                    c.table_exp_avg_sq, c.table_shadow, hp->lr_grid, hp->beta1, hp->beta2, hp->eps,
-                                                    hp->weight_decay, hp->step, hp->grad_scale, covered, st));
+        NS_CALL(wisp_hashgrid_interpolate_bwd_adamw_flags(samples, S, 3, g_feats, c.dtype_table, c.feature_dim, c.first_idx, c.resolutions,
+                                                          c.num_lods, c.bitwidth, c.zero_from_col, c.table_grad, hashgrid_workspace,
+                                                          hashgrid_workspace_bytes, level_cap_scale, c.table_param, c.table_exp_avg,
+                                                          c.table_exp_avg_sq, c.table_shadow, hp->lr_grid, hp->beta1, hp->beta2, hp->eps,
+                                                          hp->weight_decay, hp->step, hp->grad_scale, covered, nullptr, nullptr, hg_flags, st));
     else
         NS_CALL(wisp_hashgrid_interpolate_bwd(samples, S, 3, g_feats, c.dtype_table, c.feature_dim, c.first_idx, c.resolutions, c.num_lods,
                                               c.bitwidth, c.zero_from_col, c.table_grad, hashgrid_workspace, hashgrid_workspace_bytes,
diff --git a/kaolin-wisp_amd/wisp/_C.py b/kaolin-wisp_amd/wisp/_C.py
--- a/kaolin-wisp_amd/wisp/_C.py
+++ b/kaolin-wisp_amd/wisp/_C.py
@@ -28,6 +28,9 @@
                                             c_vp, c_vp, c_vp, c_vp, c_f32, c_f32, c_f32, c_f32, c_f32, c_i64, c_f32, c_vp, c_vp],
     "wisp_hashgrid_interpolate_bwd_adamw_tail": [c_vp, c_i64, c_i32, c_vp, c_i32, c_i32, c_vp, c_vp, c_i32, c_i32, c_i32, c_vp, c_vp, c_i64, c_vp,
                                                  c_vp, c_vp, c_vp, c_vp, c_f32, c_f32, c_f32, c_f32, c_f32, c_i64, c_f32, c_vp, c_vp, c_vp, c_vp],
+    "wisp_hashgrid_interpolate_bwd_adamw_flags": [c_vp, c_i64, c_i32, c_vp, c_i32, c_i32, c_vp, c_vp, c_i32, c_i32, c_i32, c_vp, c_vp, c_i64, c_vp,
+                                                  c_vp, c_vp, c_vp, c_vp, c_f32, c_f32, c_f32, c_f32, c_f32, c_i64, c_f32, c_vp, c_vp, c_vp,
+                                                  ctypes.c_uint32, c_vp],
     "wisp_hashgrid_grad_coords": [c_vp, c_i64, c_i32, c_vp, c_vp, c_i32, c_i32, c_vp, c_vp, c_i32, c_i32, c_vp, c_vp],
     "wisp_hashgrid_bwd_workspace_bytes": [c_i64, c_i32, c_i32, c_i32, c_vp, c_i32, c_i32, c_vp],
     "wisp_hashgrid_bwd_slot_stats": [c_i64, c_i32, c_i32, c_i32, c_vp, c_i32, c_i32, c_i32, c_vp, c_vp, c_i64, c_vp, c_vp, c_vp, c_vp],
@@ -152,6 +155,7 @@
     "wisp_nerf_step_reconfigure": [c_vp, c_vp],
     "wisp_nerf_step_destroy": [c_vp],
     "wisp_nerf_step_count": [c_vp, c_i32, c_vp, c_vp, c_i64, c_u64, c_vp],
+    "wisp_nerf_step_grad_clean": [c_vp],
     "wisp_nerf_step_run": [c_vp, c_i32, c_vp, c_vp, c_vp, c_i64, c_u64, c_vp, c_vp, c_vp, c_i64, c_i32, c_vp, c_vp, c_vp, c_vp],
     "wisp_nerf_step_read_timing": [c_vp, c_i32, c_vp, c_vp, c_vp],
     "wisp_mesh_to_sdf": [c_vp, c_i64, c_vp, c_i64, c_i32, c_i64, c_vp, c_vp, c_i64, c_vp],
@@ -423,14 +427,15 @@
                 assert t.is_cuda and t.dtype == torch.float32 and t.is_contiguous() and t.numel() == grad.numel()
             assert sh is None or (sh.dtype == torch.bfloat16 and sh.is_contiguous() and sh.numel() == grad.numel())
             cov = (ctypes.c_int64 * L)()
-            _check(lib.wisp_hashgrid_interpolate_bwd_adamw(_p(coords), n, dim, _p(grad_feats), dt, F,
-                                                           _p(first_idx), res_ptr, L, codebook_bitwidth, zero_from_col, _p(grad),
-                                                           _p(ws), ws.numel() if ws is not None else 0, scale_ptr,
-                                                           _p(prm), _p(m1), _p(m2), _p(sh), float(adamw["lr"]), float(adamw["beta1"]),
-                                                           float(adamw["beta2"]), float(adamw["eps"]), float(adamw["weight_decay"]),
-                                                           int(adamw["step"]), float(adamw.get("grad_scale", 1.0)),
-                                                           ctypes.cast(cov, ctypes.c_void_p), _stream()),
-                   "hashgrid_interpolate_bwd_adamw")
+            _check(lib.wisp_hashgrid_interpolate_bwd_adamw_flags(_p(coords), n, dim, _p(grad_feats), dt, F,
+                                                                 _p(first_idx), res_ptr, L, codebook_bitwidth, zero_from_col, _p(grad),
+                                                                 _p(ws), ws.numel() if ws is not None else 0, scale_ptr,
+                                                                 _p(prm), _p(m1), _p(m2), _p(sh), float(adamw["lr"]), float(adamw["beta1"]),
+                                                                 float(adamw["beta2"]), float(adamw["eps"]), float(adamw["weight_decay"]),
+                                                                 int(adamw["step"]), float(adamw.get("grad_scale", 1.0)),
+                                                                 ctypes.cast(cov, ctypes.c_void_p), None, None,
+                                                                 HG_BWD_GRAD_CLEAN if adamw.get("grad_clean") else 0, _stream()),
+                   "hashgrid_interpolate_bwd_adamw_flags")
             covered = [min(int(c), first_host[l + 1] - first_host[l]) for l, c in enumerate(cov)]
     if fit is not None and ws is not None:
         fit.after_launch(n, res_ptr, scale_arr, scale_ptr, ws, ws_bytes)
@@ -456,6 +461,7 @@
     return out
 
 
+HG_BWD_GRAD_CLEAN = 1
 HASHGRID_BWD_WORKSPACE_LIMIT = 24 << 30
 _bwd_ws = {}
 _slot_fits = {}
diff --git a/kaolin-wisp_amd/wisp/trainers/_native_step.py b/kaolin-wisp_amd/wisp/trainers/_native_step.py
--- a/kaolin-wisp_amd/wisp/trainers/_native_step.py
+++ b/kaolin-wisp_amd/wisp/trainers/_native_step.py
@@ -6,6 +6,7 @@
 
 ENABLED = os.environ.get("WISP_NATIVE_STEP", "1") != "0"
 TAIL_FOLD = os.environ.get("WISP_STEP_TAIL_FOLD", "1") != "0"
+grad_clean_enabled = lambda: os.environ.get("WISP_STEP_GRAD_CLEAN", "1") != "0"
 
 
 def _hip():
@@ -38,6 +39,9 @@
         self.hg_scale = None
         self.fallbacks = 0
         self.steps = 0
+        self.grad_clean = False
+        self.rebuilt = False
+        self.clean_steps = 0
 
     def applies(self, rays, jitter):
         t = self.t
@@ -67,6 +71,9 @@
             return False
         blas = grid.blas
         return blas.max_level <= 10 and rays.origins.shape[0] <= t.max_rays and rays.origins.is_contiguous() and rays.dirs.is_contiguous()
+
+    def dirty(self):
+        self.grad_clean = False
 
     def _capacity(self):
         t = self.t
@@ -93,6 +100,7 @@
                tuple(float(v) for v in tracer._bg_host()), torch.cuda.current_stream().cuda_stream)
         if self.handle is not None and key == self.key:
             return True
+        self.grad_clean, self.rebuilt = False, True
         level = blas.max_level
         occ = blas._bitfield(level)
         if occ is None:
@@ -197,8 +205,10 @@
     def step(self, rays, img_gts, prefetch):
         C = _hip()
         t, d = self.t, self.t._direct
+        clean, self.grad_clean, self.rebuilt = self.grad_clean, False, False
         if not self._ensure(rays):
             return None
+        clean = clean and not self.rebuilt and grad_clean_enabled()
         lib, h = C.lib, self.handle
         dev = rays.origins.device
         stream = C._stream()
@@ -230,6 +240,9 @@
         loss_ptr = ctypes.c_void_p()
         record = 1 if C.TIMING is not None else 0
         t.wait_for_parameters()
+        if clean and hp.optimizer == 2:
+            C._check(lib.wisp_nerf_step_grad_clean(h), "nerf_step_grad_clean")
+            self.clean_steps += 1
         rc = lib.wisp_nerf_step_run(h, slot, gts.data_ptr(),
                                     None if nxt is None else nxt["rays"].origins.data_ptr(), None if nxt is None else nxt["rays"].dirs.data_ptr(),
                                     0 if nxt is None else nxt["rays"].origins.shape[0], 0 if nxt is None else nxt["seed"],
@@ -253,6 +266,7 @@
             ga, gb = t.flat.ranges["grid"]
             t.fused_elements_last = 2 * sum(max(0, c) for c in cover)
             self.covered_last = cover
+            self.grad_clean = True
         else:
             t.fused_elements_last = 0
         t.flat.mark_shadow_current()
diff --git a/kaolin-wisp_amd/wisp/trainers/multiview_trainer.py b/kaolin-wisp_amd/wisp/trainers/multiview_trainer.py
--- a/kaolin-wisp_amd/wisp/trainers/multiview_trainer.py
+++ b/kaolin-wisp_amd/wisp/trainers/multiview_trainer.py
@@ -735,6 +735,8 @@
 
     def accumulate(self, rays: Rays, img_gts, jitter=None):
         assert self.grad_accum_steps > 1, "set grad_accum_steps to the number of micro-batches per optimizer step first"
+        if self._native is not None:
+            self._native.dirty()
         self._refuse_stale_master_forward()
         if self._direct is not None and self.pipeline.nef.training:
             with torch.no_grad():
@@ -763,6 +765,8 @@
                 loss = done[0]
                 self.calc_adaptive_rays(rays.origins.shape[0])
                 return loss, done[1]
+            if self._native is not None:
+                self._native.dirty()
             if not self._last_step_modular:
                 with torch.no_grad():
                     loss, _ = self._direct.run(rays, img_gts, jitter, prefetch, fused_update=self._fused_update_args())
```
